# vgl-hub/kreeq

Hardware: AMD Instinct MI355X
Metric: distinct+total k-mers/sec at k=21 (count path) (higher is better)
Workload: dtype u64

## Files before the change

### include/kreeq_amd.h

```cpp
#ifndef KREEQ_AMD_H
#define KREEQ_AMD_H

#include <stdint.h>

#ifdef __cplusplus
extern "C" {
#endif

#define KQ_ABI_VERSION 4

typedef enum {
    KQ_OK = 0,
    KQ_ERR_INVALID = -1,
    KQ_ERR_NO_DEVICE = -2,
    KQ_ERR_HIP = -3,
    KQ_ERR_NOMEM = -4,
    KQ_ERR_TABLE_FULL = -5,
    KQ_ERR_CAPACITY = -6,
    KQ_ERR_MISMATCH = -7
} kq_status;

typedef struct kq_handle kq_handle;

typedef struct {
    uint64_t key;
    uint32_t fw[4], bw[4], cov;
    uint32_t hc;
} kq_entry;

typedef struct {
    uint32_t fw, bw, cov;
    uint8_t  isFw;
    uint8_t  pad[3];
} kq_dbgbase;

typedef struct {
    uint64_t total;
    uint64_t unique;
    uint64_t distinct;
    uint64_t missing;
    uint64_t edges;
} kq_stats;

typedef struct {
    uint64_t kmers_counted;
    uint64_t slots_used;
    uint64_t slots_total;
    uint64_t hc_used;
    uint64_t hc_total;
    uint64_t table_bytes;
    uint64_t table_passes;
} kq_info;


int  kq_create(kq_handle** out, int device, int k, int map_count, uint64_t capacity_hint);
void kq_destroy(kq_handle* h);
int  kq_clear(kq_handle* h);
int  kq_set_stream(kq_handle* h, void* hip_stream);
void* kq_get_stream(kq_handle* h);
enum { KQ_OPT_TRUST_CAPACITY = 1, KQ_OPT_COUNT_PATH = 2, KQ_OPT_SLICE_KMERS = 3, KQ_OPT_COUNT_MAP_RANGE = 4, KQ_OPT_PROFILE = 5,
       KQ_OPT_LOOKUP_PATH = 6, KQ_OPT_MERGE_PATH = 7, KQ_OPT_NARROW_MID = 8, KQ_OPT_PENDING_BYTES = 9, KQ_OPT_BUCKET_WINDOW = 10, KQ_OPT_OVERLAP = 11, KQ_OPT_COUNT_MAP_PASSES = 12, KQ_OPT_KERNEL_SET = 13, KQ_OPT_SHARD_WINDOW = 14, KQ_OPT_SUBGRAPH_BATCH = 15, KQ_OPT_VARIANT_BATCH = 16,
       KQ_OPT_TEST_FAIL_PLAN = 100  };
int  kq_set_option(kq_handle* h, int option, int64_t value);
int  kq_get_profile(kq_handle* h, char* buf, uint64_t cap);
int  kq_sync(kq_handle* h);
int  kq_flush(kq_handle* h);
int  kq_get_info(kq_handle* h, kq_info* out);
const char* kq_last_error(void);
int  kq_abi_version(void);
int  kq_device_available(void);
int  kq_device_memory(int device, uint64_t* free_bytes, uint64_t* total_bytes);


int  kq_count_batch(kq_handle* h, const char* bases, uint64_t len);
int  kq_count_batch_dev(kq_handle* h, const char* d_bases, uint64_t len);

void* kq_host_alloc(uint64_t bytes);
void  kq_host_free(void* p);
int  kq_count_batch_async(kq_handle* h, const char* bases, uint64_t len, uint64_t* ticket);
int  kq_host_wait(kq_handle* h, uint64_t ticket);

void kq_pack_bases(const char* bases, uint64_t len, uint32_t* codes, uint16_t* inv);
int  kq_count_packed_dev(kq_handle* h, const uint32_t* d_codes, const uint16_t* d_inv, uint64_t n_bases);
int  kq_count_packed_async(kq_handle* h, const uint32_t* codes, const uint16_t* inv, uint64_t n_bases, uint64_t* ticket);

int  kq_pack_bases_dev(kq_handle* h, const char* d_bases, uint64_t len, uint32_t* d_codes, uint16_t* d_inv);

enum { KQ_FASTX_FASTQ = 1, KQ_FASTX_FASTA = 2 };
int  kq_parse_fastx_dev(kq_handle* h, const char* d_text, uint64_t len, int format, char* d_bases, uint64_t cap, uint64_t* n_bases);
int  kq_count_fastx_dev(kq_handle* h, const char* d_text, uint64_t len, int format);
int  kq_count_fastx_async(kq_handle* h, const char* text, uint64_t len, int format, uint64_t* ticket);

typedef struct { uint64_t off; uint32_t size; uint32_t data_off; uint32_t data_len; uint32_t crc32; uint32_t isize; } kq_bgzf_block;
enum { KQ_BGZF_END = 1 };
int  kq_bgzf_scan(const void* data, uint64_t len, kq_bgzf_block* blocks, uint64_t cap, uint64_t* n_blocks, uint64_t* consumed);
int  kq_inflate_bgzf_dev(kq_handle* h, const void* d_comp, uint64_t comp_len, const kq_bgzf_block* blocks, uint64_t n_blocks,
                         char* d_text, uint64_t cap, uint64_t* n_text);
int  kq_count_bgzf_dev(kq_handle* h, const void* d_comp, uint64_t comp_len, const kq_bgzf_block* blocks, uint64_t n_blocks, int format, uint32_t flags);

enum { KQ_BGZF_EOF = 2 };
uint64_t kq_bgzf_bound(uint64_t n_text, uint32_t flags);
int  kq_deflate_bgzf_dev(kq_handle* h, const char* d_text, uint64_t n_text, void* d_out, uint64_t cap, uint64_t* n_out, uint32_t flags);
int  kq_deflate_bgzf(kq_handle* h, const char* text, uint64_t n_text, void* out, uint64_t cap, uint64_t* n_out, uint32_t flags);

int  kq_emit_records(kq_handle* h, const char* bases, uint64_t len,
                     uint64_t* keys, uint8_t* edges, uint64_t cap, uint64_t* n_out);
int  kq_emit_partitioned_dev(kq_handle* h, const char* d_bases, uint64_t len, int n_parts,
                             uint64_t* d_keys, uint8_t* d_edges, uint64_t cap,
                             uint64_t* part_counts);

int  kq_emit_packed_dev(kq_handle* h, const char* d_bases, uint64_t len, int n_parts,
                        uint64_t* d_recs, uint64_t cap, uint64_t* part_counts);
int  kq_insert_packed_dev(kq_handle* h, const uint64_t* d_recs, uint64_t n);

int  kq_emit_sharded_dev(kq_handle* h, const char* d_bases, uint64_t len, int n_parts, uint32_t* d_recs, uint8_t* d_aux, uint64_t cap,
                         uint64_t* d_bucket_counts, uint64_t* part_counts);
int  kq_insert_sharded_dev(kq_handle* h, const uint32_t* d_recs, const uint8_t* d_aux, uint64_t n, int n_peers, const uint64_t* d_bucket_counts);

int  kq_emit_sharded8_dev(kq_handle* h, const char* d_bases, uint64_t len, int n_parts, uint64_t* d_recs, uint64_t cap,
                          uint64_t* d_bucket_counts, uint64_t* part_counts);
int  kq_insert_sharded8_dev(kq_handle* h, const uint64_t* d_recs, uint64_t n, int n_peers, const uint64_t* d_bucket_counts);

int  kq_insert_records(kq_handle* h, const uint64_t* keys, const uint8_t* edges, uint64_t n);
int  kq_insert_records_dev(kq_handle* h, const uint64_t* d_keys, const uint8_t* d_edges, uint64_t n);


int  kq_summary(kq_handle* h, kq_stats* out);
int  kq_histogram(kq_handle* h, uint64_t* cov, uint64_t* cnt, uint64_t cap, uint64_t* n_out);


int  kq_lookup_sequence(kq_handle* h, const char* bases, uint64_t len, uint32_t cov_cutoff,
                        uint16_t map_lo, uint16_t map_hi, kq_dbgbase* per_base,
                        uint64_t counters[3]);
int  kq_lookup_sequence_dev(kq_handle* h, const char* d_bases, uint64_t len, uint32_t cov_cutoff,
                            uint16_t map_lo, uint16_t map_hi, kq_dbgbase* d_per_base,
                            uint64_t* d_counters);


enum { KQ_COPY_TO_DEVICE = 1, KQ_COPY_TO_HOST = 2 };
void* kq_dev_alloc(kq_handle* h, uint64_t bytes);
void  kq_dev_free(kq_handle* h, void* p);
int   kq_copy_async(kq_handle* h, void* dst, const void* src, uint64_t bytes, int kind);

int  kq_per_base_triples_dev(kq_handle* h, const kq_dbgbase* d_per_base, const uint64_t* seg_start, const uint64_t* seg_len,
                             uint64_t n_segs, uint32_t* d_triples);

int  kq_per_base_merge_dev(kq_handle* h, kq_dbgbase* d_per_base, const uint64_t* seg_start, const uint64_t* seg_len,
                           uint64_t n_segs, uint32_t* d_triples);

typedef struct { uint64_t first, n, abs_pos; uint32_t name_off, name_len, n_ctx, flags; } kq_table_seg;
enum { KQ_TABLE_SEG_HEADER = 1 };
enum { KQ_TABLE_KWIG = 1, KQ_TABLE_BED = 2, KQ_TABLE_CSV = 3 };
int  kq_format_table_dev(kq_handle* h, int format, const uint32_t* d_triples, uint64_t n_triples, const kq_table_seg* segs, uint64_t n_segs,
                         const char* names, uint64_t names_len, char* d_out, uint64_t cap, uint64_t* n_out);
int  kq_format_table(kq_handle* h, int format, const uint32_t* triples, uint64_t n_triples, const kq_table_seg* segs, uint64_t n_segs,
                     const char* names, uint64_t names_len, char* out, uint64_t cap, uint64_t* n_out);


int  kq_lookup_keys(kq_handle* h, const uint64_t* keys, uint64_t n, kq_entry* out);

int  kq_branch_scan(kq_handle* h, const char* bases, uint64_t len, uint32_t cov_cutoff, uint8_t* flags);

typedef struct { uint64_t pos, seg_start, seq_off; uint16_t seq_len, ref_len; uint8_t type, pad[3]; } kq_variant_path;
enum { KQ_VAR_SNV = 0, KQ_VAR_INS = 1, KQ_VAR_DEL = 2, KQ_VAR_COM = 3 };
int  kq_search_variants(kq_handle* h, const char* bases, uint64_t len, int depth, int max_span, uint32_t cov_cutoff,
                        kq_variant_path* paths, uint64_t path_cap, uint64_t* n_paths,
                        char* seq, uint64_t seq_cap, uint64_t* n_seq);


int  kq_merge(kq_handle* dst, kq_handle* src);

int  kq_import(kq_handle* h, const kq_entry* entries, uint64_t n);
int  kq_export(kq_handle* h, uint16_t map_lo, uint16_t map_hi, kq_entry* out, uint64_t cap,
               uint64_t* n_out);


int  kq_export_map_images(kq_handle* h, uint16_t map_lo, uint16_t map_hi, void* out, uint64_t cap, uint64_t* offsets,
                          kq_entry* hc_out, uint64_t hc_cap, uint64_t* n_hc);
int  kq_import_map_image(kq_handle* h, uint16_t map, const void* image, uint64_t n_bytes, uint64_t* n_entries,
                         uint64_t* n_tombstones);


enum { KQ_SUBGRAPH_NO_REFERENCE = 1 };
int  kq_subgraph_seed(kq_handle* db, kq_handle* sub, const char* bases, uint64_t len, uint32_t flags);
int  kq_subgraph_seed_dev(kq_handle* db, kq_handle* sub, const char* d_bases, uint64_t len, uint32_t flags);
int  kq_subgraph_expand(kq_handle* db, kq_handle* sub, int depth, uint64_t* n_added);
int  kq_subgraph_best_first(kq_handle* db, kq_handle* sub, int depth, uint32_t cov_cutoff, uint64_t* n_added);
int  kq_subgraph_trim(kq_handle* sub, uint32_t cov_cutoff);

typedef struct { uint64_t seq_off, head_key; uint32_t n_kmers, cov; uint8_t head_rc, pad[7]; } kq_gfa_segment;
typedef struct { uint32_t from, to, count; uint8_t from_rc, to_rc, pad[2]; } kq_gfa_edge;
typedef struct { uint64_t n_segments, n_seq, n_edges, n_dropped_edges, n_cycles; } kq_gfa_counts;
enum { KQ_GFA_NO_COLLAPSE = 1 };
int  kq_subgraph_gfa(kq_handle* sub, uint32_t flags, kq_gfa_segment* segs, uint64_t seg_cap, char* seq, uint64_t seq_cap,
                     kq_gfa_edge* edges, uint64_t edge_cap, kq_gfa_counts* counts);

#ifdef __cplusplus
}
#endif
#endif
```

### kreeq_amd/capi.py

```python
import ctypes as C
import os

import numpy as np

from . import build as _build

ENTRY_DTYPE = np.dtype([("key", "<u8"), ("fw", "<u4", 4), ("bw", "<u4", 4), ("cov", "<u4"), ("hc", "<u4")])
DBGBASE_DTYPE = np.dtype([("fw", "<u4"), ("bw", "<u4"), ("cov", "<u4"), ("isFw", "u1"), ("pad", "u1", 3)])
VARIANT_PATH_DTYPE = np.dtype([("pos", "<u8"), ("seg_start", "<u8"), ("seq_off", "<u8"), ("seq_len", "<u2"), ("ref_len", "<u2"), ("type", "u1"), ("pad", "u1", 3)])
VAR_SNV, VAR_INS, VAR_DEL, VAR_COM = 0, 1, 2, 3
ERR_CAPACITY = -6

SYMBOLS = ["kq_create", "kq_destroy", "kq_clear", "kq_set_option", "kq_get_profile", "kq_set_stream", "kq_get_stream", "kq_sync", "kq_flush", "kq_get_info", "kq_last_error",
           "kq_abi_version", "kq_device_available", "kq_device_memory", "kq_count_batch", "kq_count_batch_dev", "kq_host_alloc", "kq_host_free", "kq_count_batch_async", "kq_host_wait", "kq_pack_bases", "kq_count_packed_dev", "kq_count_packed_async",
           "kq_pack_bases_dev", "kq_parse_fastx_dev", "kq_count_fastx_dev", "kq_count_fastx_async", "kq_bgzf_scan", "kq_inflate_bgzf_dev", "kq_count_bgzf_dev", "kq_bgzf_bound", "kq_deflate_bgzf_dev", "kq_deflate_bgzf", "kq_emit_records",
           "kq_emit_partitioned_dev", "kq_emit_packed_dev", "kq_insert_packed_dev", "kq_emit_sharded_dev", "kq_insert_sharded_dev", "kq_emit_sharded8_dev", "kq_insert_sharded8_dev", "kq_insert_records", "kq_insert_records_dev", "kq_summary", "kq_histogram",
           "kq_lookup_sequence", "kq_lookup_sequence_dev", "kq_dev_alloc", "kq_dev_free", "kq_copy_async", "kq_per_base_triples_dev", "kq_per_base_merge_dev", "kq_format_table_dev", "kq_format_table", "kq_lookup_keys", "kq_branch_scan", "kq_search_variants", "kq_merge", "kq_import", "kq_export",
           "kq_export_map_images", "kq_import_map_image", "kq_subgraph_seed", "kq_subgraph_seed_dev", "kq_subgraph_expand", "kq_subgraph_best_first", "kq_subgraph_trim", "kq_subgraph_gfa"]

FASTX_FASTQ, FASTX_FASTA = 1, 2
BGZF_END = 1
BGZF_EOF = 2
BGZF_MEMBER_TEXT = 0xff00
BGZF_BLOCK_DTYPE = np.dtype([("off", "<u8"), ("size", "<u4"), ("data_off", "<u4"), ("data_len", "<u4"), ("crc32", "<u4"), ("isize", "<u4"), ("pad", "<u4")])
# ... 64 lines not shown
    L = C.CDLL(path)
    vp, u64, u32, u16, ci = C.c_void_p, C.c_uint64, C.c_uint32, C.c_uint16, C.c_int
    L.kq_create.argtypes = [C.POINTER(vp), ci, ci, ci, u64]
    L.kq_destroy.argtypes = [vp]
    L.kq_destroy.restype = None
    L.kq_clear.argtypes = [vp]
    L.kq_set_stream.argtypes = [vp, vp]
    L.kq_set_option.argtypes = [vp, ci, C.c_int64]
    L.kq_get_profile.argtypes = [vp, C.c_char_p, u64]
    L.kq_get_stream.argtypes = [vp]
    L.kq_get_stream.restype = vp
    L.kq_sync.argtypes = [vp]
    L.kq_flush.argtypes = [vp]
    L.kq_get_info.argtypes = [vp, C.POINTER(Info)]
    L.kq_last_error.restype = C.c_char_p
    L.kq_device_memory.argtypes = [ci, C.POINTER(u64), C.POINTER(u64)]
    L.kq_count_batch.argtypes = [vp, vp, u64]
    L.kq_count_batch_dev.argtypes = [vp, vp, u64]
    L.kq_host_alloc.argtypes = [u64]
    L.kq_host_alloc.restype = vp
    L.kq_host_free.argtypes = [vp]
    L.kq_host_free.restype = None
    L.kq_count_batch_async.argtypes = [vp, vp, u64, C.POINTER(u64)]
    L.kq_host_wait.argtypes = [vp, u64]
    L.kq_pack_bases.argtypes = [vp, u64, vp, vp]
    L.kq_pack_bases.restype = None
    L.kq_count_packed_dev.argtypes = [vp, vp, vp, u64]
    L.kq_count_packed_async.argtypes = [vp, vp, vp, u64, C.POINTER(u64)]
    L.kq_pack_bases_dev.argtypes = [vp, vp, u64, vp, vp]
    L.kq_parse_fastx_dev.argtypes = [vp, vp, u64, ci, vp, u64, C.POINTER(u64)]
    L.kq_count_fastx_dev.argtypes = [vp, vp, u64, ci]
    L.kq_count_fastx_async.argtypes = [vp, vp, u64, ci, C.POINTER(u64)]
    L.kq_bgzf_scan.argtypes = [vp, u64, vp, u64, C.POINTER(u64), C.POINTER(u64)]
    L.kq_inflate_bgzf_dev.argtypes = [vp, vp, u64, vp, u64, vp, u64, C.POINTER(u64)]
    L.kq_count_bgzf_dev.argtypes = [vp, vp, u64, vp, u64, ci, u32]
    L.kq_bgzf_bound.argtypes = [u64, u32]
    L.kq_bgzf_bound.restype = u64
    L.kq_deflate_bgzf_dev.argtypes = [vp, vp, u64, vp, u64, C.POINTER(u64), u32]
    L.kq_deflate_bgzf.argtypes = [vp, vp, u64, vp, u64, C.POINTER(u64), u32]
    L.kq_emit_records.argtypes = [vp, vp, u64, vp, vp, u64, C.POINTER(u64)]
    L.kq_emit_partitioned_dev.argtypes = [vp, vp, u64, ci, vp, vp, u64, vp]
    L.kq_emit_packed_dev.argtypes = [vp, vp, u64, ci, vp, u64, vp]
    L.kq_insert_packed_dev.argtypes = [vp, vp, u64]
    L.kq_emit_sharded_dev.argtypes = [vp, vp, u64, ci, vp, vp, u64, vp, vp]
    L.kq_insert_sharded_dev.argtypes = [vp, vp, vp, u64, ci, vp]
    L.kq_emit_sharded8_dev.argtypes = [vp, vp, u64, ci, vp, u64, vp, vp]
    L.kq_insert_sharded8_dev.argtypes = [vp, vp, u64, ci, vp]
    L.kq_insert_records.argtypes = [vp, vp, vp, u64]
    L.kq_insert_records_dev.argtypes = [vp, vp, vp, u64]
    L.kq_summary.argtypes = [vp, C.POINTER(Stats)]
    L.kq_histogram.argtypes = [vp, vp, vp, u64, C.POINTER(u64)]
    L.kq_lookup_sequence.argtypes = [vp, vp, u64, u32, u16, u16, vp, vp]
    L.kq_lookup_sequence_dev.argtypes = [vp, vp, u64, u32, u16, u16, vp, vp]
    L.kq_dev_alloc.argtypes = [vp, u64]
    L.kq_dev_alloc.restype = vp
    L.kq_dev_free.argtypes = [vp, vp]
    L.kq_dev_free.restype = None
    L.kq_copy_async.argtypes = [vp, vp, vp, u64, ci]
    L.kq_per_base_triples_dev.argtypes = [vp, vp, vp, vp, u64, vp]
    L.kq_per_base_merge_dev.argtypes = [vp, vp, vp, vp, u64, vp]
    L.kq_format_table_dev.argtypes = [vp, ci, vp, u64, vp, u64, vp, u64, vp, u64, C.POINTER(u64)]
    L.kq_format_table.argtypes = [vp, ci, vp, u64, vp, u64, vp, u64, vp, u64, C.POINTER(u64)]
    L.kq_lookup_keys.argtypes = [vp, vp, u64, vp]
    L.kq_branch_scan.argtypes = [vp, vp, u64, u32, vp]
    L.kq_search_variants.argtypes = [vp, vp, u64, ci, ci, u32, vp, u64, C.POINTER(u64), vp, u64, C.POINTER(u64)]
    L.kq_merge.argtypes = [vp, vp]
    L.kq_import.argtypes = [vp, vp, u64]
    L.kq_export.argtypes = [vp, u16, u16, vp, u64, C.POINTER(u64)]
    L.kq_export_map_images.argtypes = [vp, u16, u16, vp, u64, vp, vp, u64, C.POINTER(u64)]
    L.kq_import_map_image.argtypes = [vp, u16, vp, u64, C.POINTER(u64), C.POINTER(u64)]
    L.kq_subgraph_seed.argtypes = [vp, vp, vp, u64, u32]
    L.kq_subgraph_seed_dev.argtypes = [vp, vp, vp, u64, u32]
    L.kq_subgraph_expand.argtypes = [vp, vp, ci, C.POINTER(u64)]
    L.kq_subgraph_best_first.argtypes = [vp, vp, ci, u32, C.POINTER(u64)]
    L.kq_subgraph_trim.argtypes = [vp, u32]
    L.kq_subgraph_gfa.argtypes = [vp, u32, vp, u64, vp, u64, vp, u64, C.POINTER(GfaCounts)]
    _lib = L
    return L


def _check(rc):
    if rc != 0:
        raise KqError(rc, load().kq_last_error().decode(errors="replace"))


def _p(a):
    return a.ctypes.data_as(C.c_void_p) if a is not None else None


def pack_bases(bases: bytes):
    buf = np.frombuffer(bases, dtype=np.uint8)
    units = (len(buf) + 15) // 16
    codes, inv = np.zeros(max(units, 1), dtype=np.uint32), np.zeros(max(units, 1), dtype=np.uint16)
    load().kq_pack_bases(_p(buf) if len(buf) else None, len(buf), _p(codes), _p(inv))
    return codes[:units], inv[:units]


def bgzf_bound(n_text, flags=0):
    return int(load().kq_bgzf_bound(n_text, flags))


def bgzf_scan(data: bytes, cap=None):
    buf = np.frombuffer(data, dtype=np.uint8)
    n, used = C.c_uint64(0), C.c_uint64(0)
    L = load()
    room = len(buf) // 26 + 1 if cap is None else cap
    blocks = np.zeros(max(room, 1), dtype=BGZF_BLOCK_DTYPE)
    rc = L.kq_bgzf_scan(_p(buf) if len(buf) else None, len(buf), _p(blocks) if room else None, room, C.byref(n), C.byref(used))
    if rc != 0:
        e = KqError(rc, L.kq_last_error().decode(errors="replace"))
        e.n_blocks, e.consumed = n.value, used.value
        raise e
    return blocks[:n.value], used.value


def device_available():
    return bool(load().kq_device_available())


def device_memory(device=0):
    f, t = C.c_uint64(0), C.c_uint64(0)
    _check(load().kq_device_memory(device, C.byref(f), C.byref(t)))
    return f.value, t.value


class KreeqDB:

    def __init__(self, k=21, map_count=128, device=0, capacity_hint=0):
        self.k, self.map_count, self.device = k, map_count, device
        self._h = C.c_void_p()
        _check(load().kq_create(C.byref(self._h), device, k, map_count, capacity_hint))

    def close(self, _load=load):
        if getattr(self, "_h", None):
            _load().kq_destroy(self._h)
            self._h = None

    __del__ = close

    @property
    def handle(self):
        return self._h

    def set_stream(self, hip_stream_ptr):
        _check(load().kq_set_stream(self._h, C.c_void_p(hip_stream_ptr)))

    def sync(self):
        _check(load().kq_sync(self._h))

    def flush(self):
        _check(load().kq_flush(self._h))

    def set_option(self, option, value):
        opt = {"trust_capacity": 1, "count_path": 2, "slice_kmers": 3, "count_map_range": 4, "profile": 5, "lookup_path": 6, "merge_path": 7, "narrow_mid": 8, "pending_bytes": 9, "bucket_window": 10, "overlap": 11, "count_map_passes": 12, "kernel_set": 13, "shard_window": 14, "subgraph_batch": 15, "variant_batch": 16, "test_fail_plan": 100}[option]
        if option == "count_map_range":
            value = int(value[0]) | (int(value[1]) << 16)
        if option in ("count_path", "lookup_path", "merge_path"):
            value = {"auto": 0, "direct": 1, "partitioned": 2}[value]
        _check(load().kq_set_option(self._h, opt, int(value)))

    def clear(self):
        _check(load().kq_clear(self._h))

    def profile(self):
        buf = C.create_string_buffer(1024)
        _check(load().kq_get_profile(self._h, buf, 1024))
        return {k: float(v) for k, v in (kv.split("=") for kv in buf.value.decode().split(";") if kv)}

    def info(self):
        i = Info()
        _check(load().kq_get_info(self._h, C.byref(i)))
        return {f: getattr(i, f) for f, _ in Info._fields_}

    def count_batch(self, bases: bytes):
        buf = np.frombuffer(bases, dtype=np.uint8)
        _check(load().kq_count_batch(self._h, _p(buf), len(buf)))

    def count_batch_async(self, host_ptr, n):
        t = C.c_uint64(0)
        _check(load().kq_count_batch_async(self._h, C.c_void_p(host_ptr), n, C.byref(t)))
        return t.value

    def count_packed_dev(self, codes_ptr, inv_ptr, n_bases):
        _check(load().kq_count_packed_dev(self._h, C.c_void_p(codes_ptr), C.c_void_p(inv_ptr), n_bases))

    def count_packed_async(self, codes_ptr, inv_ptr, n_bases):
        t = C.c_uint64(0)
        _check(load().kq_count_packed_async(self._h, C.c_void_p(codes_ptr), C.c_void_p(inv_ptr), n_bases, C.byref(t)))
        return t.value

    def pack_bases_dev(self, bases_ptr, n, codes_ptr, inv_ptr):
        _check(load().kq_pack_bases_dev(self._h, C.c_void_p(bases_ptr), n, C.c_void_p(codes_ptr), C.c_void_p(inv_ptr)))

    def parse_fastx_dev(self, text_ptr, n, fmt, out_ptr, cap):
        nb = C.c_uint64(0)
        rc = load().kq_parse_fastx_dev(self._h, C.c_void_p(text_ptr), n, fmt, C.c_void_p(out_ptr) if out_ptr else None, cap, C.byref(nb))
        if rc != 0:
            e = KqError(rc, load().kq_last_error().decode(errors="replace"))
            e.needed = nb.value
            raise e
        return nb.value

    def count_fastx_dev(self, text_ptr, n, fmt):
        _check(load().kq_count_fastx_dev(self._h, C.c_void_p(text_ptr), n, fmt))

    def count_fastx_async(self, host_ptr, n, fmt):
        t = C.c_uint64(0)
        _check(load().kq_count_fastx_async(self._h, C.c_void_p(host_ptr), n, fmt, C.byref(t)))
        return t.value

    def inflate_bgzf_dev(self, comp_ptr, comp_len, blocks, out_ptr, cap):
        blocks = np.ascontiguousarray(blocks, dtype=BGZF_BLOCK_DTYPE)
        nt = C.c_uint64(0)
        rc = load().kq_inflate_bgzf_dev(self._h, C.c_void_p(comp_ptr), comp_len, _p(blocks) if len(blocks) else None, len(blocks),
                                        C.c_void_p(out_ptr) if out_ptr else None, cap, C.byref(nt))
        if rc != 0:
            e = KqError(rc, load().kq_last_error().decode(errors="replace"))
            e.needed = nt.value
            raise e
        return nt.value

    def deflate_bgzf_dev(self, text_ptr, n_text, out_ptr, cap, flags=0):
        no = C.c_uint64(0)
        rc = load().kq_deflate_bgzf_dev(self._h, C.c_void_p(text_ptr) if text_ptr else None, n_text, C.c_void_p(out_ptr) if out_ptr else None, cap, C.byref(no), flags)
        if rc != 0:
            e = KqError(rc, load().kq_last_error().decode(errors="replace"))
            e.needed = no.value
            raise e
        return no.value

    def deflate_bgzf(self, text: bytes, flags=0, cap=None):
        src = np.frombuffer(text, dtype=np.uint8)
        room = bgzf_bound(len(src), flags) if cap is None else cap
        out = np.empty(max(room, 1), dtype=np.uint8)
        no = C.c_uint64(0)
        rc = load().kq_deflate_bgzf(self._h, _p(src) if len(src) else None, len(src), _p(out) if room else None, room, C.byref(no), flags)
        if rc != 0:
            e = KqError(rc, load().kq_last_error().decode(errors="replace"))
            e.needed = no.value
            raise e
        return out[:no.value].tobytes()

    def count_bgzf_dev(self, comp_ptr, comp_len, blocks, fmt, flags=0):
        blocks = np.ascontiguousarray(blocks, dtype=BGZF_BLOCK_DTYPE)
        _check(load().kq_count_bgzf_dev(self._h, C.c_void_p(comp_ptr), comp_len, _p(blocks) if len(blocks) else None, len(blocks), fmt, flags))

    def host_wait(self, ticket):
        _check(load().kq_host_wait(self._h, ticket))

    def count_batch_dev(self, ptr, n):
        _check(load().kq_count_batch_dev(self._h, C.c_void_p(ptr), n))

    def emit_records(self, bases: bytes):
        buf = np.frombuffer(bases, dtype=np.uint8)
        n = C.c_uint64(0)
        _check(load().kq_emit_records(self._h, _p(buf), len(buf), None, None, 0, C.byref(n)))
        keys = np.empty(n.value, dtype=np.uint64)
        edges = np.empty(n.value, dtype=np.uint8)
        if n.value:
            _check(load().kq_emit_records(self._h, _p(buf), len(buf), _p(keys), _p(edges), n.value, C.byref(n)))
        return keys, edges

    def emit_partitioned_dev(self, bases_ptr, n, n_parts, keys_ptr, edges_ptr, cap):
        counts = np.zeros(n_parts, dtype=np.uint64)
        _check(load().kq_emit_partitioned_dev(self._h, C.c_void_p(bases_ptr), n, n_parts, C.c_void_p(keys_ptr), C.c_void_p(edges_ptr),
                                              cap, _p(counts)))
        return counts

    def emit_packed_dev(self, bases_ptr, n, n_parts, recs_ptr, cap):
        counts = np.zeros(n_parts, dtype=np.uint64)
        _check(load().kq_emit_packed_dev(self._h, C.c_void_p(bases_ptr), n, n_parts, C.c_void_p(recs_ptr), cap, _p(counts)))
        return counts

    def insert_packed_dev(self, recs_ptr, n):
        _check(load().kq_insert_packed_dev(self._h, C.c_void_p(recs_ptr), n))

    def emit_sharded_dev(self, bases_ptr, n, n_parts, recs_ptr, aux_ptr, cap, bucket_counts_ptr, sync=True):
        counts = np.zeros(n_parts, dtype=np.uint64) if sync else None
        _check(load().kq_emit_sharded_dev(self._h, C.c_void_p(bases_ptr), n, n_parts, C.c_void_p(recs_ptr), C.c_void_p(aux_ptr), cap,
                                          C.c_void_p(bucket_counts_ptr), _p(counts)))
        return counts

    def insert_sharded_dev(self, recs_ptr, aux_ptr, n, n_peers, bucket_counts_ptr):
        _check(load().kq_insert_sharded_dev(self._h, C.c_void_p(recs_ptr), C.c_void_p(aux_ptr), n, n_peers, C.c_void_p(bucket_counts_ptr)))

    def emit_sharded8_dev(self, bases_ptr, n, n_parts, recs_ptr, cap, bucket_counts_ptr, sync=True):
        counts = np.zeros(n_parts, dtype=np.uint64) if sync else None
        _check(load().kq_emit_sharded8_dev(self._h, C.c_void_p(bases_ptr), n, n_parts, C.c_void_p(recs_ptr), cap,
                                           C.c_void_p(bucket_counts_ptr), _p(counts)))
        return counts

    def insert_sharded8_dev(self, recs_ptr, n, n_peers, bucket_counts_ptr):
        _check(load().kq_insert_sharded8_dev(self._h, C.c_void_p(recs_ptr), n, n_peers, C.c_void_p(bucket_counts_ptr)))

    def insert_records(self, keys, edges):
        keys = np.ascontiguousarray(keys, dtype=np.uint64)
        edges = np.ascontiguousarray(edges, dtype=np.uint8)
        assert len(keys) == len(edges)
        _check(load().kq_insert_records(self._h, _p(keys), _p(edges), len(keys)))

    def insert_records_dev(self, keys_ptr, edges_ptr, n):
        _check(load().kq_insert_records_dev(self._h, C.c_void_p(keys_ptr), C.c_void_p(edges_ptr), n))

    def summary(self, with_hist=False):
        st = Stats()
        _check(load().kq_summary(self._h, C.byref(st)))
        d = {f: getattr(st, f) for f, _ in Stats._fields_}
# ... 165 lines not shown
```

### kreeq_amd/csrc/kq_formats.h

```cpp
#pragma once
#include <cstdint>
namespace kq {
#ifndef KQ_REGION_SHIFT
#define KQ_REGION_SHIFT 11
#endif
constexpr int REGION_SHIFT = KQ_REGION_SHIFT;
constexpr uint32_t REGION_SLOTS = 1u << REGION_SHIFT;
constexpr int HI_K = 29;
constexpr int TILE_STARTS = 4032;
constexpr uint64_t n_tiles_of(uint64_t lead, uint64_t len) { return (lead + len + TILE_STARTS - 1) / TILE_STARTS; }
struct EmitRange { uint64_t lo, hi; };

constexpr int NB_MAX = 2048;
constexpr int PART_MAX_K = 28;
constexpr int FMT_PACK8 = 0, FMT_WIDE = 1, FMT_NARROW = 2;
constexpr int FMT_PACK8_TO_NARROW = 3;
constexpr uint32_t NARROW_CBITS = 8, NARROW_MAX_K = 21;
constexpr int FMT_TOP8 = 4;
constexpr int FMT_TIGHT = 5;
constexpr int FMT_NARROW_TO_TIGHT = 6;

constexpr int MS_THREADS = 256;
constexpr int MS_ITEMS = 16;
constexpr int MS_TILE = MS_THREADS * MS_ITEMS;
constexpr int SEG_MAX = 65536;
constexpr uint32_t SUB_BITS_MAX = 8;
constexpr int AUX_IDX6 = 0, AUX_EDGE_BYTE = 1, AUX_TIGHT = 2;
constexpr uint64_t TIGHT_MIN_REGIONS = 1ull << 16;
constexpr int P1_F = 1;
constexpr uint32_t P2_UNIT = 4 * MS_TILE;
constexpr uint32_t SCAN_CHUNK = 16384;

struct PartCfg {
    uint64_t n_regions;
    uint32_t g_shift;
    uint32_t n_coarse;
    uint32_t mode;
    uint32_t map_count;
    uint32_t map_mask;
    uint32_t filt_lo, filt_hi;
    uint32_t raw_out;
    uint32_t narrow;
    uint32_t owner_sub;
    uint32_t sub_bits;
    uint32_t win_lo, win_hi;
    uint32_t n_rng;
};

constexpr int P3_MAX_SETS = 64;
struct P3Set { const uint64_t* recs; const uint8_t* aux; const unsigned long long* base; uint64_t n_max; };

struct LevelCfg {
    uint64_t n_regions;
    uint32_t n_seg, nb, seg_shift, out_shift;
    uint32_t in_raw;
    uint32_t k;
    uint32_t narrow;
    uint32_t top8;
    uint32_t nr_shift, nr_rps, nr_sub, nr_div, nr_inv;
    uint32_t nr_mid, nr_fshift, nr_fmask, nr_f24;
    uint32_t spb;
    uint32_t rep_shift;
    const uint32_t* rstart = nullptr;
};
}
```

### kreeq_amd/csrc/kq_kernels.h

```cpp
#pragma once

#include <hip/hip_runtime.h>

#include <type_traits>

#include "../../include/kreeq_amd.h"
#include "kq_device.h"
#include "kq_partition.h"

using namespace kq;


__global__ __launch_bounds__(TILE_THREADS) void k_count_direct(TableView t, const uint8_t* __restrict__ ab,
                                                                uint64_t lead, uint64_t len, int k, EmitRange er, PartCfg filt,
                                                                const uint16_t* __restrict__ pinv ) {
    uint32_t n_new = 0;
    uint64_t n_kmers = 0;
    scan_tiles(ab, lead, len, k, [&](uint64_t pos, uint64_t fw, uint64_t rv, uint32_t prev, uint32_t next) {
        if (pos < er.lo || pos >= er.hi) return;
        const bool is_fw = fw < rv;
        const uint64_t key = is_fw ? fw : rv;
        if (filt.filt_lo != 0 || filt.filt_hi != filt.map_count) {
            const uint32_t m = map_index(key, filt.map_count, filt.map_mask);
            if (m < filt.filt_lo || m >= filt.filt_hi) return;
// ... 360 lines not shown
        __syncthreads();
        const uint32_t total = __builtin_amdgcn_readfirstlane(s_loff[NB]);
        s_hist[ct] = 0;
        p1c_steps(total, (uint32_t)THREADS, [&](auto n_it) {
            constexpr int N = decltype(n_it)::value;
            uint64_t cv[N];
            uint32_t cg[N];
#pragma unroll
            for (int it = 0; it < N; ++it) cv[it] = s_buf[ct + it * THREADS];
#pragma unroll
            for (int it = 0; it < N; ++it) cg[it] = s_grel[ct + it * THREADS < total ? narrow_word_bin(cv[it]) : 0u] + (ct + it * THREADS);
            landed(nxt.x); landed(nxt.y); landed(nxt.z); landed(nxt.w);
#pragma unroll
            for (int it = 0; it < N; ++it) {
                if (ct + it * THREADS < total) { recs[cg[it]] = (uint32_t)cv[it]; recs_aux[cg[it]] = (uint8_t)(cv[it] >> 48); }
            }
        });
        landed(nxt.x); landed(nxt.y); landed(nxt.z); landed(nxt.w);
    }
}

__global__ __launch_bounds__(1024) void k_lv_units(const unsigned long long* __restrict__ seg_off, const unsigned long long* __restrict__ seg_hi, LevelCfg lv,
                                                   unsigned long long* __restrict__ unit_base) {
    __shared__ unsigned long long s_part[1024];
    const uint32_t tid = threadIdx.x, per = (lv.n_seg + 1023) / 1024;
    const uint32_t lo = min(tid * per, lv.n_seg), hi = min(lo + per, lv.n_seg);
    unsigned long long sum = 0;
    for (uint32_t b = lo; b < hi; ++b) sum += (seg_hi[b] - seg_off[b] + P2_UNIT - 1) / P2_UNIT;
    s_part[tid] = sum;
    __syncthreads();
    if (tid < 64) {
        unsigned long long loc[16], tot = 0;
#pragma unroll
        for (int j = 0; j < 16; ++j) { loc[j] = s_part[tid * 16 + j]; tot += loc[j]; }
        unsigned long long incl = tot;
#pragma unroll
        for (int o = 1; o < 64; o <<= 1) { unsigned long long nn = __shfl_up(incl, o, 64); if ((int)tid >= o) incl += nn; }
        unsigned long long run = incl - tot;
#pragma unroll
        for (int j = 0; j < 16; ++j) { s_part[tid * 16 + j] = run; run += loc[j]; }
        if (tid == 63) unit_base[lv.n_seg] = incl;
    }
    __syncthreads();
    unsigned long long run = s_part[tid];
    for (uint32_t b = lo; b < hi; ++b) { unit_base[b] = run; run += (seg_hi[b] - seg_off[b] + P2_UNIT - 1) / P2_UNIT; }
}
__device__ __forceinline__ uint32_t seg_of_unit(const unsigned long long* unit_base, uint32_t n_seg, uint64_t u) {
    uint32_t lo = 0, hi = n_seg;
    while (hi - lo > 1) { uint32_t mid = (lo + hi) >> 1; if (unit_base[mid] <= u) lo = mid; else hi = mid; }
    return lo;
}
template <int FMT>
__global__ __launch_bounds__(MS_THREADS) void k_lv_hist(const uint64_t* __restrict__ recs, const uint8_t* __restrict__ , LevelCfg lv,
                                                        const unsigned long long* __restrict__ seg_off, const unsigned long long* __restrict__ seg_hi,
                                                        const unsigned long long* __restrict__ unit_base, uint32_t* __restrict__ m2) {
    __shared__ uint32_t s_hist[NB_MAX];
    const uint64_t n_units = unit_base[lv.n_seg];
    for (uint64_t u = blockIdx.x; u < n_units; u += gridDim.x) {
        const uint32_t b_in = seg_of_unit(unit_base, lv.n_seg, u);
        const uint32_t b = lv.spb > 1 ? b_in / lv.spb : b_in;
        const uint64_t lo = seg_off[b_in] + (u - unit_base[b_in]) * P2_UNIT;
        const uint64_t hi = lo + P2_UNIT < seg_hi[b_in] ? lo + P2_UNIT : seg_hi[b_in];
        for (uint32_t i = threadIdx.x; i < lv.nb; i += MS_THREADS) s_hist[i] = 0;
        __syncthreads();
        const uint64_t last = hi - 1;
        if (FMT == FMT_NARROW) {
            const uint4* v4 = reinterpret_cast<const uint4*>(recs);
            const uint64_t q0 = lo >> 2, q1 = (hi + 3) >> 2;
            for (uint64_t qb = q0; qb < q1; qb += 4ull * MS_THREADS) {
                uint4 q[4];
#pragma unroll
                for (int j = 0; j < 4; ++j) q[j] = v4[min(qb + (uint64_t)j * MS_THREADS + threadIdx.x, q1 - 1)];
#pragma unroll
                for (int j = 0; j < 4; ++j) {
                    const uint64_t qi = qb + (uint64_t)j * MS_THREADS + threadIdx.x;
                    const uint32_t e[4] = {q[j].x, q[j].y, q[j].z, q[j].w};
#pragma unroll
                    for (int c = 0; c < 4; ++c) {
                        const uint64_t ri = 4 * qi + c;
                        if (qi < q1 && ri >= lo && ri < hi) atomicAdd(&s_hist[narrow_bin(lv, b, e[c])], 1u);
                    }
                }
            }
        } else
        for (uint64_t base = lo; base < hi; base += 8ull * MS_THREADS) {
            uint64_t r[8];
#pragma unroll
            for (int j = 0; j < 8; ++j) {
                const uint64_t i = min(base + (uint64_t)j * MS_THREADS + threadIdx.x, last);
                r[j] = FMT == FMT_NARROW ? (uint64_t)reinterpret_cast<const uint32_t*>(recs)[i] : recs[i];
            }
#pragma unroll
            for (int j = 0; j < 8; ++j)
                if (base + (uint64_t)j * MS_THREADS + threadIdx.x < hi) {
                    const uint32_t bin = FMT == FMT_NARROW ? narrow_bin(lv, b, (uint32_t)r[j])
                        : FMT == FMT_TOP8 ? narrow_bin(lv, b, (uint32_t)(r[j] >> 32))
                        : (FMT == FMT_PACK8 && lv.top8) ? (uint32_t)(rec_hash<false>(r[j]) >> (64 - NARROW_CBITS))
                        : level_bin(lv, b, hash_region(lv.in_raw ? table_hash(r[j], lv.k) : rec_hash<FMT == FMT_WIDE>(r[j]), lv.n_regions));
                    atomicAdd(&s_hist[bin], 1u);
                }
        }
        __syncthreads();
        for (uint32_t i = threadIdx.x; i < lv.nb; i += MS_THREADS) m2[u * lv.nb + i] = s_hist[i];
        __syncthreads();
    }
}
__global__ __launch_bounds__(256) void k_lv_offsets(uint32_t* __restrict__ m2, LevelCfg lv, const unsigned long long* __restrict__ unit_base,
                                                    unsigned long long* __restrict__ group_count) {
    const uint64_t r = ((uint64_t)blockIdx.x * blockDim.x + threadIdx.x) >> 6;
    const uint32_t lane = threadIdx.x & 63;
    const uint32_t n_lseg = lv.n_seg / lv.spb;
    if (r >= (uint64_t)n_lseg * lv.nb) return;
    const uint32_t b = (uint32_t)(r / lv.nb), bin = (uint32_t)(r % lv.nb);
    const uint64_t u0 = unit_base[b * lv.spb], u1 = unit_base[(b + 1) * lv.spb];
    unsigned long long run = 0;
    for (uint64_t base = u0; base < u1; base += 64) {
        const uint64_t u = base + lane;
        const uint32_t c = u < u1 ? m2[u * lv.nb + bin] : 0u;
        unsigned long long incl = c;
#pragma unroll
        for (int o = 1; o < 64; o <<= 1) { const unsigned long long n = __shfl_up(incl, o, 64); if ((int)lane >= o) incl += n; }
        if (u < u1) m2[u * lv.nb + bin] = (uint32_t)(run + incl - c);
        run += __shfl(incl, 63, 64);
    }
    if (lane == 0) group_count[r] = run;
}
__global__ __launch_bounds__(256) void k_lv_offsets_thread(uint32_t* __restrict__ m2, LevelCfg lv, const unsigned long long* __restrict__ unit_base,
                                                           unsigned long long* __restrict__ group_count) {
    const uint64_t r = (uint64_t)blockIdx.x * blockDim.x + threadIdx.x;
    const uint32_t n_lseg = lv.n_seg / lv.spb;
    if (r >= (uint64_t)n_lseg * lv.nb) return;
    const uint32_t b = (uint32_t)(r / lv.nb), bin = (uint32_t)(r % lv.nb);
    const uint64_t u0 = unit_base[b * lv.spb], u1 = unit_base[(b + 1) * lv.spb];
    unsigned long long run = 0;
    for (uint64_t u = u0; u < u1; ++u) {
        const uint32_t c = m2[u * lv.nb + bin];
        m2[u * lv.nb + bin] = (uint32_t)run;
        run += c;
    }
    group_count[r] = run;
}
#ifndef KQ_LV_THREADS
#define KQ_LV_THREADS 512
#define KQ_LV_ITEMS 8
#define KQ_LV_OCC 4
#endif
constexpr int LV_THREADS = KQ_LV_THREADS, LV_ITEMS = KQ_LV_ITEMS, LV_TILE = LV_THREADS * LV_ITEMS;
template <int FMT, int NBC>
__global__ __launch_bounds__(LV_THREADS, KQ_LV_OCC) void k_lv_scatter(const uint64_t* __restrict__ recs, const uint8_t* __restrict__ recs_aux, LevelCfg lv,
                                                           const unsigned long long* __restrict__ seg_off, const unsigned long long* __restrict__ seg_hi,
                                                           const unsigned long long* __restrict__ unit_base, const uint32_t* __restrict__ m2,
                                                           const unsigned long long* __restrict__ group_base, uint64_t* __restrict__ out,
                                                           uint8_t* __restrict__ out_aux) {
    constexpr bool WIDE = FMT == FMT_WIDE, TIGHT = FMT == FMT_NARROW_TO_TIGHT, NARROW = FMT == FMT_NARROW || TIGHT, CONVERT = FMT == FMT_PACK8_TO_NARROW,
                   TOP8 = FMT == FMT_TOP8, HAS_AUX = WIDE || NARROW;
    constexpr int MS_FMT = (CONVERT || TIGHT) ? FMT_NARROW : TOP8 ? FMT_PACK8 : FMT;
    const uint32_t* recs32 = reinterpret_cast<const uint32_t*>(recs);
    __shared__ MsShared<NBC, MS_FMT, LV_TILE> s;
    __shared__ uint32_t s_rst[TIGHT ? NBC : 1];
    const uint32_t nb = lv.nb;
    const uint64_t n_units = unit_base[lv.n_seg];
    for (uint64_t u = blockIdx.x; u < n_units; u += gridDim.x) {
        const uint32_t b_in = seg_of_unit(unit_base, lv.n_seg, u);
        const uint32_t b = lv.spb > 1 ? b_in / lv.spb : b_in;
        const uint64_t lo = seg_off[b_in] + (u - unit_base[b_in]) * P2_UNIT;
        const uint64_t hi = lo + P2_UNIT < seg_hi[b_in] ? lo + P2_UNIT : seg_hi[b_in];
        for (uint32_t i = threadIdx.x; i < nb; i += LV_THREADS)
            s.gbase[i] = (uint32_t)(group_base[(uint64_t)b * nb + i] + m2[u * nb + i]);
        if (TIGHT) {
            const uint32_t first = (b >> lv.nr_shift) * lv.nr_rps + (b & ((1u << lv.nr_shift) - 1u)) * lv.nr_sub;
            for (uint32_t i = threadIdx.x; i < nb; i += LV_THREADS) s_rst[i] = lv.rstart[first + i];
        }
        __syncthreads();
        uint64_t nxt[LV_ITEMS];
        uint32_t nxt_aux[LV_ITEMS];
        const uint64_t last = hi - 1;
#pragma unroll
        for (int j = 0; j < LV_ITEMS; ++j) {
            const uint64_t i = min(lo + (uint64_t)j * LV_THREADS + threadIdx.x, last);
            nxt[j] = NARROW ? (uint64_t)recs32[i] : recs[i];
            nxt_aux[j] = HAS_AUX ? recs_aux[i] : 0;
        }
#pragma unroll
        for (int j = 0; j < LV_ITEMS; ++j) { landed(nxt[j]); if (HAS_AUX) landed(nxt_aux[j]); }
        for (uint64_t pos = lo; pos < hi; pos += LV_TILE) {
            uint64_t rec[LV_ITEMS];
            uint32_t aux[LV_ITEMS], bin[LV_ITEMS];
#pragma unroll
            for (int j = 0; j < LV_ITEMS; ++j) {
                const uint64_t i = pos + (uint64_t)j * LV_THREADS + threadIdx.x;
                rec[j] = (WIDE && lv.in_raw) ? table_hash(nxt[j], lv.k) : nxt[j];
                aux[j] = nxt_aux[j];
                if (TIGHT) {
                    const uint32_t bn = i >= hi ? nb : narrow_bin(lv, b, (uint32_t)rec[j]);
                    rec[j] = narrow_word(tight_rec(b >> lv.nr_shift, (uint32_t)rec[j], aux[j], s_rst[bn < nb ? bn : 0u]), 0u, bn);
                }
                else if (NARROW) rec[j] = narrow_word((uint32_t)rec[j], aux[j], i >= hi ? nb : narrow_bin(lv, b, (uint32_t)rec[j]));
                else if (CONVERT) {
                    const uint64_t hh = rec_hash<false>(rec[j]);
                    rec[j] = narrow_word(narrow_main(hh), narrow_aux(hh, (uint32_t)(rec[j] >> REC_EDGE_SHIFT) & 63u), i >= hi ? nb : (uint32_t)(hh >> (64 - NARROW_CBITS)));
                }
                else if (TOP8) bin[j] = i >= hi ? nb : narrow_bin(lv, b, (uint32_t)(rec[j] >> 32));
                else bin[j] = i >= hi ? nb : level_bin(lv, b, hash_region(rec_hash<WIDE>(rec[j]), lv.n_regions));
            }
#pragma unroll
            for (int j = 0; j < LV_ITEMS; ++j) {
                const uint64_t i = min(pos + LV_TILE + (uint64_t)j * LV_THREADS + threadIdx.x, last);
                nxt[j] = NARROW ? (uint64_t)recs32[i] : recs[i];
                nxt_aux[j] = HAS_AUX ? recs_aux[i] : 0;
            }
            block_multisplit<MS_FMT, LV_THREADS, LV_ITEMS>(s, rec, aux, bin, nb, out, out_aux, [&] {
#pragma unroll
                for (int j = 0; j < LV_ITEMS; ++j) { landed(nxt[j]); if (HAS_AUX) landed(nxt_aux[j]); }
            }, NBC <= 512 ? lv.rep_shift : 0u);
        }
    }
}
#ifndef KQ_LVS_OCC
#define KQ_LVS_OCC 4
#define KQ_LVS_OCC_TIGHT 4
#endif
template <bool TIGHT>
__global__ __launch_bounds__(LV_THREADS, TIGHT ? KQ_LVS_OCC_TIGHT : KQ_LVS_OCC) void k_lv_scatter_s(const uint32_t* __restrict__ recs32, const uint8_t* __restrict__ recs_aux, LevelCfg lv,
                                                           const unsigned long long* __restrict__ seg_off, const unsigned long long* __restrict__ seg_hi,
                                                           const unsigned long long* __restrict__ unit_base, const uint32_t* __restrict__ m2,
                                                           const unsigned long long* __restrict__ group_base, uint32_t* __restrict__ out,
                                                           uint8_t* __restrict__ out_aux) {
    constexpr int NC = 512;
    static_assert(LV_THREADS == NC && LV_ITEMS == 8, "one counter per thread");
    __shared__ uint64_t s_buf[LV_TILE];
    __shared__ uint32_t s_hist[2][NC], s_loff[NC + 1], s_grel[NC], s_wave[LV_THREADS / 64];
    __shared__ uint32_t s_rst[TIGHT ? NC : 1];
    const int tid = threadIdx.x;
    const uint32_t nb = lv.nb, rs = lv.rep_shift, n_ctr = (nb + 1) << rs;
    const uint32_t sub = (uint32_t)tid & ((1u << rs) - 1u), my_bin = (uint32_t)tid >> rs;
    const bool own_bin = sub == 0 && my_bin < nb;
    const uint64_t n_units = unit_base[lv.n_seg];
    for (uint64_t u = blockIdx.x; u < n_units; u += gridDim.x) {
        const uint32_t b_in = seg_of_unit(unit_base, lv.n_seg, u);
        const uint32_t b = lv.spb > 1 ? b_in / lv.spb : b_in;
        const uint64_t lo = seg_off[b_in] + (u - unit_base[b_in]) * P2_UNIT;
        const uint64_t hi = lo + P2_UNIT < seg_hi[b_in] ? lo + P2_UNIT : seg_hi[b_in];
        uint32_t gabs = own_bin ? (uint32_t)(group_base[(uint64_t)b * nb + my_bin] + m2[u * nb + my_bin]) : 0u;
        if (TIGHT) {
            const uint32_t first = (b >> lv.nr_shift) * lv.nr_rps + (b & ((1u << lv.nr_shift) - 1u)) * lv.nr_sub;
            if ((uint32_t)tid < nb) s_rst[tid] = lv.rstart[first + tid];
        }
        s_hist[0][tid] = 0;
        __syncthreads();
        uint32_t nxt[LV_ITEMS], nxt_aux[LV_ITEMS];
        const uint64_t last = hi - 1;
#pragma unroll
        for (int j = 0; j < LV_ITEMS; ++j) {
            const uint64_t i = min(lo + (uint64_t)j * LV_THREADS + tid, last);
            nxt[j] = recs32[i];
            nxt_aux[j] = recs_aux[i];
        }
#pragma unroll
        for (int j = 0; j < LV_ITEMS; ++j) { landed(nxt[j]); landed(nxt_aux[j]); }
        uint32_t par = 0;
        for (uint64_t pos = lo; pos < hi; pos += LV_TILE, par ^= 1u) {
            uint32_t* hist = s_hist[par];
            uint64_t w[LV_ITEMS];
#pragma unroll
            for (int j = 0; j < LV_ITEMS; ++j) {
                const uint64_t i = pos + (uint64_t)j * LV_THREADS + tid;
                const uint32_t bn = i >= hi ? nb : narrow_bin(lv, b, nxt[j]);
                w[j] = TIGHT ? narrow_word(tight_rec(b >> lv.nr_shift, nxt[j], nxt_aux[j], s_rst[bn < nb ? bn : 0u]), 0u, bn) : narrow_word(nxt[j], nxt_aux[j], bn);
                if (bn != nb) atomicAdd(&hist[(bn << rs) | sub], 1u);
            }
#pragma unroll
            for (int j = 0; j < LV_ITEMS; ++j) {
                const uint64_t i = min(pos + LV_TILE + (uint64_t)j * LV_THREADS + tid, last);
                nxt[j] = recs32[i];
                nxt_aux[j] = recs_aux[i];
            }
            __syncthreads();
            const uint32_t cnt = (uint32_t)tid < n_ctr ? hist[tid] : 0u;
            uint32_t incl = cnt;
#pragma unroll
            for (int o = 1; o < 64; o <<= 1) { const uint32_t n = __shfl_up(incl, o, 64); if ((tid & 63) >= o) incl += n; }
            if ((tid & 63) == 63) s_wave[tid >> 6] = incl;
            s_hist[par ^ 1u][tid] = 0;
            __syncthreads();
            uint32_t excl = incl - cnt;
            for (int v = 0; v < (tid >> 6); ++v) excl += s_wave[v];
            s_loff[tid] = excl;
            hist[tid] = excl;
            if (own_bin) s_grel[my_bin] = gabs - excl;
            __syncthreads();
            if (own_bin) gabs += s_loff[(my_bin + 1) << rs] - excl;
#pragma unroll
            for (int j = 0; j < LV_ITEMS; ++j) {
                const uint32_t bn = narrow_word_bin(w[j]);
                if (bn != nb) s_buf[atomicAdd(&hist[(bn << rs) | sub], 1u)] = w[j];
            }
            __syncthreads();
            const uint32_t total = s_loff[nb << rs];
            uint64_t cv[LV_ITEMS];
            uint32_t cg[LV_ITEMS];
#pragma unroll
            for (int it = 0; it < LV_ITEMS; ++it) cv[it] = s_buf[tid + it * LV_THREADS];
#pragma unroll
            for (int it = 0; it < LV_ITEMS; ++it) cg[it] = s_grel[(uint32_t)(tid + it * LV_THREADS) < total ? narrow_word_bin(cv[it]) : 0u] + (tid + it * LV_THREADS);
#pragma unroll
            for (int j = 0; j < LV_ITEMS; ++j) { landed(nxt[j]); landed(nxt_aux[j]); }
#pragma unroll
            for (int it = 0; it < LV_ITEMS; ++it) {
                if ((uint32_t)(tid + it * LV_THREADS) < total) {
                    out[cg[it]] = (uint32_t)cv[it];
                    if (!TIGHT) out_aux[cg[it]] = (uint8_t)(cv[it] >> 48);
                }
            }
        }
    }
}
#ifndef KQ_LVG_BACK
#define KQ_LVG_BACK 0
#endif
__global__ __launch_bounds__(LV_THREADS, KQ_LVS_OCC_TIGHT) void k_lv_segment_s(const uint32_t* __restrict__ recs32, const uint8_t* __restrict__ recs_aux, LevelCfg lv,
                                                           const unsigned long long* __restrict__ seg_off, unsigned long long* __restrict__ gb,
                                                           uint32_t* __restrict__ out) {
    constexpr int NC = 512;
    constexpr bool BACK = KQ_LVG_BACK != 0;
    static_assert(LV_THREADS == NC && LV_ITEMS == 8, "one counter per thread");
    __shared__ uint64_t s_buf[LV_TILE];
    __shared__ uint32_t s_hist[2][NC], s_loff[NC + 1], s_grel[NC], s_wave[LV_THREADS / 64], s_rst[NC];
    const int tid = threadIdx.x;
    const uint32_t nb = lv.nb, rs = lv.rep_shift, n_ctr = (nb + 1) << rs;
    const uint32_t sub = (uint32_t)tid & ((1u << rs) - 1u), my_bin = (uint32_t)tid >> rs;
    const bool own_bin = sub == 0 && my_bin < nb;
    const uint32_t b = blockIdx.x;
    const uint64_t lo = seg_off[b], hi = seg_off[b + 1];
    {
        const uint32_t first = (b >> lv.nr_shift) * lv.nr_rps + (b & ((1u << lv.nr_shift) - 1u)) * lv.nr_sub;
        if ((uint32_t)tid < nb) s_rst[tid] = lv.rstart[first + tid];
    }
    s_hist[0][tid] = 0;
    s_hist[1][tid] = 0;
    __syncthreads();
    {
        const uint4* v4 = reinterpret_cast<const uint4*>(recs32);
        const uint64_t q0 = lo >> 2, q1 = hi > lo ? (hi + 3) >> 2 : q0;
        for (uint64_t qb = q0; qb < q1; qb += 4ull * LV_THREADS) {
            uint4 q[4];
#pragma unroll
            for (int j = 0; j < 4; ++j) q[j] = v4[min(qb + (uint64_t)j * LV_THREADS + tid, q1 - 1)];
#pragma unroll
            for (int j = 0; j < 4; ++j) {
                const uint64_t qi = qb + (uint64_t)j * LV_THREADS + tid;
                const uint32_t e[4] = {q[j].x, q[j].y, q[j].z, q[j].w};
#pragma unroll
                for (int c = 0; c < 4; ++c) {
                    const uint64_t ri = 4 * qi + c;
                    if (qi < q1 && ri >= lo && ri < hi) atomicAdd(&s_hist[1][(narrow_bin(lv, b, e[c]) << rs) | sub], 1u);
                }
            }
        }
    }
    __syncthreads();
    uint32_t gabs = 0;
    {
        uint32_t cnt = 0;
        if (own_bin) for (uint32_t r = 0; r < (1u << rs); ++r) cnt += s_hist[1][(uint32_t)tid + r];
        uint32_t incl = cnt;
#pragma unroll
        for (int o = 1; o < 64; o <<= 1) { const uint32_t n = __shfl_up(incl, o, 64); if ((tid & 63) >= o) incl += n; }
        if ((tid & 63) == 63) s_wave[tid >> 6] = incl;
        __syncthreads();
        uint32_t excl = incl - cnt;
        for (int v = 0; v < (tid >> 6); ++v) excl += s_wave[v];
        if (own_bin) {
            gabs = (uint32_t)lo + excl;
            gb[(uint64_t)b * nb + my_bin] = lo + excl;
        }
        if (b + 1 == lv.n_seg && tid == 0) gb[(uint64_t)lv.n_seg * nb] = hi;
    }
    if (hi == lo) return;
    uint32_t nxt[LV_ITEMS], nxt_aux[LV_ITEMS];
    const uint64_t last = hi - 1, n_rounds = (hi - lo + LV_TILE - 1) / LV_TILE;
    uint64_t pos = BACK ? lo + (n_rounds - 1) * LV_TILE : lo;
#pragma unroll
    for (int j = 0; j < LV_ITEMS; ++j) {
        const uint64_t i = min(pos + (uint64_t)j * LV_THREADS + tid, last);
        nxt[j] = recs32[i];
        nxt_aux[j] = recs_aux[i];
    }
#pragma unroll
    for (int j = 0; j < LV_ITEMS; ++j) { landed(nxt[j]); landed(nxt_aux[j]); }
    uint32_t par = 0;
    for (uint64_t r = 0; r < n_rounds; ++r, par ^= 1u) {
        uint32_t* hist = s_hist[par];
        uint64_t w[LV_ITEMS];
#pragma unroll
        for (int j = 0; j < LV_ITEMS; ++j) {
            const uint64_t i = pos + (uint64_t)j * LV_THREADS + tid;
            const uint32_t bn = i >= hi ? nb : narrow_bin(lv, b, nxt[j]);
            w[j] = narrow_word(tight_rec(b >> lv.nr_shift, nxt[j], nxt_aux[j], s_rst[bn < nb ? bn : 0u]), 0u, bn);
            if (bn != nb) atomicAdd(&hist[(bn << rs) | sub], 1u);
        }
        pos = BACK ? (r + 1 < n_rounds ? pos - LV_TILE : pos) : pos + LV_TILE;
#pragma unroll
        for (int j = 0; j < LV_ITEMS; ++j) {
            const uint64_t i = min(pos + (uint64_t)j * LV_THREADS + tid, last);
            nxt[j] = recs32[i];
            nxt_aux[j] = recs_aux[i];
        }
        __syncthreads();
        const uint32_t cnt = (uint32_t)tid < n_ctr ? hist[tid] : 0u;
        uint32_t incl = cnt;
#pragma unroll
        for (int o = 1; o < 64; o <<= 1) { const uint32_t n = __shfl_up(incl, o, 64); if ((tid & 63) >= o) incl += n; }
        if ((tid & 63) == 63) s_wave[tid >> 6] = incl;
        s_hist[par ^ 1u][tid] = 0;
        __syncthreads();
        uint32_t excl = incl - cnt;
        for (int v = 0; v < (tid >> 6); ++v) excl += s_wave[v];
        s_loff[tid] = excl;
        hist[tid] = excl;
        if (own_bin) s_grel[my_bin] = gabs - excl;
        __syncthreads();
        if (own_bin) gabs += s_loff[(my_bin + 1) << rs] - excl;
#pragma unroll
        for (int j = 0; j < LV_ITEMS; ++j) {
            const uint32_t bn = narrow_word_bin(w[j]);
            if (bn != nb) s_buf[atomicAdd(&hist[(bn << rs) | sub], 1u)] = w[j];
        }
        __syncthreads();
        const uint32_t total = s_loff[nb << rs];
        uint64_t cv[LV_ITEMS];
        uint32_t cg[LV_ITEMS];
#pragma unroll
        for (int it = 0; it < LV_ITEMS; ++it) cv[it] = s_buf[tid + it * LV_THREADS];
#pragma unroll
        for (int it = 0; it < LV_ITEMS; ++it) cg[it] = s_grel[(uint32_t)(tid + it * LV_THREADS) < total ? narrow_word_bin(cv[it]) : 0u] + (tid + it * LV_THREADS);
#pragma unroll
        for (int j = 0; j < LV_ITEMS; ++j) { landed(nxt[j]); landed(nxt_aux[j]); }
#pragma unroll
        for (int it = 0; it < LV_ITEMS; ++it)
            if ((uint32_t)(tid + it * LV_THREADS) < total) out[cg[it]] = (uint32_t)cv[it];
    }
}
__global__ void k_set2(unsigned long long* p, unsigned long long a, unsigned long long b) { p[0] = a; p[1] = b; }

__global__ __launch_bounds__(1024) void k_scan_sums(const unsigned long long* __restrict__ a, uint64_t n, unsigned long long* __restrict__ sums) {
    const uint64_t lo = (uint64_t)blockIdx.x * SCAN_CHUNK, hi = lo + SCAN_CHUNK < n ? lo + SCAN_CHUNK : n;
    unsigned long long v = 0;
    for (uint64_t i = lo + threadIdx.x; i < hi; i += 1024) v += a[i];
    uint64_t t = block_sum(v);
    if (threadIdx.x == 0) sums[blockIdx.x] = t;
}
__global__ __launch_bounds__(1024) void k_scan_apply(unsigned long long* __restrict__ a, uint64_t n, const unsigned long long* __restrict__ sums) {
    __shared__ unsigned long long s_part[1024];
    const uint64_t lo = (uint64_t)blockIdx.x * SCAN_CHUNK + (uint64_t)threadIdx.x * (SCAN_CHUNK / 1024);
    unsigned long long v[SCAN_CHUNK / 1024], sum = 0;
#pragma unroll
    for (uint32_t j = 0; j < SCAN_CHUNK / 1024; ++j) { v[j] = lo + j < n ? a[lo + j] : 0; sum += v[j]; }
    s_part[threadIdx.x] = sum;
    __syncthreads();
    if (threadIdx.x < 64) {
        unsigned long long loc[16], tot = 0;
#pragma unroll
        for (int j = 0; j < 16; ++j) { loc[j] = s_part[threadIdx.x * 16 + j]; tot += loc[j]; }
        unsigned long long incl = tot;
#pragma unroll
        for (int o = 1; o < 64; o <<= 1) { unsigned long long nn = __shfl_up(incl, o, 64); if ((int)threadIdx.x >= o) incl += nn; }
        unsigned long long run = incl - tot;
#pragma unroll
        for (int j = 0; j < 16; ++j) { s_part[threadIdx.x * 16 + j] = run; run += loc[j]; }
    }
    __syncthreads();
    unsigned long long run = sums[blockIdx.x] + s_part[threadIdx.x];
#pragma unroll
    for (uint32_t j = 0; j < SCAN_CHUNK / 1024; ++j) { if (lo + j < n) a[lo + j] = run; run += v[j]; }
}


template <class T> __device__ __forceinline__ T ld_global(const T* p) { return *(const __attribute__((address_space(1))) T*)p; }

template <uint32_t GRP, class LO = uint64_t>
struct SetTickets {
    LO lo; uint32_t cnt, first, n_grp;
    __device__ __forceinline__ void build(const P3Set* __restrict__ sets, uint32_t n_sets, uint64_t r, uint32_t lane) {
        lo = 0; cnt = 0;
        if (lane < n_sets) { const unsigned long long* b = ld_global(&sets[lane].base); lo = (LO)ld_global(b + r); cnt = (uint32_t)(ld_global(b + r + 1) - lo); }
        scan(lane);
    }
    __device__ __forceinline__ void build(const uint32_t* __restrict__ roff, uint32_t pitch, uint64_t r, uint32_t lane) {
        lo = 0; cnt = 0;
        if (lane < pitch) { const uint32_t* p = roff + r * pitch + lane; const uint32_t a = ld_global(p), b = ld_global(p + pitch); lo = a; cnt = b - a; }
        scan(lane);
    }
    __device__ __forceinline__ void scan(uint32_t lane) {
        const uint32_t mine = (cnt + GRP - 1) / GRP;
        uint32_t incl = mine;
#pragma unroll
        for (int o = 1; o < P3_MAX_SETS; o <<= 1) { const uint32_t v = __shfl_up(incl, o, 64); if ((int)lane >= o) incl += v; }
        first = incl - mine;
        n_grp = __builtin_amdgcn_readlane(incl, 63);
    }
    __device__ __forceinline__ void locate(uint32_t g, uint32_t& q, uint32_t& off, uint32_t& q_cnt, uint64_t& q_lo) const {
        const uint64_t nonempty = __ballot(cnt != 0);
        const uint64_t m = __ballot(cnt != 0 && first <= g);
        q = (g < n_grp && m) ? 63u - (uint32_t)__clzll((unsigned long long)m) : (uint32_t)__ffsll((unsigned long long)nonempty) - 1u;
        const uint32_t f = __builtin_amdgcn_readlane(first, q);
        q_cnt = __builtin_amdgcn_readlane(cnt, q);
        if constexpr (sizeof(LO) == 8) q_lo = ((uint64_t)__builtin_amdgcn_readlane((uint32_t)((uint64_t)lo >> 32), q) << 32) | __builtin_amdgcn_readlane((uint32_t)lo, q);
        else q_lo = __builtin_amdgcn_readlane((uint32_t)lo, q);
        off = (g < n_grp ? g - f : 0u) * GRP;
    }
};

template <int THREADS, bool HOT, class TK>
__device__ __forceinline__ bool region_gate_built(const TK& tk, const TableView& t, uint64_t r,
                                                  int table_is_empty, unsigned long long* __restrict__ hot_list ) {
    const int tid = threadIdx.x;
    uint64_t n_recs = tk.cnt;
#pragma unroll
    for (int o = 32; o > 0; o >>= 1) n_recs += __shfl_xor(n_recs, o, 64);
    if (n_recs == 0) {
        if (!HOT && table_is_empty == 2) {
            ulonglong2* g2 = reinterpret_cast<ulonglong2*>(t.slots + (r << REGION_SHIFT));
            for (int i = tid; i < (int)REGION_SLOTS; i += THREADS) g2[i] = make_ulonglong2(0ull, 0ull);
        }
        return false;
    }
    if (!HOT && n_recs > 32ull * REGION_SLOTS) {
        if (tid == 0) hot_list[1 + atomicAdd(&hot_list[0], 1ull)] = r;
        return false;
    }
    return true;
}
template <int THREADS, bool HOT, uint32_t GRP>
__device__ __forceinline__ bool region_gate(SetTickets<GRP>& tk, const TableView& t, const P3Set* __restrict__ sets, uint32_t n_sets, uint64_t r,
                                            int table_is_empty, unsigned long long* __restrict__ hot_list) {
    tk.build(sets, n_sets, r, threadIdx.x & 63u);
    return region_gate_built<THREADS, HOT>(tk, t, r, table_is_empty, hot_list);
}
constexpr int HC_LDS = 64;
__device__ __forceinline__ void hc_lds_reset(uint64_t (&hckey)[HC_LDS], uint32_t (&hccnt)[HC_LDS][8]) {
    const int tid = threadIdx.x;
    if (tid < HC_LDS) {
        hckey[tid] = EMPTY_KEY;
#pragma unroll
        for (int e = 0; e < 8; ++e) hccnt[tid][e] = 0;
    }
}
__device__ __forceinline__ void hc_lds_add(const TableView& t, uint64_t (&hckey)[HC_LDS], uint32_t (&hccnt)[HC_LDS][8], uint64_t h, const uint32_t (&e)[8]) {
    const uint64_t key = key_of_hash(h, t.k);
    int hslot = -1;
    uint32_t hp = (uint32_t)(h >> 40) & (HC_LDS - 1);
    for (int probe = 0; probe < HC_LDS; ++probe, hp = (hp + 1) & (HC_LDS - 1)) {
        uint64_t cur = __hip_atomic_load(&hckey[hp], __ATOMIC_RELAXED, __HIP_MEMORY_SCOPE_WORKGROUP);
        if (cur == EMPTY_KEY) cur = atomicCAS((unsigned long long*)&hckey[hp], (unsigned long long)EMPTY_KEY, (unsigned long long)key);
        if (cur == EMPTY_KEY || cur == key) { hslot = (int)hp; break; }
    }
    if (hslot >= 0) {
#pragma unroll
        for (int w = 0; w < 8; ++w) if (e[w]) atomicAdd(&hccnt[hslot][w], e[w]);
    } else {
        hc_add(t, h, 0, 0, e);
    }
}
__device__ __forceinline__ void hc_lds_flush(const TableView& t, uint64_t (&hckey)[HC_LDS], uint32_t (&hccnt)[HC_LDS][8]) {
    const int tid = threadIdx.x;
    if (tid < HC_LDS && hckey[tid] != EMPTY_KEY) {
        HcSlot* hs = hc_upsert(t, hckey[tid]);
        if (!hs) atomicOr(&t.st->err_hc_full, 1u);
        else {
#pragma unroll
            for (int e = 0; e < 8; ++e) if (hccnt[tid][e]) atomicAdd((unsigned long long*)&hs->cnt[e], (unsigned long long)hccnt[tid][e]);
        }
    }
}
template <class C>
__device__ __forceinline__ void region_totals_wave(uint32_t n_new, uint32_t n_ok, C& s_new, C& s_kmers) {
#pragma unroll
    for (int o = 32; o > 0; o >>= 1) { n_new += __shfl_down(n_new, o, 64); n_ok += __shfl_down(n_ok, o, 64); }
    if ((threadIdx.x & 63) == 0) { if (n_new) atomicAdd(&s_new, (C)n_new); if (n_ok) atomicAdd(&s_kmers, (C)n_ok); }
}
template <class C>
__device__ __forceinline__ void region_totals_store(const TableView& t, const C& s_new, const C& s_kmers) {
    if (threadIdx.x == 0) {
        if (s_new) atomicAdd(&t.st->slots_used, (unsigned long long)s_new);
        if (s_kmers) atomicAdd(&t.st->kmers_added, (unsigned long long)s_kmers);
    }
}

constexpr uint32_t TOT_LINES = 4096;
template <class C>
// ... 920 lines not shown
```

### kreeq_amd/csrc/kq_partition.h

```cpp
#pragma once
#include "kq_device.h"
#include "kq_formats.h"

namespace kq {

constexpr int REC_EDGE_SHIFT = 56;

__device__ __forceinline__ uint32_t level_bin(const LevelCfg& lv, uint32_t b, uint64_t region) {
    return (uint32_t)(region >> lv.out_shift) - (lv.seg_shift >= 32 ? 0u : (b << (lv.seg_shift - lv.out_shift)));
}

__device__ __forceinline__ uint32_t edge_idx6(bool is_fw, uint32_t prev, uint32_t next) {
    uint32_t f, b;
    if (is_fw) { f = next < 4 ? next : 7u; b = prev < 4 ? prev : 7u; }
    else       { f = prev < 4 ? 3u - prev : 7u; b = next < 4 ? 3u - next : 7u; }
    return f | (b << 3);
}
__device__ __forceinline__ uint32_t edge_idx6_any(bool is_fw, uint32_t prev, uint32_t next) {
    const uint32_t f = is_fw ? next : prev, b = is_fw ? prev : next, m = is_fw ? 0u : 0x1Bu;
    return (f | (b << 3)) ^ m;
}
__device__ __forceinline__ uint64_t rec_pack(uint64_t key, bool is_fw, uint32_t prev, uint32_t next) {
    return key | ((uint64_t)edge_idx6(is_fw, prev, next) << REC_EDGE_SHIFT);
}
__device__ __forceinline__ uint64_t idx6_to_pack(uint32_t v) {
    const uint32_t f = v & 7u, b = (v >> 3) & 7u;
    return (f < 4 ? 1ull << (8 * f) : 0ull) | (b < 4 ? 1ull << (8 * (4 + b)) : 0ull);
}
__device__ __forceinline__ uint32_t idx6_to_edge_byte(uint32_t v) {
    const uint32_t f = v & 7u, b = (v >> 3) & 7u;
    return (f < 4 ? 1u << (7 - f) : 0u) | (b < 4 ? 1u << (7 - (4 + b)) : 0u);
}
__device__ __forceinline__ uint64_t rec_key(uint64_t rec) { return rec & ((1ull << REC_EDGE_SHIFT) - 1); }
__device__ __forceinline__ uint64_t rec_edge_pack(uint64_t rec) {
    const uint32_t f = (uint32_t)(rec >> REC_EDGE_SHIFT) & 7u, b = (uint32_t)(rec >> (REC_EDGE_SHIFT + 3)) & 7u;
    return (f < 4 ? 1ull << (8 * f) : 0ull) | (b < 4 ? 1ull << (8 * (4 + b)) : 0ull);
}
template <bool WIDE>
__device__ __forceinline__ uint64_t rec_hash(uint64_t rec) { return WIDE ? rec : rec << 8; }
__device__ __forceinline__ uint64_t rec_pack_hash(uint64_t h, bool is_fw, uint32_t prev, uint32_t next) {
    return (h >> 8) | ((uint64_t)edge_idx6(is_fw, prev, next) << REC_EDGE_SHIFT);
}

__device__ __forceinline__ uint32_t tight_rec(uint32_t bucket, uint32_t main32, uint32_t aux, uint32_t rstart_r) {
    const uint32_t d = ((bucket << (32 - NARROW_CBITS)) | (main32 >> NARROW_CBITS)) - rstart_r;
    return (d << 16) | ((main32 & 0xFFu) << 8) | ((aux & 3u) << 6) | (aux >> 2);
}
__device__ __forceinline__ uint64_t tight_hash(uint32_t t, uint32_t rstart_r) { return ((uint64_t)((t >> 16) + rstart_r) << 32) | ((uint64_t)((t >> 6) & 1023u) << 22); }
__device__ __forceinline__ uint64_t top8_rec(uint64_t h, uint32_t idx6) { return ((h << NARROW_CBITS) & ~63ull) | idx6; }
__device__ __forceinline__ uint64_t top8_hash(uint32_t bucket, uint64_t rec) { return ((uint64_t)bucket << (64 - NARROW_CBITS)) | ((rec & ~63ull) >> NARROW_CBITS); }
__device__ __forceinline__ uint32_t narrow_main(uint64_t h) { return (uint32_t)(h >> (32 - NARROW_CBITS)); }
__device__ __forceinline__ uint32_t narrow_aux(uint64_t h, uint32_t idx6) { return ((uint32_t)(h >> (30 - NARROW_CBITS)) & 3u) | (idx6 << 2); }
__device__ __forceinline__ uint64_t narrow_hash(uint32_t bucket, uint32_t main32, uint32_t aux) {
    return ((uint64_t)bucket << (64 - NARROW_CBITS)) | ((uint64_t)main32 << (32 - NARROW_CBITS)) | ((uint64_t)(aux & 3u) << (30 - NARROW_CBITS));
}
__device__ __forceinline__ uint64_t narrow_word(uint32_t main32, uint32_t aux, uint32_t bin) { return (uint64_t)main32 | ((uint64_t)(bin | (aux << 16)) << 32); }
__device__ __forceinline__ uint32_t narrow_word_bin(uint64_t w) { return (uint32_t)(w >> 32) & 0xFFFFu; }
__device__ __forceinline__ uint32_t narrow_region(uint32_t bucket, uint32_t main32, uint64_t n_regions) {
    return __umulhi((bucket << (32 - NARROW_CBITS)) | (main32 >> NARROW_CBITS), (uint32_t)n_regions);
}
__device__ __forceinline__ uint32_t narrow_bin(const LevelCfg& lv, uint32_t , uint32_t main32) {
    const uint32_t f = main32 >> NARROW_CBITS;
    if (lv.nr_mid) return f >> lv.nr_fshift;
    const uint32_t fs = f & lv.nr_fmask;
    return lv.nr_f24 ? umul24u(fs, lv.nr_sub) >> lv.nr_fshift : (uint32_t)(((uint64_t)fs * lv.nr_sub) >> lv.nr_fshift);
}

template <int NBC, int FMT, int TILE = MS_TILE>
struct MsShared {
    static constexpr int tile = TILE;
    uint64_t stage[TILE];
    uint16_t sbin[FMT != FMT_NARROW ? TILE : 4];
    uint8_t  saux[FMT == FMT_WIDE ? TILE : 8];
    uint32_t hist[NBC];
    uint32_t loff[NBC];
    uint32_t gbase[NBC];
    uint32_t wave_sum[16];
};

template <int THREADS, class S>
__device__ __forceinline__ void ms_scan(S& s, uint32_t nb) {
    constexpr int NBC = (int)(sizeof(s.hist) / sizeof(uint32_t));
    constexpr int MS_BINS_PER_THREAD = (NBC + THREADS - 1) / THREADS;
    const int tid = threadIdx.x;
    uint32_t v[MS_BINS_PER_THREAD], sum = 0;
#pragma unroll
    for (int j = 0; j < MS_BINS_PER_THREAD; ++j) { uint32_t b = MS_BINS_PER_THREAD * tid + j; v[j] = (b < nb) ? s.hist[b] : 0; sum += v[j]; }
    uint32_t incl = sum;
#pragma unroll
    for (int o = 1; o < 64; o <<= 1) { uint32_t n = __shfl_up(incl, o, 64); if ((tid & 63) >= o) incl += n; }
    if ((tid & 63) == 63) s.wave_sum[tid >> 6] = incl;
    __syncthreads();
    uint32_t base = 0;
    for (int w = 0; w < (tid >> 6); ++w) base += s.wave_sum[w];
    uint32_t run = base + incl - sum;
#pragma unroll
    for (int j = 0; j < MS_BINS_PER_THREAD; ++j) { uint32_t b = MS_BINS_PER_THREAD * tid + j; if (b < nb) s.loff[b] = run; run += v[j]; }
    __syncthreads();
}

__device__ __forceinline__ void landed(uint32_t& v) { asm volatile("" : "+v"(v)); }
__device__ __forceinline__ void landed(uint64_t& v) { asm volatile("" : "+v"(v)); }
struct NoHook { __device__ __forceinline__ void operator()() const {} };
template <int FMT, int THREADS = MS_THREADS, int ITEMS = MS_ITEMS, class S, class F = NoHook>
__device__ __forceinline__ void block_multisplit(S& s, const uint64_t (&rec)[ITEMS], const uint32_t (&aux)[ITEMS],
                                                 const uint32_t (&bin)[ITEMS], uint32_t nb,
                                                 uint64_t* __restrict__ out, uint8_t* __restrict__ out_aux, F pre_store = F(), uint32_t rs = 0) {
    const int tid = threadIdx.x;
    const uint32_t sub = (uint32_t)tid & ((1u << rs) - 1u), n_ctr = (nb + 1) << rs;
    for (uint32_t b = tid; b < n_ctr; b += THREADS) s.hist[b] = 0;
    __syncthreads();
    static_assert(THREADS * ITEMS <= S::tile, "round size");
    uint32_t rank[ITEMS];
#pragma unroll
    for (int i = 0; i < ITEMS; ++i) {
        const uint32_t b = FMT == FMT_NARROW ? narrow_word_bin(rec[i]) : bin[i];
        rank[i] = 0;
        if (b != nb) rank[i] = atomicAdd(&s.hist[(b << rs) | sub], 1u);
    }
    __syncthreads();
    ms_scan<THREADS>(s, n_ctr);
    for (uint32_t b = tid; b < nb; b += THREADS) s.gbase[b] -= s.loff[b << rs];
#pragma unroll
    for (int i = 0; i < ITEMS; ++i) {
        const uint32_t b = FMT == FMT_NARROW ? narrow_word_bin(rec[i]) : bin[i];
        if (b == nb) continue;
        const uint32_t p = s.loff[(b << rs) | sub] + rank[i];
        if (FMT == FMT_NARROW) {
            s.stage[p] = rec[i];
        } else {
            s.stage[p] = rec[i];
            s.sbin[p] = (uint16_t)bin[i];
            if (FMT == FMT_WIDE) s.saux[p] = (uint8_t)aux[i];
        }
    }
    __syncthreads();
    const uint32_t total = s.loff[nb << rs];
    uint32_t cb[ITEMS];
    uint32_t cg[ITEMS];
    uint64_t cv[ITEMS];
    if (FMT == FMT_NARROW) {
#pragma unroll
        for (int it = 0; it < ITEMS; ++it) { cv[it] = s.stage[tid + it * THREADS]; cb[it] = (uint32_t)(tid + it * THREADS) < total ? narrow_word_bin(cv[it]) : 0u; }
    } else {
#pragma unroll
        for (int it = 0; it < ITEMS; ++it) { const uint32_t j = tid + it * THREADS; cb[it] = j < total ? s.sbin[j] : 0u; cv[it] = s.stage[j]; }
    }
#pragma unroll
    for (int it = 0; it < ITEMS; ++it) cg[it] = s.gbase[cb[it]] + (tid + it * THREADS);
    pre_store();
#pragma unroll
    for (int it = 0; it < ITEMS; ++it) {
        const uint32_t j = tid + it * THREADS;
        if (j < total) {
            if (FMT == FMT_NARROW) {
                reinterpret_cast<uint32_t*>(out)[cg[it]] = (uint32_t)cv[it];
                if (out_aux) out_aux[cg[it]] = (uint8_t)(cv[it] >> 48);
            } else {
                out[cg[it]] = cv[it];
                if (FMT == FMT_WIDE) out_aux[cg[it]] = s.saux[j];
            }
        }
    }
    __syncthreads();
    for (uint32_t b = tid; b < nb; b += THREADS) s.gbase[b] += s.loff[(b + 1) << rs];
}

__device__ __forceinline__ uint32_t owner_part_of(uint64_t key, uint32_t map_count, uint32_t map_mask, uint32_t n_parts) {
    const uint32_t m = map_mask ? (uint32_t)key & map_mask : (uint32_t)(key % map_count);
    return (uint32_t)(((uint64_t)m * n_parts) / map_count);
}
__device__ __forceinline__ uint32_t map_index(uint64_t key, uint32_t map_count, uint32_t map_mask) {
    return map_mask ? (uint32_t)key & map_mask : (uint32_t)(key % map_count);
}
__device__ __forceinline__ uint32_t p1_bin(const PartCfg& cfg, uint64_t key, uint64_t h) {
    if (cfg.filt_lo != 0 || cfg.filt_hi != cfg.map_count) {
        const uint32_t m = map_index(key, cfg.map_count, cfg.map_mask);
        if (m < cfg.filt_lo || m >= cfg.filt_hi) return cfg.n_coarse;
    }
    return cfg.mode == 0 ? (cfg.narrow ? (uint32_t)(h >> (64 - NARROW_CBITS)) : (uint32_t)(hash_region(h, cfg.n_regions) >> cfg.g_shift))
                         : (owner_part_of(key, cfg.map_count, cfg.map_mask, cfg.n_coarse >> cfg.owner_sub) << cfg.owner_sub) |
                           (threadIdx.x & ((1u << cfg.owner_sub) - 1u));
}

}
```

### kreeq_amd/csrc/kq_plan_host.h

```cpp
#pragma once
#include <algorithm>
#include <cstddef>
#include <cstdint>

#include "kq_formats.h"

namespace kq {

inline uint64_t round_regions(uint64_t regions, int k) {
    if (regions < 16) regions = 16;
    if (regions >= (uint64_t)NB_MAX || k >= HI_K) regions = (regions + 255) / 256 * 256;
    if (regions >= (1ull << 19)) {
        uint32_t sbits = 3;
        while (sbits < SUB_BITS_MAX && (((regions + 255) / 256) >> sbits) > 256) ++sbits;
        const uint64_t unit = 256ull << sbits;
        regions = (regions + unit - 1) / unit * unit;
    }
    return regions;
}
inline uint64_t initial_regions(uint64_t capacity_hint, int k) {
    const uint64_t slots = (uint64_t)((double)(capacity_hint ? capacity_hint : (1u << 20)) / 0.7);
    return round_regions((slots + REGION_SLOTS - 1) >> REGION_SHIFT, k);
}
struct GrowTarget { uint64_t slots, regions; bool ok; };
inline GrowTarget grow_target(uint64_t n_slots, uint64_t n_regions, uint64_t need_slots) {
    GrowTarget g{n_slots, n_regions, true};
    while (g.slots < need_slots) { g.slots *= 2; g.regions *= 2; }
    g.ok = g.regions < (1ull << 32);
    return g;
}
struct WindowGeom { uint64_t virt, alloc_new; bool ok; };
inline WindowGeom window_geometry(uint64_t alloc_now, uint32_t lo, uint32_t hi, int k) {
    const uint64_t nb = hi - lo;
    WindowGeom g;
    g.virt = round_regions(std::max<uint64_t>((alloc_now + nb - 1) / nb * 256, (uint64_t)NB_MAX), k);
    g.ok = g.virt < (1ull << 32);
    g.alloc_new = lo == 0 && hi == 256 ? g.virt : nb * (g.virt >> 8);
    return g;
}
inline uint64_t main_need(uint64_t used, uint64_t extra) { return (uint64_t)((double)(used + extra) / 0.85) + REGION_SLOTS; }
constexpr uint64_t HC_CAP_BIG = 1ull << 25;
constexpr uint64_t HC_UNOBSERVED = ~0ull;
inline bool hc_follows_fill(uint64_t kmers_bound) { return kmers_bound / 255 + 1 > (1ull << 23); }
inline uint64_t hc_need(uint64_t kmers_bound, uint64_t hc_used = HC_UNOBSERVED) {
    const uint64_t bound = kmers_bound / 255 + 1;
    uint64_t need = hc_follows_fill(kmers_bound) ? HC_CAP_BIG : 2 * bound;
    if (hc_used != HC_UNOBSERVED) need = std::max<uint64_t>(need, 8 * hc_used);
    return need;
}

struct TableShape { int k; uint64_t n_regions; int map_count; uint32_t mid_rps; };

inline PartCfg plan_cfg(const TableShape& t, bool allow_narrow = false) {
    PartCfg cfg;
    cfg.n_regions = t.n_regions;
    uint32_t g = 1;
    while (((cfg.n_regions + (1ull << g) - 1) >> g) > 512 && g < 10) ++g;
    while (((cfg.n_regions + (1ull << g) - 1) >> g) >= (uint64_t)NB_MAX) ++g;
    cfg.g_shift = cfg.n_regions < (uint64_t)NB_MAX ? 0 : g;
    cfg.n_coarse = (uint32_t)((cfg.n_regions + (1ull << cfg.g_shift) - 1) >> cfg.g_shift);
    cfg.mode = 0; cfg.map_count = (uint32_t)t.map_count;
    cfg.map_mask = (t.map_count & (t.map_count - 1)) == 0 ? (uint32_t)t.map_count - 1 : 0;
    cfg.filt_lo = 0; cfg.filt_hi = (uint32_t)t.map_count;
    cfg.raw_out = 0;
    cfg.narrow = 0; cfg.sub_bits = 0; cfg.owner_sub = 0; cfg.n_rng = 0; cfg.win_lo = 0; cfg.win_hi = 1u << NARROW_CBITS;
    if (allow_narrow && (t.k <= (int)NARROW_MAX_K || t.k > PART_MAX_K) && cfg.n_regions >= (uint64_t)NB_MAX && cfg.n_regions % (1u << NARROW_CBITS) == 0) {
        const uint64_t rps = cfg.n_regions >> NARROW_CBITS;
        uint32_t sb = 0;
        if (rps >= t.mid_rps) {
            const uint64_t target_nb = std::max<uint64_t>(1, std::min<uint64_t>(256, t.mid_rps / 8));
            while ((rps >> sb) > target_nb && sb < SUB_BITS_MAX && rps % (2ull << sb) == 0) ++sb;
        }
        if ((rps >> sb) < (uint64_t)NB_MAX && (sb > 0 || rps < (uint64_t)NB_MAX)) { cfg.narrow = 1; cfg.sub_bits = sb; }
    }
    if (cfg.narrow) { cfg.n_coarse = 1u << NARROW_CBITS; if (cfg.g_shift == 0) cfg.g_shift = 1; }
    return cfg;
}
inline bool part_table_ok(const TableShape& t, bool narrow_possible) {
    if (t.n_regions <= (1ull << 20)) return true;
    if (!narrow_possible) return false;
    return plan_cfg(t, true).narrow != 0;
}
inline int plan_fmt(const PartCfg& cfg, int k) { return !cfg.narrow ? FMT_PACK8 : k > PART_MAX_K ? FMT_TOP8 : FMT_NARROW; }
inline int sequence_fmt(int fmt, int k) { return k > PART_MAX_K && fmt != FMT_TOP8 ? FMT_WIDE : fmt; }
inline bool tight_ok(int fmt, uint64_t n_regions, bool has_region_starts) { return fmt == FMT_NARROW && n_regions >= TIGHT_MIN_REGIONS && has_region_starts; }

struct PlanSizes {
    PartCfg cfg;
    bool two_level;
    int fmt;
    uint64_t n_max, R;
    uint32_t g1;
    uint64_t m1_n, m2_n, sums_n, groups_n;
    uint64_t seg_max;
    uint64_t rec_words, aux_words;
    bool split2;
};
inline PlanSizes plan_sizes(const TableShape& t, int n_cu, uint64_t n_max, uint64_t n_tiles, uint32_t p1_bins, bool allow_narrow, uint64_t min_segs) {
    PlanSizes p;
    p.cfg = plan_cfg(t, allow_narrow);
    n_max = (n_max + 7) & ~7ull;
    p.two_level = p.cfg.g_shift != 0;
    p.fmt = plan_fmt(p.cfg, t.k);
    p.n_max = n_max; p.R = p.cfg.n_regions;
    p.g1 = (uint32_t)std::max<uint64_t>(1, std::min<uint64_t>(n_tiles, (uint64_t)n_cu * (p1_bins < 512 ? 18 : 12)));
    p.m1_n = (uint64_t)p1_bins * p.g1 * P1_F;
    const uint64_t nb_max = std::max<uint64_t>(std::max<uint64_t>(1ull << p.cfg.g_shift, p.cfg.n_coarse), p.cfg.narrow ? (p.cfg.n_regions >> NARROW_CBITS) >> p.cfg.sub_bits : 0);
    p.seg_max = std::max<uint64_t>(min_segs, p.cfg.narrow ? ((uint64_t)1 << NARROW_CBITS) << p.cfg.sub_bits : (uint64_t)NB_MAX);
    p.m2_n = (n_max / P2_UNIT + p.seg_max + 2) * nb_max;
    p.groups_n = std::max<uint64_t>(std::max<uint64_t>(p.R, (uint64_t)p.cfg.n_coarse << p.cfg.g_shift), min_segs) + 2;
    p.sums_n = std::max(p.m1_n, p.groups_n) / SCAN_CHUNK + 2;
    p.aux_words = (n_max + 7) / 8 + 1;
    p.rec_words = p.fmt == FMT_NARROW ? n_max / 2 + 2 : n_max;
    p.split2 = (p.rec_words + p.aux_words) * 8 >= ((size_t)512 << 20);
    return p;
}
struct PlanLayout { uint64_t recs1, aux1, recs2, aux2, m1, seg_off, unit_base, group_base, sums, total, hot, m2, words; size_t part2_bytes; };
inline PlanLayout plan_layout(const PlanSizes& p) {
    uint64_t here = 0, there = 0;
    auto take = [](uint64_t& cursor, uint64_t n_words) { const uint64_t at = cursor; cursor += n_words; return at; };
    PlanLayout l;
    l.recs1 = take(here, p.rec_words);
    l.aux1 = take(here, p.aux_words);
    uint64_t& second = p.split2 ? there : here;
    l.recs2 = take(second, p.rec_words);
    l.aux2 = take(second, p.aux_words);
    l.m1 = take(here, p.m1_n);
    l.seg_off = take(here, p.seg_max + 2);
    l.unit_base = take(here, p.seg_max + 2);
    l.group_base = take(here, p.groups_n);
    l.sums = take(here, p.sums_n);
    l.total = take(here, 4);
    l.hot = take(here, p.R + 2);
    l.m2 = take(here, (p.m2_n + 1) / 2);
    l.words = here;
    l.part2_bytes = (size_t)there * 8;
    return l;
}

inline LevelCfg with_rep_shift(const LevelCfg& lv) {
    LevelCfg lvr = lv;
    lvr.rep_shift = 0;
    while (lvr.rep_shift < 6 && (((uint64_t)lv.nb + 1) << (lvr.rep_shift + 1)) <= 512) ++lvr.rep_shift;
    return lvr;
}
inline LevelCfg level_coarse_to_regions(const PartCfg& cfg) {
    LevelCfg lv; lv.n_regions = cfg.n_regions; lv.n_seg = cfg.n_coarse; lv.nb = 1u << cfg.g_shift; lv.seg_shift = cfg.g_shift; lv.out_shift = 0; lv.in_raw = 0; lv.k = 0; lv.narrow = 0; lv.top8 = 0;
    lv.nr_shift = lv.nr_rps = lv.nr_sub = lv.nr_inv = 0; lv.nr_div = 1;
    lv.nr_mid = 0; lv.nr_fshift = 24; lv.nr_fmask = 0xFFFFFFu; lv.nr_f24 = 0;
    lv.spb = 1;
    return lv;
}
inline LevelCfg level_narrow(const PartCfg& cfg, uint32_t sub_bits = 0, bool middle = false, bool top8_records = false) {
    LevelCfg lv; lv.n_regions = cfg.n_regions;
    const uint32_t rps = (uint32_t)(cfg.n_regions >> NARROW_CBITS), subsz = rps >> sub_bits;
    lv.seg_shift = 0; lv.out_shift = 0; lv.in_raw = 0; lv.k = 0; lv.narrow = top8_records ? 2 : 1; lv.top8 = 0;
    lv.nr_rps = rps; lv.nr_sub = subsz;
    if (middle) { lv.n_seg = 1u << NARROW_CBITS; lv.nb = 1u << sub_bits; lv.nr_shift = 0; lv.nr_div = subsz; }
    else        { lv.n_seg = (1u << NARROW_CBITS) << sub_bits; lv.nb = subsz; lv.nr_shift = sub_bits; lv.nr_div = 1; }
    lv.nr_inv = lv.nr_div > 1 ? (uint32_t)(((1ull << 32) + lv.nr_div - 1) / lv.nr_div) : 0;
    lv.nr_mid = middle ? 1u : 0u; lv.nr_fshift = 24 - sub_bits; lv.nr_fmask = (1u << (24 - sub_bits)) - 1u;
    lv.nr_f24 = ((uint64_t)subsz << (24 - sub_bits)) <= (1ull << 32) && subsz < (1u << 24) ? 1u : 0u;
    lv.spb = 1;
    return lv;
}
inline LevelCfg level_flat_to_coarse(const PartCfg& cfg) {
    LevelCfg lv; lv.n_regions = cfg.n_regions; lv.n_seg = 1; lv.nb = cfg.n_coarse; lv.seg_shift = 32; lv.out_shift = cfg.g_shift; lv.in_raw = 0; lv.k = 0; lv.narrow = 0; lv.top8 = 0;
    lv.nr_shift = lv.nr_rps = lv.nr_sub = lv.nr_inv = 0; lv.nr_div = 1;
    lv.nr_mid = 0; lv.nr_fshift = 24; lv.nr_fmask = 0xFFFFFFu; lv.nr_f24 = 0;
    lv.spb = 1;
    return lv;
}

struct SetLayout { bool has_aux; size_t aux_off , base_off, total; };
inline SetLayout set_bytes(uint64_t n_max, int fmt, uint64_t R) {
    const size_t rec = (fmt == FMT_NARROW || fmt == FMT_TIGHT) ? 4 : 8;
    SetLayout l;
    l.has_aux = fmt == FMT_NARROW || fmt == FMT_WIDE;
    l.aux_off = ((size_t)n_max * rec + 63) & ~(size_t)63;
    l.base_off = l.aux_off + (l.has_aux ? ((size_t)n_max + 63) & ~(size_t)63 : 0);
    l.total = (l.base_off + (size_t)(R + 2) * 8 + 255) & ~(size_t)255;
    return l;
}
inline size_t arena_want(size_t need, size_t arena_bytes, bool was_full, int64_t pend_budget) {
    if (need > arena_bytes) return pend_budget > 0 ? (size_t)pend_budget : std::max<size_t>(4 * need, (size_t)64 << 20);
    return was_full && pend_budget < 0 ? 2 * arena_bytes : arena_bytes;
}
constexpr size_t ARENA_STAY = ~(size_t)0;
inline size_t arena_budget(size_t want, size_t need, size_t arena_bytes, int64_t pend_budget, size_t free_b, size_t total_b, size_t table_bytes) {
    size_t budget = want;
    const size_t avail = free_b + arena_bytes, reserve = std::max<size_t>(total_b / 8, (size_t)8 << 30);
    const size_t ceiling = avail > 2 * reserve ? avail - reserve : avail / 2;
    if (pend_budget < 0) budget = std::min<size_t>(want, std::min<size_t>(ceiling, std::max<size_t>(4 * need, 4 * table_bytes)));
    if (budget <= arena_bytes && need <= arena_bytes) return 0;
    return budget < need ? ARENA_STAY : budget;
}

inline void aligned_view(const char* d, const uint8_t** ab, uint64_t* lead) {
    uintptr_t p = (uintptr_t)d;
    *lead = p & 15;
    *ab = (const uint8_t*)(p - *lead);
}
struct SliceView { const uint8_t* ab; const uint16_t* pinv; uint64_t lead, len; EmitRange er; };
inline SliceView slice_view(const char* d_bases, const uint16_t* d_inv, uint64_t len, int k, uint64_t a, uint64_t b) {
    const uint64_t sub_off = a ? a - 1 : 0;
    SliceView v;
    v.len = std::min(len, b + k) - sub_off;
    v.er = EmitRange{a - sub_off, b - sub_off};
    v.pinv = nullptr;
    if (d_inv) { v.ab = (const uint8_t*)(reinterpret_cast<const uint32_t*>(d_bases) + sub_off / 16); v.pinv = d_inv + sub_off / 16; v.lead = sub_off % 16; }
    else aligned_view(d_bases + sub_off, &v.ab, &v.lead);
    return v;
}
inline uint64_t slice_at_cap(uint64_t kmers, uint64_t slice_kmers, uint64_t n_slots, uint64_t cap) {
    const uint64_t slice = std::min<uint64_t>(cap, std::max<uint64_t>(slice_kmers, n_slots / 4));
    const uint64_t n_slices = (kmers + slice - 1) / slice;
    return (kmers + n_slices - 1) / n_slices;
}
inline bool slice_reads_free(uint64_t kmers, uint64_t slice_kmers, bool slice_user, int64_t pend_budget, uint64_t n_slots) {
    if (slice_user || kmers <= slice_kmers) return false;
    return pend_budget != 0 ? slice_at_cap(kmers, slice_kmers, n_slots, 1ull << 31) > (1ull << 30) : 2 * n_slots > slice_kmers;
}
inline uint64_t choose_slice(uint64_t kmers, uint64_t slice_kmers, bool slice_user, int64_t pend_budget, uint64_t n_slots, size_t free_b, size_t work_bytes, bool have_mem_info) {
    if (slice_user || kmers <= slice_kmers) return slice_kmers;
    if (pend_budget != 0) {
        const uint64_t large = slice_at_cap(kmers, slice_kmers, n_slots, 1ull << 31);
        if (large <= (1ull << 30) || (have_mem_info && free_b + work_bytes >= (size_t)11 * large + ((size_t)2 << 30))) return large;
        return slice_at_cap(kmers, slice_kmers, n_slots, 1ull << 30);
    }
    if (2 * n_slots <= slice_kmers || !have_mem_info) return slice_kmers;
    const uint64_t by_mem = (uint64_t)((free_b + work_bytes) / 24);
    return std::max(slice_kmers, std::min<uint64_t>(std::min<uint64_t>(2 * n_slots, 1ull << 31), by_mem));
}
inline bool slices_fork(int overlap, bool profile, int count_path, uint64_t kmers, uint64_t slice, bool whole_table) {
    return overlap && !profile && count_path != 1 && (kmers + slice - 1) / slice >= 2 && slice >= (1u << 20) && (overlap == 2 || whole_table);
}
inline bool slice_partitions(uint64_t n, bool table_ok, uint64_t table_bytes, uint64_t n_regions, int64_t pend_budget, uint64_t pend_records, bool have_arena, size_t arena_bytes) {
    double pass_records = (double)n;
    if (pend_budget != 0) {
        const double per_set = (double)set_bytes(n, FMT_PACK8, n_regions).total;
        const double room = have_arena ? (double)arena_bytes : 4.0 * (double)table_bytes;
        pass_records = (double)pend_records + (double)n * std::max(1.0, std::min(8.0, room / per_set));
    }
    return n >= (1u << 20) && table_ok && (double)table_bytes <= 200.0 * pass_records;
}
inline bool lookup_partitions(bool per_base, int lookup_path, bool table_ok, uint64_t kmers, uint64_t slice_kmers, uint64_t table_bytes) {
    return !per_base && lookup_path != 1 && table_ok &&
           (lookup_path == 2 || (kmers >= (1u << 20) && (double)table_bytes <= 64.0 * (double)std::min<uint64_t>(kmers, slice_kmers)));
}

inline uint32_t part_first_bucket(int p, int n_parts) { return (uint32_t)(((uint64_t)p * 256 + n_parts - 1) / n_parts); }
inline uint32_t owner_sub_bits(int n_parts) {
    uint32_t sb = 0;
    while (((uint32_t)n_parts << (sb + 1)) <= 256u && sb < 5) ++sb;
    return sb;
}

}
```

### kreeq_amd/csrc/kq_select_host.h

```cpp
#pragma once
#include "kq_formats.h"

namespace kq {

constexpr int KS_P1_ROUND2 = 1,
              KS_LV_NARROW_S = 2,
              KS_LV_TIGHT_UNITS = 4,
              KS_P3_SET_OFFSETS = 16,
              KS_SEG_NEVER = 32,
              KS_SEG_ALWAYS = 64,
              KS_P1_NO_COMPACT = 128,
              KS_ALL = KS_P1_ROUND2 | KS_LV_NARROW_S | KS_LV_TIGHT_UNITS | KS_P3_SET_OFFSETS | KS_SEG_NEVER | KS_SEG_ALWAYS | KS_P1_NO_COMPACT;

enum Kernel { K_P1_HIST, K_P1_SCATTER, K_P1_SCATTER_S, K_P1_SCATTER_C, K_LV_HIST, K_LV_SCATTER, K_LV_SCATTER_S, K_LV_SEGMENT_S, K_LV_UNITS ,
              K_COUNT_REGIONS, K_COUNT_REGIONS_Q4, K_COUNT_REGIONS_Q4R, K_LOOKUP_REGIONS };
struct KernelSel {
    Kernel fam; int fmt = 0, nbc = 0, bin = 0, kc = 0, tpr = 0; bool flag = false;
    bool operator==(const KernelSel& o) const { return fam == o.fam && fmt == o.fmt && nbc == o.nbc && bin == o.bin && kc == o.kc && tpr == o.tpr && flag == o.flag; }
};
inline KernelSel sel_of(Kernel fam, int fmt, int nbc, int bin, int kc, int tpr = 0, bool flag = false) { KernelSel s{fam}; s.fmt = fmt; s.nbc = nbc; s.bin = bin; s.kc = kc; s.tpr = tpr; s.flag = flag; return s; }

struct P1Case { bool plain, owner_plain, narrow_filt, narrow_win; };
inline P1Case p1_case(int k, uint32_t mode, uint32_t narrow, uint32_t map_mask, bool full_range, bool windowed) {
    const bool plain = mode == 0 && full_range;
    return P1Case{plain, mode == 1 && map_mask != 0 && full_range, mode == 0 && narrow && !plain && map_mask != 0 && k <= (int)NARROW_MAX_K,
                  plain && narrow && (k <= (int)NARROW_MAX_K || k > PART_MAX_K) && windowed};
}
inline KernelSel select_p1_hist(int k, uint32_t mode, uint32_t narrow, uint32_t map_mask, bool full_range, bool windowed) {
    const P1Case c = p1_case(k, mode, narrow, map_mask, full_range, windowed);
    const int bin = c.owner_plain ? 3 : c.narrow_filt ? 4 : c.narrow_win ? 6 : !c.plain ? 0 : narrow ? 2 : 1;
    return sel_of(K_P1_HIST, 0, 0, bin, bin == 0 ? 0 : bin == 1 ? (k == 31 ? 31 : 0) : bin == 6 && k == 31 ? 31 : k == 21 ? 21 : 0);
}
inline KernelSel select_p1_hist_cached(int k, int pass_bin) { return sel_of(K_P1_HIST, 0, 0, pass_bin == 4 ? 5 : 2, k == 21 ? 21 : 0); }
inline KernelSel select_p1_scatter(int k, uint32_t mode, uint32_t narrow, uint32_t map_mask, bool full_range, bool windowed, bool lockstep,
                                   uint32_t n_coarse, int tpr, int kernel_set) {
    const P1Case c = p1_case(k, mode, narrow, map_mask, full_range, windowed);
    const bool small = n_coarse < 512;
    const int nbc = small ? 512 : NB_MAX, kc21 = k == 21 ? 21 : 0, kc31 = k == 31 ? 31 : 0;
    if (narrow) {
        const bool top8 = k > PART_MAX_K;
        int bin, kc, t = 1;
        if (top8) { bin = c.narrow_win ? 6 : c.plain ? 2 : 0; kc = bin ? kc31 : 0; }
        else if (c.narrow_filt) { bin = 4; kc = kc21; }
        else if (c.narrow_win) { bin = 6; kc = kc21; }
        else if (c.plain) { bin = 2; kc = kc21; t = tpr; }
        else { bin = 0; kc = 0; }
        if (kernel_set & KS_P1_ROUND2) return sel_of(K_P1_SCATTER, top8 ? FMT_TOP8 : FMT_NARROW, 512, bin, kc);
        if (bin == 4 && !(kernel_set & KS_P1_NO_COMPACT)) return sel_of(K_P1_SCATTER_C, 0, 0, 0, kc);
        return sel_of(K_P1_SCATTER_S, 0, 0, bin, kc, t, top8);
    }
    if (lockstep) return c.plain && k == 31 ? sel_of(K_P1_SCATTER, FMT_WIDE, nbc, 1, 31)  : sel_of(K_P1_SCATTER, FMT_WIDE, nbc, 0, 0);
    if (c.owner_plain && small) return sel_of(K_P1_SCATTER, FMT_PACK8, 512, 3, kc21);
    return sel_of(K_P1_SCATTER, FMT_PACK8, nbc, c.plain ? 1 : 0, 0);
}

inline int level_format(uint32_t lv_narrow, bool lockstep) { return lv_narrow == 2 ? FMT_TOP8 : lv_narrow ? FMT_NARROW : lockstep ? FMT_WIDE : FMT_PACK8; }
inline KernelSel select_level_hist(uint32_t lv_narrow, bool lockstep) { return sel_of(K_LV_HIST, level_format(lv_narrow, lockstep), 0, 0, 0); }
inline KernelSel select_level_scatter(uint32_t lv_narrow, bool lockstep, bool lv_top8, uint32_t nb, bool rstart, int kernel_set) {
    const int fmt = level_format(lv_narrow, lockstep), nbc = nb < 512 ? 512 : NB_MAX;
    if (lv_top8) return sel_of(K_LV_SCATTER, FMT_PACK8_TO_NARROW, 512, 0, 0);
    if (fmt == FMT_NARROW && nb < 512 && (rstart ? !(kernel_set & KS_LV_TIGHT_UNITS) : (kernel_set & KS_LV_NARROW_S) != 0)) return sel_of(K_LV_SCATTER_S, 0, 0, 0, 0, 0, rstart);
    return sel_of(K_LV_SCATTER, fmt == FMT_NARROW && rstart ? FMT_NARROW_TO_TIGHT : fmt, nbc, 0, 0);
}
inline KernelSel select_last_level(int plan_fmt, uint32_t lv_narrow, bool rstart, uint32_t nr_shift, uint32_t nb, uint32_t spb, bool even_buckets, int kernel_set) {
    const bool ok = plan_fmt == FMT_NARROW && lv_narrow == 1 && rstart && nr_shift != 0 && nb < 512 && spb == 1;
    return sel_of(ok && ((kernel_set & KS_SEG_ALWAYS) || (even_buckets && !(kernel_set & KS_SEG_NEVER))) ? K_LV_SEGMENT_S : K_LV_UNITS, 0, 0, 0, 0);
}

inline bool table_pass_wants_matrix(int fmt, int kernel_set) { return (fmt == FMT_TIGHT || fmt == FMT_NARROW) && !(kernel_set & KS_P3_SET_OFFSETS); }
inline KernelSel select_table_pass(int fmt, int k, bool matrix) {
    if (fmt == FMT_TIGHT || fmt == FMT_NARROW) return sel_of(matrix ? K_COUNT_REGIONS_Q4R : K_COUNT_REGIONS_Q4, 0, 0, 0, k == 21 ? 21 : 0, 0, fmt == FMT_TIGHT);
    return sel_of(K_COUNT_REGIONS, fmt, 0, 0, 0);
}
inline KernelSel select_hot_pass(int fmt) { return sel_of(K_COUNT_REGIONS, fmt == FMT_TIGHT ? FMT_NARROW : fmt, 0, 0, 0, 0, true); }
inline KernelSel select_lookup(int fmt) { return sel_of(K_LOOKUP_REGIONS, fmt, 0, 0, 0); }

}
```

### kreeq_amd/csrc/kreeq_amd.hip

```cpp
#include <hip/hip_runtime.h>
#include <hipcub/hipcub.hpp>

#include <algorithm>
#include <cstdarg>
#include <cstdio>
#include <cstdlib>
#include <cstring>
#include <mutex>
#include <new>
#include <numeric>
#include <string>
#include <thread>
#include <type_traits>
#include <vector>

#include "../../include/kreeq_amd.h"
#include "kq_device.h"
#include "kq_partition.h"
#include "kq_mem_host.h"
#include "kq_plan_host.h"
#include "kq_roff_host.h"
#include "kq_seg_gate_host.h"
#include "kq_select_host.h"
#include "kq_bgzf_host.h"

using namespace kq;

#include "kq_kernels.h"
#include "kq_fastx.h"
#include "kq_bgzf.h"
#include "kq_deflate.h"
#include "kq_dbimage.h"
#include "kq_subgraph.h"
#include "kq_gfa.h"
#include "kq_variants.h"
#include "kq_table.h"


static thread_local std::string g_err;
static int fail(int code, const char* fmt, ...) {
    char buf[512];
    va_list ap; va_start(ap, fmt); vsnprintf(buf, sizeof buf, fmt, ap); va_end(ap);
    g_err = buf;
    return code;
}
#define HIPC(expr)                                                                                   \
    do {                                                                                             \
        hipError_t e_ = (expr);                                                                      \
        if (e_ != hipSuccess)                                                                        \
            return fail(e_ == hipErrorOutOfMemory ? KQ_ERR_NOMEM : KQ_ERR_HIP, "%s: %s (%s:%d)", #expr, \
                        hipGetErrorString(e_), __FILE__, __LINE__);                                  \
    } while (0)

struct Scrambled {
    void* p = nullptr; size_t bytes = 0, chunk = 0;
    std::vector<hipMemGenericAllocationHandle_t> hs;
    bool vmm = false;

    Scrambled() = default;
    Scrambled(const Scrambled&) = delete;
    Scrambled& operator=(const Scrambled&) = delete;
    Scrambled(Scrambled&& o) noexcept { swap(o); }
    Scrambled& operator=(Scrambled&& o) noexcept { if (this != &o) { reset(); swap(o); } return *this; }
    ~Scrambled() { reset(); }
    void swap(Scrambled& o) noexcept { std::swap(p, o.p); std::swap(bytes, o.bytes); std::swap(chunk, o.chunk); hs.swap(o.hs); std::swap(vmm, o.vmm); }
    friend void swap(Scrambled& a, Scrambled& b) noexcept { a.swap(b); }

    void reset() {
        if (!p) return;
        (void)hipDeviceSynchronize();
        if (vmm) {
            (void)hipMemUnmap(p, hs.size() * chunk);
            for (auto& hnd : hs) (void)hipMemRelease(hnd);
            (void)hipMemAddressFree(p, hs.size() * chunk);
        } else (void)hipFree(p);
        p = nullptr; bytes = chunk = 0; hs.clear(); vmm = false;
    }
    bool alloc(size_t n, int device, bool try_vmm) {
        reset();
        if (try_vmm && map_chunks(n, device)) return true;
        if (hipMalloc(&p, n) != hipSuccess) { (void)hipGetLastError(); p = nullptr; return false; }
        bytes = n; vmm = false;
        return true;
    }
private:
    bool map_chunks(size_t n_bytes, int device) {
        static const size_t chunk_mb = getenv("KQ_SCRAMBLE_MB") ? (size_t)atoi(getenv("KQ_SCRAMBLE_MB")) : 2;
        if (!chunk_mb) return false;
        hipMemAllocationProp prop = {};
        prop.type = hipMemAllocationTypePinned; prop.location.type = hipMemLocationTypeDevice; prop.location.id = device;
        size_t gran = 0;
        if (hipMemGetAllocationGranularity(&gran, &prop, hipMemAllocationGranularityMinimum) != hipSuccess || !gran) { (void)hipGetLastError(); return false; }
        const size_t ck = ((chunk_mb << 20) + gran - 1) / gran * gran, n = (n_bytes + ck - 1) / ck;
        void* base = nullptr;
        if (hipMemAddressReserve(&base, n * ck, 0, nullptr, 0) != hipSuccess) { (void)hipGetLastError(); return false; }
        std::vector<hipMemGenericAllocationHandle_t> fresh;
        fresh.reserve(n);
        bool ok = true;
        for (size_t i = 0; i < n && ok; ++i) { hipMemGenericAllocationHandle_t hnd; ok = hipMemCreate(&hnd, ck, &prop, 0) == hipSuccess; if (ok) fresh.push_back(hnd); }
        size_t mapped = 0;
        if (ok) {
            size_t mul = 7919;
            while (std::gcd(mul, n) != 1) ++mul;
            for (; mapped < n && ok; ++mapped) ok = hipMemMap((char*)base + mapped * ck, ck, 0, fresh[(mapped * mul + 13) % n], 0) == hipSuccess;
            if (!ok) --mapped;
        }
        if (ok) {
            hipMemAccessDesc acc = {};
            acc.location = prop.location; acc.flags = hipMemAccessFlagsProtReadWrite;
            ok = hipMemSetAccess(base, n * ck, &acc, 1) == hipSuccess;
        }
        if (!ok) {
            (void)hipGetLastError();
            if (mapped) (void)hipMemUnmap(base, mapped * ck);
            for (auto& hnd : fresh) (void)hipMemRelease(hnd);
            (void)hipMemAddressFree(base, n * ck);
            return false;
        }
        p = base; bytes = n * ck; chunk = ck; hs.swap(fresh); vmm = true;
        return true;
    }
};
static int scr_ensure(Scrambled& b, size_t need, int device) {
    if (b.bytes >= need) return KQ_OK;
    b.reset();
    const size_t sz = need + std::min<size_t>(need / 4, (size_t)256 << 20) + 4096;
    if (!b.alloc(sz, device, true)) return fail(KQ_ERR_NOMEM, "partition scratch allocation failed");
    return KQ_OK;
}

struct ScratchSet { DevMem part; Scrambled part2; };

struct kq_handle {
    int device = 0, k = 0, map_count = 0;
    Stream own_stream;
    hipStream_t stream = nullptr;
    int n_cu = 256;
    DevMem slots;
    uint64_t n_regions = 0;
    uint32_t win_lo = 0, win_hi = 256;
    bool windowed = false;
    DevMem hc;
    uint64_t hc_cap = 0;
    DevMem rstart;
    DevMem st;
    PinnedMem st_host;
    DevMem scratch;
    DevMem stage;
    uint64_t kmers_bound = 0;
    uint64_t used_bound = 0;
    uint64_t hc_check_at = 0;
    bool table_empty = true;
    uint32_t mid_rps = 2048;
    int merge_path = 0;
    int lookup_path = 0;
    bool slots_dirty = false;
    bool trust_capacity = false;
    int count_path = 0;
    uint64_t slice_kmers = 1ull << 28;
    bool slice_user = false;
    uint32_t filt_lo = 0, filt_hi = 0;
    bool profile = false;
    std::vector<std::pair<const char*, Event>> marks;
    ScratchSet work, fork_work;
    hipStream_t base = nullptr;
    Stream fork_stream[2];
    bool fork_busy[2] = {false, false};
    static constexpr int EV_RING = 64;
    Event ev_ring[EV_RING];
    uint64_t ev_next = 0;
    int overlap = 1;
    int kernel_set = 0;
    struct HistKey { const void* ab; const void* pinv; uint64_t lead, len, er_lo, er_hi; uint32_t g1, n_rng; int k;
                     bool operator==(const HistKey& o) const { return ab == o.ab && pinv == o.pinv && lead == o.lead && len == o.len && er_lo == o.er_lo && er_hi == o.er_hi && g1 == o.g1 && n_rng == o.n_rng && k == o.k; } };
    struct HistEntry { HistKey key; DevMem m1_all; };
    std::vector<HistEntry> hist_cache;
    size_t hist_cache_bytes = 0;
    int map_passes = 1;
    Scrambled arena;
    size_t arena_bytes = 0, arena_used = 0;
    DevMem d_sets;
    P3Set pend_sets[P3_MAX_SETS] = {};
    DevMem tot;
    DevMem roff;
    int n_pend = 0, pend_fmt = -1, pend_aux_fmt = 0;
    uint64_t pend_records = 0;
    int64_t pend_budget = -1;
    uint64_t table_passes = 0;
    static constexpr int IN_SLOTS = 3, IN_TICKETS = 512;
    Stream copy_stream;
    DevMem in_buf[IN_SLOTS];
    Event in_consumed[IN_SLOTS];
    std::vector<Event> in_copied;
    uint64_t in_next = 0;
    std::mutex in_m;
    uint8_t in_bad[IN_TICKETS] = {};
    DevMem fx_units, fx_out, in_cmp[IN_SLOTS];
    DevMem fx_res;
    PinnedMem fx_res_host;
    int fx_bad = 0;
    DevMem bz_desc, bz_stat, bz_text, bz_carry;
    PinnedMem bz_desc_host, bz_stat_host;
    DevMem df_slots, df_sizes, df_offs, df_stat, df_in, df_out;
    PinnedMem df_stat_host;
    uint64_t bz_carry_len = 0;
    bool bz_bad = false;
    std::string bz_err;
    bool hist_cache_off = false;
    bool test_fail_plan = false;
    DevMem hot;
    uint64_t var_batch = 0;
    uint64_t sg_batch = 0;
    std::vector<DevMem> user_mem;
    DevMem tab_segs;

    TableView view() const {
        TableView v; v.slots = slots.as<Slot>() - (reg_lo() << REGION_SHIFT); v.n_regions = n_regions; v.hc = hc.as<HcSlot>(); v.hc_mask = hc_cap - 1; v.st = d_state(); v.k = (uint32_t)k;
        v.reg_lo = reg_lo(); v.reg_hi = reg_hi();
        v.rps = k >= HI_K ? (uint32_t)(n_regions >> 8) : 0u;
        v.rstart = rstart.as<uint32_t>();
        return v;
    }
    DevState* d_state() const { return st.as<DevState>(); }
    DevState* host_state() const { return st_host.as<DevState>(); }
    FxResult* fx_host() const { return fx_res_host.as<FxResult>(); }
    uint64_t reg_lo() const { return windowed ? (uint64_t)win_lo * (n_regions >> 8) : 0; }
    uint64_t reg_hi() const { return windowed ? (uint64_t)win_hi * (n_regions >> 8) : n_regions; }
    uint64_t n_alloc_regions() const { return reg_hi() - reg_lo(); }
    uint64_t n_slots() const { return n_alloc_regions() << REGION_SHIFT; }
    uint64_t table_bytes() const { return n_slots() * sizeof(Slot); }
    TableShape shape() const { return TableShape{k, n_regions, map_count, mid_rps}; }
};

static void marks_reset(kq_handle* h);
static int flush_pending(kq_handle* h);

static int ev_get(kq_handle* h, hipEvent_t* out) {
    Event& e = h->ev_ring[h->ev_next++ % kq_handle::EV_RING];
    if (!e) HIPC(e.create(hipEventDisableTiming));
    else HIPC(hipEventSynchronize(e.get()));
    *out = e.get();
    return KQ_OK;
}
static int join_forks(kq_handle* h) {
    for (int w = 0; w < 2; ++w) {
        if (!h->fork_busy[w]) continue;
        hipEvent_t e; int rc = ev_get(h, &e); if (rc) return rc;
        HIPC(hipEventRecord(e, h->fork_stream[w].get()));
        HIPC(hipStreamWaitEvent(h->base, e, 0));
        h->fork_busy[w] = false;
    }
    return KQ_OK;
}

static int grid_for(const kq_handle* h, uint64_t work_items, int per_block, int per_cu = 8) {
    uint64_t blocks = (work_items + per_block - 1) / per_block;
    uint64_t cap = (uint64_t)h->n_cu * per_cu;
    if (blocks > cap) blocks = cap;
    if (blocks < 1) blocks = 1;
    return (int)blocks;
}

static void clear_words(kq_handle* h, void* p, uint32_t words_per_slot, uint64_t n_slots) {
    const uint64_t n_pairs = n_slots * words_per_slot / 2;
    hipLaunchKernelGGL(k_clear_slots, dim3(grid_for(h, n_pairs, 256)), dim3(256), 0, h->stream, (ulonglong2*)p, words_per_slot, n_pairs);
}
static void clear_main(kq_handle* h, Slot* p, uint64_t n_slots) { (void)hipMemsetAsync(p, 0, (size_t)n_slots * sizeof(Slot), h->stream); }
static void materialize(kq_handle* h) {
    if (!h->slots_dirty) return;
    clear_main(h, h->slots.as<Slot>(), h->n_slots());
    h->slots_dirty = false;
}
static int alloc_main(kq_handle* h, uint64_t n_regions, uint64_t alloc_regions, DevMem& slots, DevMem& rstart) {
    HIPC(slots.alloc((size_t)(alloc_regions << REGION_SHIFT) * sizeof(Slot)));
    if (rstart.alloc((size_t)(n_regions + 1) * sizeof(uint32_t)) != hipSuccess) { slots.reset(); return fail(KQ_ERR_NOMEM, "region index allocation failed"); }
    clear_main(h, slots.as<Slot>(), alloc_regions << REGION_SHIFT);
    hipLaunchKernelGGL(k_region_starts, dim3(grid_for(h, n_regions + 1, 256)), dim3(256), 0, h->stream, rstart.as<uint32_t>(), n_regions);
    return KQ_OK;
}
static int alloc_hc(kq_handle* h, uint64_t cap, DevMem& hc) {
    HIPC(hc.alloc((size_t)cap * sizeof(HcSlot)));
    clear_words(h, hc.get(), sizeof(HcSlot) / 8, cap);
    return KQ_OK;
}

static int read_state_raw(kq_handle* h) {
    HIPC(hipMemcpyAsync(h->host_state(), h->d_state(), sizeof(DevState), hipMemcpyDeviceToHost, h->stream));
    HIPC(hipStreamSynchronize(h->stream));
    return KQ_OK;
}
static int read_state(kq_handle* h) {
    int frc = flush_pending(h);
    if (frc) return frc;
    return read_state_raw(h);
}
static int check_errors(kq_handle* h) {
    int rc = read_state(h);
    if (rc) return rc;
    if (h->host_state()->err_table_full) return fail(KQ_ERR_TABLE_FULL, "k-mer table region overflow (slots %llu / %llu)",
                                                 (unsigned long long)h->host_state()->slots_used, (unsigned long long)h->n_slots());
    if (h->host_state()->err_hc_full) return fail(KQ_ERR_TABLE_FULL, "high-copy side table overflow (%llu / %llu)",
                                              (unsigned long long)h->host_state()->hc_used, (unsigned long long)h->hc_cap);
    return KQ_OK;
}

static int grow_main(kq_handle* h, uint64_t need_slots) {
    int frc = flush_pending(h);
    if (frc) return frc;
    const GrowTarget grown = grow_target(h->n_slots(), h->n_regions, need_slots);
    const uint64_t want = grown.slots, new_regions = grown.regions;
    if (!grown.ok) return fail(KQ_ERR_TABLE_FULL, "cannot grow k-mer table to %llu slots: region index overflow", (unsigned long long)want);
    DevMem slots, rstart;
    int rc = alloc_main(h, new_regions, want >> REGION_SHIFT, slots, rstart);
    if (rc) return rc == KQ_ERR_NOMEM ? fail(KQ_ERR_TABLE_FULL, "cannot grow k-mer table to %llu slots: out of device memory",
                                             (unsigned long long)want) : rc;
    const uint64_t n_old = h->n_slots();
    const TableView old_view = h->view();
    slots.swap(h->slots); rstart.swap(h->rstart);
    h->n_regions = new_regions;
    if (h->slots_dirty) h->slots_dirty = false;
    else hipLaunchKernelGGL(k_rehash, dim3(grid_for(h, n_old, 256)), dim3(256), 0, h->stream, h->view(), old_view);
    HIPC(hipStreamSynchronize(h->stream));
    return KQ_OK;
}
static int grow_hc(kq_handle* h, uint64_t need) {
    uint64_t want = h->hc_cap;
    while (want < need) want *= 2;
    DevMem hc;
    int rc = alloc_hc(h, want, hc);
    if (rc) return rc;
    const uint64_t n_old = h->hc_cap;
    hc.swap(h->hc); h->hc_cap = want;
    HIPC(hipMemsetAsync(&h->d_state()->hc_used, 0, sizeof(unsigned long long), h->stream));
    hipLaunchKernelGGL(k_rehash_hc, dim3(grid_for(h, n_old, 256)), dim3(256), 0, h->stream, h->view(), hc.as<HcSlot>(), n_old);
    HIPC(hipStreamSynchronize(h->stream));
    return KQ_OK;
}

static int reserve(kq_handle* h, uint64_t extra, uint64_t extra_instances) {
    int rc;
    bool state_read = false;
    if (!h->trust_capacity) {
        uint64_t need = main_need(h->used_bound, extra);
        if (need > h->n_slots()) {
            rc = read_state(h); if (rc) return rc;
            state_read = true;
            h->used_bound = h->host_state()->slots_used;
            need = main_need(h->used_bound, extra);
            if (need > h->n_slots()) { rc = grow_main(h, need); if (rc) return rc; }
        }
    }
    h->used_bound += extra;
    h->kmers_bound += extra_instances;
    uint64_t need_hc = hc_need(h->kmers_bound);
    if (hc_follows_fill(h->kmers_bound) && h->kmers_bound >= h->hc_check_at && h->n_pend == 0) {
        if (!state_read) { rc = read_state_raw(h); if (rc) return rc; }
        need_hc = hc_need(h->kmers_bound, h->host_state()->hc_used);
        h->hc_check_at = 2 * h->kmers_bound;
    }
    if (need_hc > h->hc_cap) { rc = grow_hc(h, need_hc); if (rc) return rc; }
    return KQ_OK;
}

static int stage_in(kq_handle* h, const void* host, size_t bytes, void** dev) {
    HIPC(h->stage.ensure(bytes + 64));
    if (bytes) HIPC(hipMemcpyAsync(h->stage.get(), host, bytes, hipMemcpyHostToDevice, h->stream));
    *dev = h->stage.get();
    return KQ_OK;
}

static void parallel_sort_entries(kq_entry* a, uint64_t n) {
    auto less = [](const kq_entry& x, const kq_entry& y) { return x.key < y.key; };
    unsigned hw = std::thread::hardware_concurrency();
    unsigned t = std::max(1u, std::min(16u, hw ? hw : 1u));
    while (t > 1 && n / t < (1u << 16)) t /= 2;
    if (t <= 1) { std::sort(a, a + n, less); return; }
    std::vector<uint64_t> cut(t + 1);
    for (unsigned i = 0; i <= t; ++i) cut[i] = n * i / t;
    {
        std::vector<std::thread> th;
        for (unsigned i = 0; i < t; ++i) th.emplace_back([&, i] { std::sort(a + cut[i], a + cut[i + 1], less); });
        for (auto& x : th) x.join();
    }
    for (unsigned width = 1; width < t; width *= 2) {
        std::vector<std::thread> th;
        for (unsigned i = 0; i + width < t; i += 2 * width) {
            const uint64_t lo = cut[i], mid = cut[i + width], hi = cut[std::min(i + 2 * width, t)];
            th.emplace_back([=] { std::inplace_merge(a + lo, a + mid, a + hi, less); });
        }
        for (auto& x : th) x.join();
    }
}

template <class Fn> struct KernelRow { KernelSel sel; Fn fn; };
template <class Fn, size_t N, class... A>
static int launch_row(const KernelRow<Fn> (&rows)[N], const char* family, const KernelSel& s, kq_handle* h, dim3 grid, dim3 block, A... args) {
    for (const KernelRow<Fn>& r : rows) if (r.sel == s) { hipLaunchKernelGGL(r.fn, grid, block, 0, h->stream, args...); return KQ_OK; }
    return fail(KQ_ERR_INVALID, "%s has no instantiation <fmt %d, nbc %d, bin %d, kc %d, tpr %d, flag %d> (selector family %d)", family, s.fmt, s.nbc, s.bin, s.kc, s.tpr, (int)s.flag, (int)s.fam);
}
template <int B, int K> static KernelRow<decltype(&k_p1_hist<0, 0>)> p1h() { return {sel_of(K_P1_HIST, 0, 0, B, K), k_p1_hist<B, K>}; }
template <int W, int N, int B, int K> static KernelRow<decltype(&k_p1_scatter<0, 512, 0, 0>)> p1w() { return {sel_of(K_P1_SCATTER, W, N, B, K), k_p1_scatter<W, N, B, K>}; }
template <int B, int K, int T, bool TOP8 = false> static KernelRow<decltype(&k_p1_scatter_s<0, 0, 1>)> p1s() { return {sel_of(K_P1_SCATTER_S, 0, 0, B, K, T, TOP8), k_p1_scatter_s<B, K, T, TOP8>}; }
template <int K> static KernelRow<decltype(&k_p1_scatter_c<0>)> p1c() { return {sel_of(K_P1_SCATTER_C, 0, 0, 0, K), k_p1_scatter_c<K>}; }
template <int W> static KernelRow<decltype(&k_lv_hist<0>)> lvh() { return {sel_of(K_LV_HIST, W, 0, 0, 0), k_lv_hist<W>}; }
template <int W, int N> static KernelRow<decltype(&k_lv_scatter<0, 512>)> lvw() { return {sel_of(K_LV_SCATTER, W, N, 0, 0), k_lv_scatter<W, N>}; }
template <bool T> static KernelRow<decltype(&k_lv_scatter_s<false>)> lvs() { return {sel_of(K_LV_SCATTER_S, 0, 0, 0, 0, 0, T), k_lv_scatter_s<T>}; }
template <int W, bool HOT> static KernelRow<decltype(&k_count_regions<0, false>)> p3g() { return {sel_of(K_COUNT_REGIONS, W, 0, 0, 0, 0, HOT), k_count_regions<W, HOT>}; }
template <int K, bool T> static KernelRow<decltype(&k_count_regions_q4<0, false>)> p3q() { return {sel_of(K_COUNT_REGIONS_Q4, 0, 0, 0, K, 0, T), k_count_regions_q4<K, T>}; }
template <int K, bool T> static KernelRow<decltype(&k_count_regions_q4r<0, false>)> p3r() { return {sel_of(K_COUNT_REGIONS_Q4R, 0, 0, 0, K, 0, T), k_count_regions_q4r<K, T>}; }
template <int W> static KernelRow<decltype(&k_lookup_regions<0>)> lkr() { return {sel_of(K_LOOKUP_REGIONS, W, 0, 0, 0), k_lookup_regions<W>}; }

extern "C" {

const char* kq_last_error(void) { return g_err.c_str(); }
int kq_abi_version(void) { return KQ_ABI_VERSION; }

int kq_device_available(void) {
    int n = 0;
    if (hipGetDeviceCount(&n) != hipSuccess || n <= 0) return 0;
    hipDeviceProp_t p;
    if (hipGetDeviceProperties(&p, 0) != hipSuccess) return 0;
    return strncmp(p.gcnArchName, "gfx950", 6) == 0 ? 1 : 0;
}

int kq_device_memory(int device, uint64_t* free_bytes, uint64_t* total_bytes) {
    if (!free_bytes || !total_bytes) return fail(KQ_ERR_INVALID, "null argument");
    int n = 0;
    if (hipGetDeviceCount(&n) != hipSuccess || n <= 0) return fail(KQ_ERR_NO_DEVICE, "no HIP device visible (this library has no CPU path)");
    if (device < 0 || device >= n) return fail(KQ_ERR_NO_DEVICE, "device %d out of range (%d visible)", device, n);
    HIPC(hipSetDevice(device));
    size_t f = 0, t = 0;
    HIPC(hipMemGetInfo(&f, &t));
    *free_bytes = f; *total_bytes = t;
    return KQ_OK;
}

static int set_window(kq_handle* h, uint32_t lo, uint32_t hi, bool shard = false) {
    if (lo >= hi || hi > 256) return fail(KQ_ERR_INVALID, "bucket window [%u, %u) is not a range of the 256 hash-prefix buckets", lo, hi);
    if (shard && h->k > (int)NARROW_MAX_K && h->k < HI_K)
        return fail(KQ_ERR_INVALID, "shard windows need k <= %u (5-byte records) or k >= %d (8-byte hash-remainder records); k = %u..%d shards own map ranges", NARROW_MAX_K, HI_K, NARROW_MAX_K + 1, HI_K - 1);
    if (!shard && h->k > (int)NARROW_MAX_K) return fail(KQ_ERR_INVALID, "bucket windows need k <= %u (5-byte records)", NARROW_MAX_K);
    if (!h->table_empty || h->n_pend || h->kmers_bound) return fail(KQ_ERR_INVALID, "the bucket window is chosen before anything is counted");
    if (h->windowed && hi - lo == h->win_hi - h->win_lo && !(lo == 0 && hi == 256)) {
        HIPC(hipStreamSynchronize(h->stream));
        h->win_lo = lo; h->win_hi = hi;
        return KQ_OK;
    }
    const WindowGeom g = window_geometry(h->n_alloc_regions(), lo, hi, h->k);
    if (!g.ok) return fail(KQ_ERR_INVALID, "bucket window too narrow for a table of %llu regions", (unsigned long long)h->n_alloc_regions());
    HIPC(hipStreamSynchronize(h->stream));
    DevMem slots, rstart;
    int rc = alloc_main(h, g.virt, g.alloc_new, slots, rstart);
    if (rc) return rc;
    HIPC(hipStreamSynchronize(h->stream));
    slots.swap(h->slots); rstart.swap(h->rstart);
    h->n_regions = g.virt; h->win_lo = lo; h->win_hi = hi; h->windowed = !(lo == 0 && hi == 256);
    h->slots_dirty = false;
    return KQ_OK;
}

int kq_create(kq_handle** out, int device, int k, int map_count, uint64_t capacity_hint) {
    if (!out) return fail(KQ_ERR_INVALID, "out is null");
    *out = nullptr;
    if (k < 2 || k > 32) return fail(KQ_ERR_INVALID, "k must be in 2..32 (got %d)", k);
    if (map_count < 1 || map_count > 65535) return fail(KQ_ERR_INVALID, "map_count must be in 1..65535 (got %d)", map_count);
    int n = 0;
    if (hipGetDeviceCount(&n) != hipSuccess || n <= 0) return fail(KQ_ERR_NO_DEVICE, "no HIP device visible (this library has no CPU path)");
    if (device < 0 || device >= n) return fail(KQ_ERR_NO_DEVICE, "device %d out of range (%d visible)", device, n);
    HIPC(hipSetDevice(device));
    hipDeviceProp_t prop;
    HIPC(hipGetDeviceProperties(&prop, device));
    if (strncmp(prop.gcnArchName, "gfx950", 6) != 0)
        return fail(KQ_ERR_NO_DEVICE, "device %d is %s; this library carries gfx950 code only", device, prop.gcnArchName);
    kq_handle* h = new (std::nothrow) kq_handle();
    if (!h) return fail(KQ_ERR_NOMEM, "host allocation failed");
    h->device = device; h->k = k; h->map_count = map_count; h->n_cu = prop.multiProcessorCount;
    h->filt_hi = (uint32_t)map_count;
    hipError_t e = h->own_stream.create(hipStreamNonBlocking);
    if (e != hipSuccess) { delete h; return fail(KQ_ERR_HIP, "hipStreamCreate: %s", hipGetErrorString(e)); }
    h->stream = h->base = h->own_stream.get();
    int rc = KQ_OK;
    do {
        if (h->st.alloc(sizeof(DevState)) != hipSuccess || h->st_host.alloc(sizeof(DevState)) != hipSuccess) {
            rc = fail(KQ_ERR_NOMEM, "state allocation failed"); break;
        }
        (void)hipMemsetAsync(h->d_state(), 0, sizeof(DevState), h->stream);
        const uint64_t regions = initial_regions(capacity_hint, k);
        rc = alloc_main(h, regions, regions, h->slots, h->rstart); if (rc) break;
        h->n_regions = regions;
        uint64_t hc = 1u << 16;
        rc = alloc_hc(h, hc, h->hc); if (rc) break;
        h->hc_cap = hc;
        if (hipStreamSynchronize(h->stream) != hipSuccess) { rc = fail(KQ_ERR_HIP, "table initialisation failed"); break; }
    } while (0);
    if (rc) { kq_destroy(h); return rc; }
    *out = h;
    return KQ_OK;
}

void kq_destroy(kq_handle* h) {
    if (!h) return;
    (void)hipSetDevice(h->device);
    if (h->stream) (void)hipStreamSynchronize(h->stream);
    for (auto& s : h->fork_stream) if (s) (void)hipStreamSynchronize(s.get());
    if (h->copy_stream) (void)hipStreamSynchronize(h->copy_stream.get());
    delete h;
}

int kq_clear(kq_handle* h) {
    if (!h) return fail(KQ_ERR_INVALID, "null handle");
    HIPC(hipSetDevice(h->device));
    h->slots_dirty = true;
    clear_words(h, h->hc.get(), sizeof(HcSlot) / 8, h->hc_cap);
    HIPC(hipMemsetAsync(h->d_state(), 0, sizeof(DevState), h->stream));
    h->kmers_bound = 0;
    h->used_bound = 0;
    h->hc_check_at = 0;
    h->table_empty = true;
    h->n_pend = 0; h->arena_used = 0; h->pend_records = 0;
    h->fx_bad = 0;
    h->bz_bad = false; h->bz_carry_len = 0;
    return KQ_OK;
}

int kq_set_stream(kq_handle* h, void* s) {
    if (!h) return fail(KQ_ERR_INVALID, "null handle");
    HIPC(hipStreamSynchronize(h->stream));
    h->stream = h->base = s ? (hipStream_t)s : h->own_stream.get();
    return KQ_OK;
}
int kq_set_option(kq_handle* h, int option, int64_t value) {
    if (!h) return fail(KQ_ERR_INVALID, "null handle");
    switch (option) {
        case KQ_OPT_TRUST_CAPACITY: h->trust_capacity = value != 0; return KQ_OK;
        case KQ_OPT_COUNT_PATH:
            if (value < 0 || value > 2) return fail(KQ_ERR_INVALID, "KQ_OPT_COUNT_PATH must be 0, 1 or 2");
            h->count_path = (int)value; return KQ_OK;
        case KQ_OPT_COUNT_MAP_RANGE: {
            const int64_t lo = value & 0xFFFF, hi = (value >> 16) & 0xFFFF;
            if (lo >= hi || hi > h->map_count) return fail(KQ_ERR_INVALID, "map range [%lld,%lld) outside [0,%d]", (long long)lo, (long long)hi, h->map_count);
            h->filt_lo = (uint32_t)lo; h->filt_hi = (uint32_t)hi; return KQ_OK;
        }
        case KQ_OPT_NARROW_MID:
            if (value < 2 || value > (1 << 14)) return fail(KQ_ERR_INVALID, "KQ_OPT_NARROW_MID must be in [2, 16384]");
            h->mid_rps = (uint32_t)value; return KQ_OK;
        case KQ_OPT_MERGE_PATH:
            if (value < 0 || value > 2) return fail(KQ_ERR_INVALID, "KQ_OPT_MERGE_PATH must be 0, 1 or 2");
            h->merge_path = (int)value; return KQ_OK;
        case KQ_OPT_LOOKUP_PATH:
            if (value < 0 || value > 2) return fail(KQ_ERR_INVALID, "KQ_OPT_LOOKUP_PATH must be 0, 1 or 2");
            h->lookup_path = (int)value; return KQ_OK;
        case KQ_OPT_PROFILE: h->profile = value != 0; if (!h->profile) marks_reset(h); return KQ_OK;
        case KQ_OPT_TEST_FAIL_PLAN: h->test_fail_plan = value != 0; return KQ_OK;
        case KQ_OPT_COUNT_MAP_PASSES: {
            if (value != 1 && value != 2 && value != 4 && value != 8) return fail(KQ_ERR_INVALID, "KQ_OPT_COUNT_MAP_PASSES must be 1, 2, 4 or 8");
            if ((h->map_count & (h->map_count - 1)) != 0 || value > h->map_count) return fail(KQ_ERR_INVALID, "KQ_OPT_COUNT_MAP_PASSES needs a power-of-two map count");
            HIPC(hipStreamSynchronize(h->stream));
            h->hist_cache.clear(); h->hist_cache_bytes = 0;
            h->map_passes = (int)value; return KQ_OK;
        }
        case KQ_OPT_KERNEL_SET:
            if (value < 0 || (value & ~(int64_t)KS_ALL)) return fail(KQ_ERR_INVALID, "KQ_OPT_KERNEL_SET is a mask of bits 1, 2, 4, 16, 32, 64, 128");
            h->kernel_set = (int)value; return KQ_OK;
        case KQ_OPT_OVERLAP:
            if (value < 0 || value > 2) return fail(KQ_ERR_INVALID, "KQ_OPT_OVERLAP must be 0, 1 or 2");
            h->overlap = (int)value; return KQ_OK;
        case KQ_OPT_PENDING_BYTES: {
            if (value < -1) return fail(KQ_ERR_INVALID, "KQ_OPT_PENDING_BYTES must be -1 (auto), 0 (off) or a byte count");
            int rc = flush_pending(h);
            if (rc) return rc;
            if (h->arena.p && value != h->pend_budget) { HIPC(hipStreamSynchronize(h->stream)); h->arena.reset(); h->arena_bytes = 0; }
            h->pend_budget = value; return KQ_OK;
        }
        case KQ_OPT_BUCKET_WINDOW:
            HIPC(hipSetDevice(h->device));
            return set_window(h, (uint32_t)(value & 0xFFFF), (uint32_t)((value >> 16) & 0xFFFF));
        case KQ_OPT_SHARD_WINDOW:
            HIPC(hipSetDevice(h->device));
            return set_window(h, (uint32_t)(value & 0xFFFF), (uint32_t)((value >> 16) & 0xFFFF), true);
        case KQ_OPT_SLICE_KMERS:
            if (value < 1) return fail(KQ_ERR_INVALID, "KQ_OPT_SLICE_KMERS must be positive");
            h->slice_kmers = (uint64_t)value; h->slice_user = true; return KQ_OK;
        case KQ_OPT_SUBGRAPH_BATCH:
            if (value < 0) return fail(KQ_ERR_INVALID, "KQ_OPT_SUBGRAPH_BATCH must be 0 (automatic) or a number of searches");
            h->sg_batch = (uint64_t)value; return KQ_OK;
        case KQ_OPT_VARIANT_BATCH:
            if (value < 0) return fail(KQ_ERR_INVALID, "KQ_OPT_VARIANT_BATCH must be 0 (automatic) or a number of searches");
            h->var_batch = (uint64_t)value; return KQ_OK;
        default: return fail(KQ_ERR_INVALID, "unknown option %d", option);
    }
}
int kq_get_profile(kq_handle* h, char* buf, uint64_t cap) {
    if (!h || !buf || !cap) return fail(KQ_ERR_INVALID, "null argument");
    HIPC(hipSetDevice(h->device));
    HIPC(hipStreamSynchronize(h->stream));
    std::string out;
    for (size_t i = 1; i < h->marks.size(); ++i) {
        float ms = 0;
        HIPC(hipEventElapsedTime(&ms, h->marks[i - 1].second.get(), h->marks[i].second.get()));
        char tmp[96];
        snprintf(tmp, sizeof tmp, "%s%s=%.4f", out.empty() ? "" : ";", h->marks[i].first, ms);
        out += tmp;
    }
    if (out.size() + 1 > cap) return fail(KQ_ERR_CAPACITY, "profile buffer too small: need %zu", out.size() + 1);
    memcpy(buf, out.c_str(), out.size() + 1);
    return KQ_OK;
}
void* kq_get_stream(kq_handle* h) { return h ? (void*)h->stream : nullptr; }
int kq_sync(kq_handle* h) {
    if (!h) return fail(KQ_ERR_INVALID, "null handle");
    HIPC(hipSetDevice(h->device));
    HIPC(hipStreamSynchronize(h->stream));
    const int rc = check_errors(h);
    if (h->bz_bad) return fail(KQ_ERR_INVALID, "%s: submitted for counting and skipped (kq_clear resets this)", h->bz_err.c_str());
    if (h->fx_bad) return fail(KQ_ERR_INVALID, "malformed %s text was submitted for counting and skipped (kq_clear resets this)", h->fx_bad == KQ_FASTX_FASTQ ? "FASTQ" : "FASTA");
    return rc;
}
int kq_flush(kq_handle* h) {
    if (!h) return fail(KQ_ERR_INVALID, "null handle");
    HIPC(hipSetDevice(h->device));
    return flush_pending(h);
}
int kq_get_info(kq_handle* h, kq_info* out) {
    if (!h || !out) return fail(KQ_ERR_INVALID, "null argument");
    HIPC(hipSetDevice(h->device));
    int rc = read_state(h);
    if (rc) return rc;
    out->kmers_counted = h->host_state()->kmers_added;
    out->slots_used = h->host_state()->slots_used;
    out->slots_total = h->n_slots();
    out->hc_used = h->host_state()->hc_used;
    out->hc_total = h->hc_cap;
    out->table_bytes = h->n_slots() * sizeof(Slot) + h->hc_cap * sizeof(HcSlot);
    out->table_passes = h->table_passes;
    return KQ_OK;
}

struct PartPlan : PlanSizes {
    bool even_buckets = false;
    uint64_t *recs1, *recs2;
    uint8_t *aux1, *aux2;
    unsigned long long *m1, *seg_off, *unit_base, *group_base, *sums, *total, *hot;
    uint32_t* m2;
    uint8_t* a1() const { return fmt == FMT_WIDE || fmt == FMT_NARROW ? aux1 : nullptr; }
    uint8_t* a2() const { return fmt == FMT_WIDE || fmt == FMT_NARROW ? aux2 : nullptr; }
};
static int plan_alloc(kq_handle* h, PartPlan* p, uint64_t n_max, uint64_t n_tiles, uint32_t p1_bins, bool allow_narrow = false,
                      uint64_t min_segs = 0 ) {
    if (h->test_fail_plan) { h->test_fail_plan = false; return fail(KQ_ERR_NOMEM, "partition scratch allocation failed (injected by KQ_OPT_TEST_FAIL_PLAN)"); }
    if (n_max >= (1ull << 32) - 16) return fail(KQ_ERR_INVALID, "a partition pass handles fewer than 2^32 records (got %llu): slice the input", (unsigned long long)n_max);
    static_cast<PlanSizes&>(*p) = plan_sizes(h->shape(), h->n_cu, n_max, n_tiles, p1_bins, allow_narrow, min_segs);
    const PlanLayout at = plan_layout(*p);
    if (p->split2) { int rc2 = scr_ensure(h->work.part2, at.part2_bytes, h->device); if (rc2) return rc2; }
    HIPC(h->work.part.ensure((size_t)at.words * 8));
    uint64_t* const base = h->work.part.as<uint64_t>();
    uint64_t* const base2 = p->split2 ? (uint64_t*)h->work.part2.p : base;
    p->recs1 = base + at.recs1; p->aux1 = (uint8_t*)(base + at.aux1);
    p->recs2 = base2 + at.recs2; p->aux2 = (uint8_t*)(base2 + at.aux2);
    p->m1 = (unsigned long long*)(base + at.m1);
    p->seg_off = (unsigned long long*)(base + at.seg_off);
    p->unit_base = (unsigned long long*)(base + at.unit_base);
    p->group_base = (unsigned long long*)(base + at.group_base);
    p->sums = (unsigned long long*)(base + at.sums);
    p->total = (unsigned long long*)(base + at.total);
    p->hot = (unsigned long long*)(base + at.hot);
    p->m2 = (uint32_t*)(base + at.m2);
    return KQ_OK;
}
static void scan_u64(kq_handle* h, unsigned long long* a, uint64_t n, unsigned long long* sums_scratch, unsigned long long* total) {
    if (n <= 2 * SCAN_CHUNK) {
        hipLaunchKernelGGL(k_exclusive_scan, dim3(1), dim3(1024), 0, h->stream, a, n, total);
        return;
    }
    const uint64_t chunks = (n + SCAN_CHUNK - 1) / SCAN_CHUNK;
    hipLaunchKernelGGL(k_scan_sums, dim3((unsigned)chunks), dim3(1024), 0, h->stream, a, n, sums_scratch);
    hipLaunchKernelGGL(k_exclusive_scan, dim3(1), dim3(1024), 0, h->stream, sums_scratch, chunks, total);
    hipLaunchKernelGGL(k_scan_apply, dim3((unsigned)chunks), dim3(1024), 0, h->stream, a, n, sums_scratch);
}
static void mark(kq_handle* h, const char* name) {
    if (!h->profile) return;
    Event e;
    if (e.create(hipEventDefault) != hipSuccess) return;
    (void)hipEventRecord(e.get(), h->stream);
    h->marks.emplace_back(name, std::move(e));
}
static void marks_reset(kq_handle* h) { h->marks.clear(); }

struct P1Scan { const uint8_t* ab; uint64_t lead, len; EmitRange er; const uint16_t* pinv; };
static int launch_p1_hist(kq_handle* h, const KernelSel& s, uint32_t grid, const P1Scan& in, const PartCfg& cfg, uint32_t g1, unsigned long long* m1) {
    static const KernelRow<decltype(&k_p1_hist<0, 0>)> rows[] = {p1h<6, 21>(), p1h<6, 31>(), p1h<6, 0>(), p1h<2, 21>(), p1h<2, 0>(), p1h<1, 31>(), p1h<1, 0>(),
                                                                  p1h<3, 21>(), p1h<3, 0>(), p1h<4, 21>(), p1h<4, 0>(), p1h<0, 0>(), p1h<5, 21>(), p1h<5, 0>()};
    return launch_row(rows, "k_p1_hist", s, h, dim3(grid), dim3(TILE_THREADS), in.ab, in.lead, in.len, h->k, cfg, in.er, g1, m1, in.pinv);
}
static int launch_p1_scatter(kq_handle* h, const KernelSel& s, uint32_t grid, const P1Scan& in, const PartCfg& cfg, const unsigned long long* m1, uint64_t* out, uint8_t* out_aux, int aux_fmt) {
    static const KernelRow<decltype(&k_p1_scatter<0, 512, 0, 0>)> wide[] = {
        p1w<FMT_TOP8, 512, 6, 31>(), p1w<FMT_TOP8, 512, 6, 0>(), p1w<FMT_TOP8, 512, 2, 31>(), p1w<FMT_TOP8, 512, 2, 0>(), p1w<FMT_TOP8, 512, 0, 0>(),
        p1w<FMT_NARROW, 512, 4, 21>(), p1w<FMT_NARROW, 512, 4, 0>(), p1w<FMT_NARROW, 512, 6, 21>(), p1w<FMT_NARROW, 512, 6, 0>(), p1w<FMT_NARROW, 512, 2, 21>(), p1w<FMT_NARROW, 512, 2, 0>(), p1w<FMT_NARROW, 512, 0, 0>(),
        p1w<FMT_WIDE, 512, 1, 31>(), p1w<FMT_WIDE, NB_MAX, 1, 31>(), p1w<FMT_WIDE, 512, 0, 0>(), p1w<FMT_WIDE, NB_MAX, 0, 0>(),
        p1w<FMT_PACK8, 512, 3, 21>(), p1w<FMT_PACK8, 512, 3, 0>(), p1w<FMT_PACK8, 512, 1, 0>(), p1w<FMT_PACK8, NB_MAX, 1, 0>(), p1w<FMT_PACK8, 512, 0, 0>(), p1w<FMT_PACK8, NB_MAX, 0, 0>()};
    static const KernelRow<decltype(&k_p1_scatter_s<0, 0, 1>)> streamed[] = {
        p1s<4, 21, 1>(), p1s<4, 0, 1>(), p1s<6, 21, 1>(), p1s<6, 0, 1>(), p1s<2, 21, KQ_P1S_TPR>(), p1s<2, 0, KQ_P1S_TPR>(), p1s<0, 0, 1>(),
        p1s<6, 31, 1, true>(), p1s<6, 0, 1, true>(), p1s<2, 31, 1, true>(), p1s<2, 0, 1, true>(), p1s<0, 0, 1, true>()};
    static const KernelRow<decltype(&k_p1_scatter_c<0>)> compact[] = {p1c<21>(), p1c<0>()};
    if (s.fam == K_P1_SCATTER_S) return launch_row(streamed, "k_p1_scatter_s", s, h, dim3(grid), dim3(TILE_THREADS * s.tpr), in.ab, in.lead, in.len, h->k, cfg, in.er, m1, (uint32_t*)out, out_aux, in.pinv);
    if (s.fam == K_P1_SCATTER_C) return launch_row(compact, "k_p1_scatter_c", s, h, dim3(grid), dim3(TILE_THREADS), in.ab, in.lead, in.len, h->k, cfg, in.er, m1, (uint32_t*)out, out_aux, in.pinv);
    return launch_row(wide, "k_p1_scatter", s, h, dim3(grid), dim3(TILE_THREADS), in.ab, in.lead, in.len, h->k, cfg, in.er, m1, out, out_aux, aux_fmt, in.pinv);
}

static int run_p1(kq_handle* h, PartPlan* p, const PartCfg& cfg, const uint8_t* ab, uint64_t lead, uint64_t len, EmitRange er, uint64_t* out,
                  uint8_t* out_aux, int aux_fmt, const uint16_t* pinv = nullptr ) {
    const P1Scan in{ab, lead, len, er, pinv};
    const bool full_range = cfg.filt_lo == 0 && cfg.filt_hi == cfg.map_count, windowed = cfg.win_lo != 0 || cfg.win_hi != (1u << NARROW_CBITS);
    const KernelSel hist = select_p1_hist(h->k, cfg.mode, cfg.narrow, cfg.map_mask, full_range, windowed);
    const bool narrow_filt = hist.bin == 4, narrow_win = hist.bin == 6;
    int rc = KQ_OK;
    auto cached_hist = [&](const kq_handle::HistKey& key, size_t bytes, const PartCfg& all) -> kq_handle::HistEntry* {
        for (auto& e : h->hist_cache) if (e.key == key) return &e;
        if (h->hist_cache_bytes + bytes > ((size_t)4 << 30)) return nullptr;
        DevMem buf;
        if (buf.alloc(bytes) != hipSuccess) { (void)hipGetLastError(); return nullptr; }
        rc = launch_p1_hist(h, select_p1_hist_cached(h->k, hist.bin), p->g1, in, all, p->g1, buf.as<unsigned long long>());
        if (rc) return nullptr;
        h->hist_cache.push_back(kq_handle::HistEntry{key, std::move(buf)});
        h->hist_cache_bytes += bytes;
        return &h->hist_cache.back();
    };
    bool have_hist = false;
    const size_t row = (size_t)p->g1 * sizeof(unsigned long long), block = row << NARROW_CBITS;
    if (narrow_filt && h->map_passes > 1 && P1_F == 1 && !h->hist_cache_off) {
        const uint32_t n = (uint32_t)h->map_passes, per = cfg.map_count / n, rr = cfg.filt_lo / per;
        if (cfg.filt_lo == rr * per && cfg.filt_hi == (rr + 1) * per) {
            PartCfg all = cfg;
            all.n_rng = n; all.n_coarse = n << NARROW_CBITS;
            if (const auto* ent = cached_hist({ab, pinv, lead, len, er.lo, er.hi, p->g1, n, h->k}, n * block, all)) {
                (void)hipMemcpyAsync(p->m1, ent->m1_all.as<char>() + rr * block, block, hipMemcpyDeviceToDevice, h->stream);
                have_hist = true;
            }
        }
    }
    if (narrow_win && h->map_passes > 1 && P1_F == 1 && !h->hist_cache_off) {
        PartCfg all = cfg;
        all.win_lo = 0; all.win_hi = 1u << NARROW_CBITS;
        if (const auto* ent = cached_hist({ab, pinv, lead, len, er.lo, er.hi, p->g1, 0xB0C4E7u, h->k}, block, all)) {
            (void)hipMemcpyAsync(p->m1, ent->m1_all.get(), block, hipMemcpyDeviceToDevice, h->stream);
            if (cfg.win_lo) (void)hipMemsetAsync(p->m1, 0, (size_t)cfg.win_lo * row, h->stream);
            if (cfg.win_hi < (1u << NARROW_CBITS)) (void)hipMemsetAsync((char*)p->m1 + (size_t)cfg.win_hi * row, 0, (size_t)((1u << NARROW_CBITS) - cfg.win_hi) * row, h->stream);
            have_hist = true;
        }
    }
    if (!rc && !have_hist) rc = launch_p1_hist(h, hist, p->g1 * P1_F, in, cfg, p->g1, p->m1);
    if (rc) return rc;
    scan_u64(h, p->m1, (uint64_t)cfg.n_coarse * p->g1 * P1_F, p->sums, p->total);
    hipLaunchKernelGGL(k_p1_offsets, dim3((cfg.n_coarse + 256) / 256), dim3(256), 0, h->stream, p->m1, p->total, cfg, p->g1, p->seg_off);
    mark(h, "k_p1_hist+scan");
    rc = launch_p1_scatter(h, select_p1_scatter(h->k, cfg.mode, cfg.narrow, cfg.map_mask, full_range, windowed, out_aux != nullptr, cfg.n_coarse, KQ_P1S_TPR, h->kernel_set), p->g1, in, cfg, p->m1, out, out_aux, aux_fmt);
    mark(h, "k_p1_scatter");
    return rc;
}
struct LevelIn { const uint64_t* recs; const uint8_t* aux; const unsigned long long *seg_lo, *seg_hi; uint32_t n_seg, spb; };
static LevelIn own_segments(const PartPlan& p, const uint64_t* recs, const uint8_t* aux, uint32_t n_seg) { return LevelIn{recs, aux, p.seg_off, p.seg_off + 1, n_seg, 1}; }
struct LevelUnits { const uint64_t* in; const uint8_t* in_aux; LevelCfg lv; const unsigned long long *seg_lo, *seg_hi, *unit_base; uint32_t* m2; unsigned grid; };
static int launch_level_hist(kq_handle* h, const KernelSel& s, const LevelUnits& u) {
    static const KernelRow<decltype(&k_lv_hist<0>)> rows[] = {lvh<FMT_TOP8>(), lvh<FMT_NARROW>(), lvh<FMT_WIDE>(), lvh<FMT_PACK8>()};
    return launch_row(rows, "k_lv_hist", s, h, dim3(u.grid), dim3(MS_THREADS), u.in, u.in_aux, u.lv, u.seg_lo, u.seg_hi, u.unit_base, u.m2);
}
static int launch_level_scatter(kq_handle* h, const KernelSel& s, const LevelUnits& u, const unsigned long long* gb, uint64_t* out, uint8_t* out_aux) {
    static const KernelRow<decltype(&k_lv_scatter<0, 512>)> rows[] = {
        lvw<FMT_PACK8_TO_NARROW, 512>(), lvw<FMT_TOP8, 512>(), lvw<FMT_TOP8, NB_MAX>(), lvw<FMT_NARROW_TO_TIGHT, 512>(), lvw<FMT_NARROW_TO_TIGHT, NB_MAX>(),
        lvw<FMT_NARROW, 512>(), lvw<FMT_NARROW, NB_MAX>(), lvw<FMT_WIDE, 512>(), lvw<FMT_WIDE, NB_MAX>(), lvw<FMT_PACK8, 512>(), lvw<FMT_PACK8, NB_MAX>()};
    static const KernelRow<decltype(&k_lv_scatter_s<false>)> streamed[] = {lvs<true>(), lvs<false>()};
    if (s.fam == K_LV_SCATTER_S) return launch_row(streamed, "k_lv_scatter_s", s, h, dim3(u.grid), dim3(LV_THREADS), (const uint32_t*)u.in, u.in_aux, u.lv, u.seg_lo, u.seg_hi, u.unit_base, u.m2, gb, (uint32_t*)out, out_aux);
    return launch_row(rows, "k_lv_scatter", s, h, dim3(u.grid), dim3(LV_THREADS), u.in, u.in_aux, u.lv, u.seg_lo, u.seg_hi, u.unit_base, u.m2, gb, out, out_aux);
}
static int run_level(kq_handle* h, PartPlan* p, const LevelCfg& lv, const LevelIn& src, uint64_t* out, uint8_t* out_aux,
                     unsigned long long* gb = nullptr ) {
    if (!gb) gb = p->group_base;
    const LevelCfg lv_ = with_rep_shift(lv);
    const uint64_t groups = (uint64_t)(lv.n_seg / lv.spb) * lv.nb;
    hipLaunchKernelGGL(k_lv_units, dim3(1), dim3(1024), 0, h->stream, src.seg_lo, src.seg_hi, lv_, p->unit_base);
    const LevelUnits u{src.recs, src.aux, lv_, src.seg_lo, src.seg_hi, p->unit_base, p->m2, (unsigned)std::min<uint64_t>(p->n_max / P2_UNIT + lv.n_seg + 1, 1u << 30)};
    int rc = launch_level_hist(h, select_level_hist(lv.narrow, src.aux != nullptr), u);
    if (rc) return rc;
    if (p->n_max / P2_UNIT + 1 <= 8 * (uint64_t)(lv.n_seg / lv.spb))
        hipLaunchKernelGGL(k_lv_offsets_thread, dim3((unsigned)((groups + 255) / 256)), dim3(256), 0, h->stream, p->m2, lv_, p->unit_base, gb);
    else
        hipLaunchKernelGGL(k_lv_offsets, dim3((unsigned)((groups * 64 + 255) / 256)), dim3(256), 0, h->stream, p->m2, lv_, p->unit_base, gb);
    (void)hipMemsetAsync(gb + groups, 0, 8, h->stream);
    scan_u64(h, gb, groups + 1, p->sums, p->total + 1);
    mark(h, "k_lv_hist+offsets+scan");
    rc = launch_level_scatter(h, select_level_scatter(lv.narrow, src.aux != nullptr, lv.top8 != 0, lv.nb, lv.rstart != nullptr, h->kernel_set), u, gb, out, out_aux);
    mark(h, "k_lv_scatter");
    return rc;
}
static void run_segment_level(kq_handle* h, PartPlan* p, const LevelCfg& lv, const uint64_t* in, const uint8_t* in_aux, uint64_t* out, unsigned long long* gb) {
    mark(h, "segment_level");
    mark(h, "k_lv_hist+offsets+scan");
    hipLaunchKernelGGL(k_lv_segment_s, dim3(lv.n_seg), dim3(LV_THREADS), 0, h->stream, (const uint32_t*)in, in_aux, with_rep_shift(lv), p->seg_off, gb, (uint32_t*)out);
    mark(h, "k_lv_scatter");
}
__global__ void k_p3set(P3Set* sets, int i, P3Set v) { sets[i] = v; }

struct Dest {
    int fmt, aux_fmt;
    bool tight = false;
    uint64_t* recs = nullptr; uint8_t* aux = nullptr; unsigned long long* base = nullptr; uint64_t n_max = 0;
    bool in_arena() const { return recs != nullptr; }
};
static int arena_take(kq_handle* h, uint64_t n_max, uint64_t R, Dest* d) {
    if (h->pend_budget == 0) return KQ_OK;
    const int fmt = d->fmt;
    const SetLayout lay = set_bytes(n_max, fmt, R);
    const size_t need = lay.total;
    bool was_full = false;
    if (h->n_pend && (h->n_pend >= P3_MAX_SETS || h->pend_fmt != fmt || h->arena_used + need > h->arena_bytes)) {
        was_full = h->pend_fmt == fmt && h->n_pend < P3_MAX_SETS;
        int rc = flush_pending(h);
        if (rc) return rc;
    }
    const size_t want = arena_want(need, h->arena_bytes, was_full, h->pend_budget);
    if (want > h->arena_bytes) {
        size_t free_b = 0, total_b = 0;
        if (hipMemGetInfo(&free_b, &total_b) != hipSuccess) return KQ_OK;
        const size_t budget = arena_budget(want, need, h->arena_bytes, h->pend_budget, free_b, total_b, (size_t)h->table_bytes());
        if (budget == ARENA_STAY) return KQ_OK;
        if (budget) {
            if (h->arena.p) { HIPC(hipStreamSynchronize(h->stream)); HIPC(hipStreamSynchronize(h->base)); h->arena.reset(); h->arena_bytes = 0; }
            static const bool scramble_arena = !getenv("KQ_SCRAMBLE_ARENA") || atoi(getenv("KQ_SCRAMBLE_ARENA")) != 0;
            if (!h->arena.alloc(budget, h->device, scramble_arena && budget >= ((size_t)1 << 30))) return KQ_OK;
            h->arena_bytes = budget; h->arena_used = 0;
        }
    }
    uint8_t* set = (uint8_t*)h->arena.p + h->arena_used;
    d->recs = (uint64_t*)set;
    d->aux = lay.has_aux ? set + lay.aux_off : nullptr;
    d->base = (unsigned long long*)(set + lay.base_off);
    d->n_max = n_max;
    h->arena_used += need;
    return KQ_OK;
}
static int pend_add(kq_handle* h, const P3Set& set, int fmt, int aux_fmt) {
    if (h->n_pend && (h->n_pend >= P3_MAX_SETS || h->pend_fmt != fmt || h->pend_aux_fmt != aux_fmt)) {
        int rc = flush_pending(h);
        if (rc) return rc;
    }
    if (!h->d_sets) HIPC(h->d_sets.alloc(sizeof(P3Set) * P3_MAX_SETS));
    hipLaunchKernelGGL(k_p3set, dim3(1), dim3(1), 0, h->stream, h->d_sets.as<P3Set>(), h->n_pend, set);
    h->pend_sets[h->n_pend] = set;
    h->pend_fmt = fmt; h->pend_aux_fmt = aux_fmt;
    ++h->n_pend;
    h->pend_records += set.n_max;
    return KQ_OK;
}
static int flush_pending_base(kq_handle* h);
static int flush_pending(kq_handle* h) {
    if (!h->n_pend) return KQ_OK;
    hipStream_t work = h->stream;
    h->stream = h->base;
    int rc = join_forks(h);
    if (!rc) rc = flush_pending_base(h);
    if (!rc && h->fork_stream[0]) {
        hipEvent_t e; rc = ev_get(h, &e);
        if (!rc && hipEventRecord(e, h->base) != hipSuccess) rc = fail(KQ_ERR_HIP, "hipEventRecord failed");
        for (int w = 0; w < 2 && !rc; ++w) if (hipStreamWaitEvent(h->fork_stream[w].get(), e, 0) != hipSuccess) rc = fail(KQ_ERR_HIP, "hipStreamWaitEvent failed");
    }
    h->stream = work;
    return rc;
}
static_assert(ROFF_MAX_SETS == (uint32_t)P3_MAX_SETS, "the offset matrix has a column for every set of a pass");
static uint32_t* roff_take(kq_handle* h) {
    for (int i = 0; i < h->n_pend; ++i) if (h->pend_sets[i].n_max >> 32) return nullptr;
    const size_t need = roff_bytes(h->n_alloc_regions());
    if (!need || !roff_pitch((uint32_t)h->n_pend)) return nullptr;
    if (h->roff.bytes() < need && h->roff.alloc(need) != hipSuccess) { (void)hipGetLastError(); return nullptr; }
    return h->roff.as<uint32_t>();
}
static int launch_table_pass(kq_handle* h, const KernelSel& s, dim3 grid, const Q4SetsRow& rows, int empty, unsigned long long* hot, uint32_t rps) {
    static const KernelRow<decltype(&k_count_regions<0, false>)> generic[] = {p3g<FMT_TOP8, false>(), p3g<FMT_WIDE, false>(), p3g<FMT_PACK8, false>(), p3g<FMT_NARROW, true>(), p3g<FMT_TOP8, true>(), p3g<FMT_WIDE, true>(), p3g<FMT_PACK8, true>()};
    static const KernelRow<decltype(&k_count_regions_q4<0, false>)> compact[] = {p3q<21, true>(), p3q<0, true>(), p3q<21, false>(), p3q<0, false>()};
    static const KernelRow<decltype(&k_count_regions_q4r<0, false>)> matrix[] = {p3r<21, true>(), p3r<0, true>(), p3r<21, false>(), p3r<0, false>()};
    const P3Set* sets = h->d_sets.as<P3Set>();
    if (s.fam == K_COUNT_REGIONS_Q4R) return launch_row(matrix, "k_count_regions_q4r", s, h, grid, dim3(Q4_THREADS), h->view(), rows, empty, hot, rps);
    if (s.fam == K_COUNT_REGIONS_Q4) return launch_row(compact, "k_count_regions_q4", s, h, grid, dim3(Q4_THREADS), h->view(), sets, (uint32_t)h->n_pend, empty, hot, rps);
    return launch_row(generic, "k_count_regions", s, h, grid, dim3(P3_THREADS), h->view(), sets, (uint32_t)h->n_pend, h->pend_aux_fmt, empty, hot, rps);
}
static int flush_pending_base(kq_handle* h) {
    const uint64_t R = h->n_regions;
    HIPC(h->hot.ensure((size_t)(R + 2) * 8));
    int rc;
    if (hc_follows_fill(h->kmers_bound)) {
        rc = read_state_raw(h); if (rc) return rc;
        const uint64_t need_hc = hc_need(h->kmers_bound, h->host_state()->hc_used);
        if (need_hc > h->hc_cap) { rc = grow_hc(h, need_hc); if (rc) return rc; }
    }
    unsigned long long* hot = h->hot.as<unsigned long long>();
    HIPC(hipMemsetAsync(hot, 0, 8, h->stream));
    const dim3 grid((unsigned)std::min<uint64_t>(h->n_alloc_regions(), 1u << 30)), grid_hot(h->n_cu);
    const int empty = h->slots_dirty ? 2 : h->table_empty ? 1 : 0;
    const int fmt = h->pend_fmt;
    const uint32_t rps = (fmt == FMT_NARROW || fmt == FMT_TIGHT || fmt == FMT_TOP8) ? (uint32_t)(R >> NARROW_CBITS) : 1u;
    Q4SetsRow rows = {};
    if (table_pass_wants_matrix(fmt, h->kernel_set)) {
        if (uint32_t* roff = roff_take(h)) {
            rows.pitch = roff_pitch((uint32_t)h->n_pend);
            if (!h->tot) {
                const size_t tb = (size_t)TOT_LINES * 64;
                if (h->tot.alloc(tb) != hipSuccess) (void)hipGetLastError();
                else HIPC(hipMemsetAsync(h->tot.get(), 0, tb, h->stream));
            }
            rows.tot = h->tot.as<unsigned long long>();
            rows.roff = roff - h->reg_lo() * rows.pitch;
            for (int i = 0; i < h->n_pend; ++i) { rows.d[i].recs = (const uint32_t*)h->pend_sets[i].recs; rows.d[i].aux = h->pend_sets[i].aux; }
            const uint64_t n_rows = roff_rows(h->n_alloc_regions());
            hipLaunchKernelGGL(k_p3_region_offsets, dim3(grid_for(h, n_rows, ROFF_ROWS, 32)), dim3(ROFF_THREADS), 0, h->stream,
                               roff, h->d_sets.as<P3Set>(), (uint32_t)h->n_pend, rows.pitch, h->reg_lo(), n_rows);
        }
    }
    rc = launch_table_pass(h, select_table_pass(fmt, h->k, rows.roff != nullptr), grid, rows, empty, hot, rps);
    if (!rc) rc = launch_table_pass(h, select_hot_pass(fmt), grid_hot, rows, empty, hot, rps);
    if (rc) return rc;
    if (rows.roff && rows.tot) hipLaunchKernelGGL(k_fold_totals, dim3(1), dim3(256), 0, h->stream, rows.tot, h->d_state());
    h->n_pend = 0; h->arena_used = 0; h->pend_records = 0;
    ++h->table_passes;
    h->slots_dirty = false;
    h->table_empty = false;
    mark(h, "k_count_regions");
    HIPC(hipGetLastError());
    return KQ_OK;
}

static int dest_take(kq_handle* h, const PartPlan& p, uint64_t n_max, Dest* d) {
    d->tight = tight_ok(p.fmt, p.R, (bool)h->rstart);
    if (d->tight) { d->fmt = FMT_TIGHT; d->aux_fmt = AUX_TIGHT; }
    return arena_take(h, n_max, p.R, d);
}
static int sort_to_regions(kq_handle* h, PartPlan* p, const LevelIn& in, const Dest& d, P3Set* set) {
    const bool arena = d.in_arena();
    int rc = KQ_OK;
    uint64_t* fin = arena ? d.recs : p->recs2;
    uint8_t* fin_aux = arena ? d.aux : p->a2();
    unsigned long long* fin_base = arena ? d.base : p->group_base;
    if (p->fmt == FMT_NARROW || p->fmt == FMT_TOP8) {
        const uint32_t sb = p->cfg.sub_bits;
        const bool t8 = p->fmt == FMT_TOP8;
        const bool mid_to_2 = sb != 0 && in.recs == p->recs1;
        if (!arena && mid_to_2) { fin = p->recs1; fin_aux = p->a1(); }
        if (d.tight) fin_aux = nullptr;
        LevelCfg last = level_narrow(p->cfg, sb, false, t8);
        if (d.tight) last.rstart = h->rstart.as<uint32_t>();
        if (sb == 0) {
            last.n_seg = in.n_seg; last.spb = in.spb;
            rc = run_level(h, p, last, in, fin, fin_aux, fin_base);
        } else {
            LevelCfg mid = level_narrow(p->cfg, sb, true, t8);
            mid.n_seg = in.n_seg; mid.spb = in.spb;
            uint64_t* m = mid_to_2 ? p->recs2 : p->recs1;
            uint8_t* m_aux = mid_to_2 ? p->a2() : p->a1();
            rc = run_level(h, p, mid, in, m, m_aux);
            if (rc) return rc;
            (void)hipMemcpyAsync(p->seg_off, p->group_base, (size_t)(((1u << NARROW_CBITS) << sb) + 1) * 8, hipMemcpyDeviceToDevice, h->stream);
            if (select_last_level(p->fmt, last.narrow, last.rstart != nullptr, last.nr_shift, last.nb, last.spb, p->even_buckets, h->kernel_set).fam == K_LV_SEGMENT_S)
                run_segment_level(h, p, last, m, m_aux, fin, fin_base);
            else
                rc = run_level(h, p, last, own_segments(*p, m, m_aux, last.n_seg), fin, fin_aux, fin_base);
        }
    } else if (p->two_level) {
        rc = run_level(h, p, level_coarse_to_regions(p->cfg), in, fin, fin_aux, fin_base);
    } else {
        *set = P3Set{in.recs, in.aux, in.seg_lo, p->n_max};
        return KQ_OK;
    }
    *set = P3Set{fin, fin_aux, fin_base, arena ? d.n_max : p->n_max};
    return rc;
}

static int submit(kq_handle* h, const P3Set& set, const Dest& d) {
    HIPC(hipGetLastError());
    int rc = pend_add(h, set, d.fmt, d.aux_fmt);
    if (rc) return rc;
    return d.in_arena() ? KQ_OK : flush_pending(h);
}
static int sort_and_submit(kq_handle* h, PartPlan* p, const LevelIn& in, const Dest& d) {
    P3Set set; int rc = sort_to_regions(h, p, in, d, &set);
    return rc ? rc : submit(h, set, d);
}

static int plan_sequence(kq_handle* h, PartPlan* p, uint64_t lead, uint64_t len) {
    int rc = plan_alloc(h, p, len, n_tiles_of(lead, len), plan_cfg(h->shape(), true).n_coarse, true);
    if (rc) return rc;
    p->fmt = sequence_fmt(p->fmt, h->k);
    return KQ_OK;
}

static int count_partitioned(kq_handle* h, const uint8_t* ab, uint64_t lead, uint64_t len, EmitRange er, const uint16_t* pinv = nullptr) {
    PartPlan p;
    int rc = plan_sequence(h, &p, lead, len);
    if (rc) return rc;
    p.cfg.filt_lo = h->filt_lo; p.cfg.filt_hi = h->filt_hi;
    if (h->windowed) { p.cfg.win_lo = h->win_lo; p.cfg.win_hi = h->win_hi; }
    const bool leveled = p.fmt == FMT_NARROW || p.fmt == FMT_TOP8 || p.two_level;
    Dest dst{p.fmt, AUX_IDX6};
    const bool filtered = p.cfg.filt_lo != 0 || p.cfg.filt_hi != p.cfg.map_count || h->windowed;
    if (leveled && !filtered) { rc = dest_take(h, p, p.n_max, &dst); if (rc) return rc; }
    marks_reset(h);
    mark(h, "start");
    rc = run_p1(h, &p, p.cfg, ab, lead, len, er, p.recs1, p.a1(), AUX_IDX6, pinv);
    if (rc) return rc;
    if (leveled && filtered) {
        constexpr uint32_t NBK = 1u << NARROW_CBITS;
        const bool with_offsets = p.fmt == FMT_NARROW && p.cfg.sub_bits != 0 && p.cfg.n_coarse == NBK;
        unsigned long long offs[NBK + 1];
        unsigned long long n_recs = 0;
        if (with_offsets) HIPC(hipMemcpyAsync(offs, p.seg_off, sizeof offs, hipMemcpyDeviceToHost, h->stream));
        else HIPC(hipMemcpyAsync(&n_recs, p.total, sizeof n_recs, hipMemcpyDeviceToHost, h->stream));
        HIPC(hipStreamSynchronize(h->stream));
        if (with_offsets) { n_recs = offs[NBK]; p.even_buckets = kq::seg_gate_even(offs, NBK); }
        rc = dest_take(h, p, std::min<uint64_t>(p.n_max, ((uint64_t)n_recs + 15) & ~7ull), &dst); if (rc) return rc;
    }
    return sort_and_submit(h, &p, own_segments(p, p.recs1, p.a1(), p.cfg.n_coarse), dst);
}
static int count_partitioned_records(kq_handle* h, const uint64_t* d_recs, const uint8_t* d_aux, int aux_fmt, uint64_t n, bool raw) {
    PartPlan p;
    int rc = plan_alloc(h, &p, n, 0, 1, !d_aux && !raw);
    if (rc) return rc;
    if (d_aux) p.fmt = FMT_WIDE;
    Dest dst{p.fmt, aux_fmt};
    LevelCfg first = level_flat_to_coarse(p.cfg);
    if (p.fmt == FMT_NARROW) {
        rc = dest_take(h, p, p.n_max, &dst); if (rc) return rc;
        first.top8 = 1;
    } else {
        first.in_raw = raw ? 1 : 0; first.k = (uint32_t)h->k;
    }
    hipLaunchKernelGGL(k_set2, dim3(1), dim3(1), 0, h->stream, p.seg_off, 0ull, (unsigned long long)n);
    rc = run_level(h, &p, first, own_segments(p, d_recs, d_aux, 1), p.recs1, p.a1());
    if (rc) return rc;
    LevelIn coarse{p.recs1, p.a1(), p.group_base, p.group_base + 1, p.cfg.n_coarse, 1};
    if (p.two_level) {
        HIPC(hipMemcpyAsync(p.seg_off, p.group_base, (size_t)(p.cfg.n_coarse + 1) * 8, hipMemcpyDeviceToDevice, h->stream));
        coarse = own_segments(p, p.recs1, p.a1(), p.cfg.n_coarse);
    }
    return sort_and_submit(h, &p, coarse, dst);
}

static int count_seq_dev(kq_handle* h, const char* d_bases, const uint16_t* d_inv, uint64_t len) {
    if (!h || (!d_bases && len)) return fail(KQ_ERR_INVALID, "null argument");
    HIPC(hipSetDevice(h->device));
    if (len < (uint64_t)h->k) return KQ_OK;
    const uint64_t kmers = len - h->k + 1;
    size_t free_b = 0, total_b = 0;
    const bool have_mem_info = slice_reads_free(kmers, h->slice_kmers, h->slice_user, h->pend_budget, h->n_slots()) && hipMemGetInfo(&free_b, &total_b) == hipSuccess;
    const uint64_t slice = choose_slice(kmers, h->slice_kmers, h->slice_user, h->pend_budget, h->n_slots(), free_b, h->work.part.bytes(), have_mem_info);
    struct ForkGuard {
        kq_handle* h; bool swapped = false;
        void leave() { if (swapped) { std::swap(h->work, h->fork_work); swapped = false; } h->stream = h->base; }
        ~ForkGuard() { leave(); (void)join_forks(h); }
    } guard{h};
    const bool forked = slices_fork(h->overlap, h->profile, h->count_path, kmers, slice, h->filt_lo == 0 && h->filt_hi == (uint32_t)h->map_count && !h->windowed);
    if (forked) {
        for (int w = 0; w < 2; ++w) if (!h->fork_stream[w]) HIPC(h->fork_stream[w].create(hipStreamNonBlocking));
        hipEvent_t e_in; int erc = ev_get(h, &e_in); if (erc) return erc;
        HIPC(hipEventRecord(e_in, h->base));
        for (int w = 0; w < 2; ++w) HIPC(hipStreamWaitEvent(h->fork_stream[w].get(), e_in, 0));
    }
    uint64_t slice_no = 0;
    for (uint64_t a = 0; a < kmers; a += slice, ++slice_no) {
        const uint64_t b = std::min(kmers, a + slice);
        int rc = reserve(h, b - a, b - a);
        if (rc) return rc;
        const SliceView v = slice_view(d_bases, d_inv, len, h->k, a, b);
        const bool table_ok = part_table_ok(h->shape(), true);
        bool part = slice_partitions(b - a, table_ok, h->table_bytes(), h->n_regions, h->pend_budget, h->pend_records, h->arena.p != nullptr, h->arena_bytes);
        if (h->count_path == 1) part = false;
        if (h->count_path == 2) {
            if (!table_ok) return fail(KQ_ERR_INVALID, "table too large for the partitioned path");
            part = true;
        }
        if (part) {
            if (forked) {
                const int w = (int)(slice_no & 1);
                if (w == 1) { std::swap(h->work, h->fork_work); guard.swapped = true; }
                h->stream = h->fork_stream[w].get();
                h->fork_busy[w] = true;
            }
            rc = count_partitioned(h, v.ab, v.lead, v.len, v.er, v.pinv);
            if (forked) h->fork_busy[slice_no & 1] = true;
            guard.leave();
            if (rc) return rc;
            continue;
        }
        if (forked) { rc = join_forks(h); if (rc) return rc; }
        PartCfg filt = plan_cfg(h->shape());
        filt.filt_lo = h->filt_lo; filt.filt_hi = h->filt_hi;
        materialize(h);
        h->table_empty = false;
        hipLaunchKernelGGL(k_count_direct, dim3(grid_for(h, n_tiles_of(v.lead, v.len), 1, 32)), dim3(TILE_THREADS), 0, h->stream,
                           h->view(), v.ab, v.lead, v.len, h->k, v.er, filt, v.pinv);
        HIPC(hipGetLastError());
    }
    return KQ_OK;
}
int kq_count_batch_dev(kq_handle* h, const char* d_bases, uint64_t len) { return count_seq_dev(h, d_bases, nullptr, len); }
int kq_count_packed_dev(kq_handle* h, const uint32_t* d_codes, const uint16_t* d_inv, uint64_t n_bases) {
    if (!d_inv && n_bases) return fail(KQ_ERR_INVALID, "null argument");
    return count_seq_dev(h, (const char*)d_codes, d_inv, n_bases);
}
void kq_pack_bases(const char* bases, uint64_t len, uint32_t* codes, uint16_t* inv) {
    static const struct Lut { uint8_t v[256]; Lut() { for (int i = 0; i < 256; ++i) v[i] = 4; v['A'] = v['a'] = 0; v['C'] = v['c'] = 1; v['G'] = v['g'] = 2; v['T'] = v['t'] = 3; } } lut;
    const uint64_t full = len / 16;
    const uint8_t* b = (const uint8_t*)bases;
    for (uint64_t u = 0; u < full; ++u, b += 16) {
        uint32_t c = 0, m = 0;
        for (int i = 0; i < 16; ++i) { const uint32_t x = lut.v[b[i]]; c |= (x & 3u) << (2 * i); m |= (x >> 2) << i; }
        codes[u] = c; inv[u] = (uint16_t)m;
    }
// ... 1722 lines not shown
```

Before: 59.68 billion.

## Add compact MID4 intermediate record format to drop aux byte stream between levels

Adds a new intermediate format that packs the narrow record and its edge/aux bits into a single 32-bit word, with edge indices re-encoded base-5, for the middle partition level. Each segment is split into two halves, so the segment kernel reads a 2x offset table. The last tight level then no longer reads or writes a separate aux byte array. The new path is on by default when its eligibility checks pass, and an option or env var can force the old narrow path. This cuts memory traffic between levels at the cost of extra bit manipulation and a doubled offset table copy.

```diff
diff --git a/include/kreeq_amd.h b/include/kreeq_amd.h
--- a/include/kreeq_amd.h
+++ b/include/kreeq_amd.h
@@ -59,7 +59,7 @@
 int  kq_set_stream(kq_handle* h, void* hip_stream);
 void* kq_get_stream(kq_handle* h);
 enum { KQ_OPT_TRUST_CAPACITY = 1, KQ_OPT_COUNT_PATH = 2, KQ_OPT_SLICE_KMERS = 3, KQ_OPT_COUNT_MAP_RANGE = 4, KQ_OPT_PROFILE = 5,
-       KQ_OPT_LOOKUP_PATH = 6, KQ_OPT_MERGE_PATH = 7, KQ_OPT_NARROW_MID = 8, KQ_OPT_PENDING_BYTES = 9, KQ_OPT_BUCKET_WINDOW = 10, KQ_OPT_OVERLAP = 11, KQ_OPT_COUNT_MAP_PASSES = 12, KQ_OPT_KERNEL_SET = 13, KQ_OPT_SHARD_WINDOW = 14, KQ_OPT_SUBGRAPH_BATCH = 15, KQ_OPT_VARIANT_BATCH = 16,
+       KQ_OPT_LOOKUP_PATH = 6, KQ_OPT_MERGE_PATH = 7, KQ_OPT_NARROW_MID = 8, KQ_OPT_PENDING_BYTES = 9, KQ_OPT_BUCKET_WINDOW = 10, KQ_OPT_OVERLAP = 11, KQ_OPT_COUNT_MAP_PASSES = 12, KQ_OPT_KERNEL_SET = 13, KQ_OPT_SHARD_WINDOW = 14, KQ_OPT_SUBGRAPH_BATCH = 15, KQ_OPT_VARIANT_BATCH = 16, KQ_OPT_MID_FORMAT = 17,
        KQ_OPT_TEST_FAIL_PLAN = 100  };
 int  kq_set_option(kq_handle* h, int option, int64_t value);
 int  kq_get_profile(kq_handle* h, char* buf, uint64_t cap);
diff --git a/kreeq_amd/capi.py b/kreeq_amd/capi.py
--- a/kreeq_amd/capi.py
+++ b/kreeq_amd/capi.py
@@ -240,7 +240,7 @@
         _check(load().kq_flush(self._h))
 
     def set_option(self, option, value):
-        opt = {"trust_capacity": 1, "count_path": 2, "slice_kmers": 3, "count_map_range": 4, "profile": 5, "lookup_path": 6, "merge_path": 7, "narrow_mid": 8, "pending_bytes": 9, "bucket_window": 10, "overlap": 11, "count_map_passes": 12, "kernel_set": 13, "shard_window": 14, "subgraph_batch": 15, "variant_batch": 16, "test_fail_plan": 100}[option]
+        opt = {"trust_capacity": 1, "count_path": 2, "slice_kmers": 3, "count_map_range": 4, "profile": 5, "lookup_path": 6, "merge_path": 7, "narrow_mid": 8, "pending_bytes": 9, "bucket_window": 10, "overlap": 11, "count_map_passes": 12, "kernel_set": 13, "shard_window": 14, "subgraph_batch": 15, "variant_batch": 16, "mid_format": 17, "test_fail_plan": 100}[option]
         if option == "count_map_range":
             value = int(value[0]) | (int(value[1]) << 16)
         if option in ("count_path", "lookup_path", "merge_path"):
diff --git a/kreeq_amd/csrc/kq_formats.h b/kreeq_amd/csrc/kq_formats.h
--- a/kreeq_amd/csrc/kq_formats.h
+++ b/kreeq_amd/csrc/kq_formats.h
@@ -19,6 +19,8 @@
 constexpr int FMT_TOP8 = 4;
 constexpr int FMT_TIGHT = 5;
 constexpr int FMT_NARROW_TO_TIGHT = 6;
+constexpr int FMT_MID4 = 7;
+constexpr int FMT_NARROW_TO_MID4 = 8;
 
 constexpr int MS_THREADS = 256;
 constexpr int MS_ITEMS = 16;
@@ -61,6 +63,7 @@
     uint32_t nr_mid, nr_fshift, nr_fmask, nr_f24;
     uint32_t spb;
     uint32_t rep_shift;
+    uint32_t mid4_sb = 0;
     const uint32_t* rstart = nullptr;
 };
 }
diff --git a/kreeq_amd/csrc/kq_kernels.h b/kreeq_amd/csrc/kq_kernels.h
--- a/kreeq_amd/csrc/kq_kernels.h
+++ b/kreeq_amd/csrc/kq_kernels.h
@@ -536,9 +536,9 @@
                                                            const unsigned long long* __restrict__ unit_base, const uint32_t* __restrict__ m2,
                                                            const unsigned long long* __restrict__ group_base, uint64_t* __restrict__ out,
                                                            uint8_t* __restrict__ out_aux) {
-    constexpr bool WIDE = FMT == FMT_WIDE, TIGHT = FMT == FMT_NARROW_TO_TIGHT, NARROW = FMT == FMT_NARROW || TIGHT, CONVERT = FMT == FMT_PACK8_TO_NARROW,
-                   TOP8 = FMT == FMT_TOP8, HAS_AUX = WIDE || NARROW;
-    constexpr int MS_FMT = (CONVERT || TIGHT) ? FMT_NARROW : TOP8 ? FMT_PACK8 : FMT;
+    constexpr bool WIDE = FMT == FMT_WIDE, TIGHT = FMT == FMT_NARROW_TO_TIGHT, MID4 = FMT == FMT_NARROW_TO_MID4, NARROW = FMT == FMT_NARROW || TIGHT || MID4,
+                   CONVERT = FMT == FMT_PACK8_TO_NARROW, TOP8 = FMT == FMT_TOP8, HAS_AUX = WIDE || NARROW;
+    constexpr int MS_FMT = (CONVERT || TIGHT || MID4) ? FMT_NARROW : TOP8 ? FMT_PACK8 : FMT;
     const uint32_t* recs32 = reinterpret_cast<const uint32_t*>(recs);
     __shared__ MsShared<NBC, MS_FMT, LV_TILE> s;
     __shared__ uint32_t s_rst[TIGHT ? NBC : 1];
@@ -579,6 +579,7 @@
                     const uint32_t bn = i >= hi ? nb : narrow_bin(lv, b, (uint32_t)rec[j]);
                     rec[j] = narrow_word(tight_rec(b >> lv.nr_shift, (uint32_t)rec[j], aux[j], s_rst[bn < nb ? bn : 0u]), 0u, bn);
                 }
+                else if (MID4) rec[j] = narrow_word(mid4_from_narrow((uint32_t)rec[j], aux[j], lv.mid4_sb), 0u, i >= hi ? nb : narrow_bin(lv, b, (uint32_t)rec[j]));
                 else if (NARROW) rec[j] = narrow_word((uint32_t)rec[j], aux[j], i >= hi ? nb : narrow_bin(lv, b, (uint32_t)rec[j]));
                 else if (CONVERT) {
                     const uint64_t hh = rec_hash<false>(rec[j]);
@@ -702,6 +703,7 @@
 #ifndef KQ_LVG_BACK
 #define KQ_LVG_BACK 0
 #endif
+template <bool MID4>
 __global__ __launch_bounds__(LV_THREADS, KQ_LVS_OCC_TIGHT) void k_lv_segment_s(const uint32_t* __restrict__ recs32, const uint8_t* __restrict__ recs_aux, LevelCfg lv,
                                                            const unsigned long long* __restrict__ seg_off, unsigned long long* __restrict__ gb,
                                                            uint32_t* __restrict__ out) {
@@ -715,7 +717,10 @@
     const uint32_t sub = (uint32_t)tid & ((1u << rs) - 1u), my_bin = (uint32_t)tid >> rs;
     const bool own_bin = sub == 0 && my_bin < nb;
     const uint32_t b = blockIdx.x;
-    const uint64_t lo = seg_off[b], hi = seg_off[b + 1];
+    const uint64_t lo = MID4 ? seg_off[2 * b] : seg_off[b], hi = MID4 ? seg_off[2 * b + 2] : seg_off[b + 1];
+    const uint64_t half_at = MID4 ? seg_off[2 * b + 1] : 0;
+    const uint32_t sb = lv.nr_shift;
+    auto bin_of = [&](uint64_t ri, uint32_t e) { return MID4 ? narrow_bin_pos(lv, mid4_pos(e, ri >= half_at ? 1u : 0u, sb)) : narrow_bin(lv, b, e); };
     {
         const uint32_t first = (b >> lv.nr_shift) * lv.nr_rps + (b & ((1u << lv.nr_shift) - 1u)) * lv.nr_sub;
         if ((uint32_t)tid < nb) s_rst[tid] = lv.rstart[first + tid];
@@ -737,7 +742,7 @@
 #pragma unroll
                 for (int c = 0; c < 4; ++c) {
                     const uint64_t ri = 4 * qi + c;
-                    if (qi < q1 && ri >= lo && ri < hi) atomicAdd(&s_hist[1][(narrow_bin(lv, b, e[c]) << rs) | sub], 1u);
+                    if (qi < q1 && ri >= lo && ri < hi) atomicAdd(&s_hist[1][(bin_of(ri, e[c]) << rs) | sub], 1u);
                 }
             }
         }
@@ -768,10 +773,10 @@
     for (int j = 0; j < LV_ITEMS; ++j) {
         const uint64_t i = min(pos + (uint64_t)j * LV_THREADS + tid, last);
         nxt[j] = recs32[i];
-        nxt_aux[j] = recs_aux[i];
-    }
-#pragma unroll
-    for (int j = 0; j < LV_ITEMS; ++j) { landed(nxt[j]); landed(nxt_aux[j]); }
+        nxt_aux[j] = MID4 ? 0u : recs_aux[i];
+    }
+#pragma unroll
+    for (int j = 0; j < LV_ITEMS; ++j) { landed(nxt[j]); if (!MID4) landed(nxt_aux[j]); }
     uint32_t par = 0;
     for (uint64_t r = 0; r < n_rounds; ++r, par ^= 1u) {
         uint32_t* hist = s_hist[par];
@@ -779,8 +784,10 @@
 #pragma unroll
         for (int j = 0; j < LV_ITEMS; ++j) {
             const uint64_t i = pos + (uint64_t)j * LV_THREADS + tid;
-            const uint32_t bn = i >= hi ? nb : narrow_bin(lv, b, nxt[j]);
-            w[j] = narrow_word(tight_rec(b >> lv.nr_shift, nxt[j], nxt_aux[j], s_rst[bn < nb ? bn : 0u]), 0u, bn);
+            const uint32_t bn = i >= hi ? nb : bin_of(i, nxt[j]);
+            const uint32_t rst = s_rst[bn < nb ? bn : 0u];
+            w[j] = narrow_word(MID4 ? tight_from_mid4(b, mid4_pos(nxt[j], i >= half_at ? 1u : 0u, sb), nxt[j], sb, rst)
+                                    : tight_rec(b >> lv.nr_shift, nxt[j], nxt_aux[j], rst), 0u, bn);
             if (bn != nb) atomicAdd(&hist[(bn << rs) | sub], 1u);
         }
         pos = BACK ? (r + 1 < n_rounds ? pos - LV_TILE : pos) : pos + LV_TILE;
@@ -788,7 +795,7 @@
         for (int j = 0; j < LV_ITEMS; ++j) {
             const uint64_t i = min(pos + (uint64_t)j * LV_THREADS + tid, last);
             nxt[j] = recs32[i];
-            nxt_aux[j] = recs_aux[i];
+            nxt_aux[j] = MID4 ? 0u : recs_aux[i];
         }
         __syncthreads();
         const uint32_t cnt = (uint32_t)tid < n_ctr ? hist[tid] : 0u;
@@ -819,7 +826,7 @@
 #pragma unroll
         for (int it = 0; it < LV_ITEMS; ++it) cg[it] = s_grel[(uint32_t)(tid + it * LV_THREADS) < total ? narrow_word_bin(cv[it]) : 0u] + (tid + it * LV_THREADS);
 #pragma unroll
-        for (int j = 0; j < LV_ITEMS; ++j) { landed(nxt[j]); landed(nxt_aux[j]); }
+        for (int j = 0; j < LV_ITEMS; ++j) { landed(nxt[j]); if (!MID4) landed(nxt_aux[j]); }
 #pragma unroll
         for (int it = 0; it < LV_ITEMS; ++it)
             if ((uint32_t)(tid + it * LV_THREADS) < total) out[cg[it]] = (uint32_t)cv[it];
diff --git a/kreeq_amd/csrc/kq_mid4_core.h b/kreeq_amd/csrc/kq_mid4_core.h
--- /dev/null
+++ b/kreeq_amd/csrc/kq_mid4_core.h
@@ -0,0 +1,36 @@
+#pragma once
+#include <cstdint>
+#include "kq_formats.h"
+
+#if defined(__HIPCC__)
+#define KQ_M4_HD __host__ __device__ __forceinline__
+#else
+#define KQ_M4_HD inline
+#endif
+
+namespace kq {
+
+KQ_M4_HD uint32_t idx6_to_e5(uint32_t idx6) {
+    const uint32_t f = idx6 & 7u, b = (idx6 >> 3) & 7u;
+    return 5u * (f < 4u ? f : 4u) + (b < 4u ? b : 4u);
+}
+KQ_M4_HD uint32_t e5_to_idx6(uint32_t e5) {
+    const uint32_t f = (e5 * 13u) >> 6;
+    return f | ((e5 - 5u * f) << 3);
+}
+KQ_M4_HD uint32_t mid4_from_narrow(uint32_t main32, uint32_t aux, uint32_t sb) {
+    const uint32_t t = (main32 << 2) | (aux & 3u);
+    return ((t << (sb - 1u)) & ~31u) | idx6_to_e5(aux >> 2);
+}
+KQ_M4_HD uint32_t mid4_pos(uint32_t w, uint32_t half, uint32_t sb) { return (half << (23u - sb)) | (w >> (9u + sb)); }
+
+KQ_M4_HD uint32_t tight_rec(uint32_t bucket, uint32_t main32, uint32_t aux, uint32_t rstart_r) {
+    const uint32_t d = ((bucket << (32 - NARROW_CBITS)) | (main32 >> NARROW_CBITS)) - rstart_r;
+    return (d << 16) | ((main32 & 0xFFu) << 8) | ((aux & 3u) << 6) | (aux >> 2);
+}
+KQ_M4_HD uint32_t tight_from_mid4(uint32_t seg, uint32_t pos, uint32_t w, uint32_t sb, uint32_t rstart_r) {
+    const uint32_t d = ((seg << (24u - sb)) | pos) - rstart_r;
+    return (d << 16) | ((((w & ~31u) >> (sb - 1u)) & 1023u) << 6) | e5_to_idx6(w & 31u);
+}
+
+}
diff --git a/kreeq_amd/csrc/kq_partition.h b/kreeq_amd/csrc/kq_partition.h
--- a/kreeq_amd/csrc/kq_partition.h
+++ b/kreeq_amd/csrc/kq_partition.h
@@ -1,6 +1,7 @@
 #pragma once
 #include "kq_device.h"
 #include "kq_formats.h"
+#include "kq_mid4_core.h"
 
 namespace kq {
 
@@ -42,10 +43,6 @@
     return (h >> 8) | ((uint64_t)edge_idx6(is_fw, prev, next) << REC_EDGE_SHIFT);
 }
 
-__device__ __forceinline__ uint32_t tight_rec(uint32_t bucket, uint32_t main32, uint32_t aux, uint32_t rstart_r) {
-    const uint32_t d = ((bucket << (32 - NARROW_CBITS)) | (main32 >> NARROW_CBITS)) - rstart_r;
-    return (d << 16) | ((main32 & 0xFFu) << 8) | ((aux & 3u) << 6) | (aux >> 2);
-}
 __device__ __forceinline__ uint64_t tight_hash(uint32_t t, uint32_t rstart_r) { return ((uint64_t)((t >> 16) + rstart_r) << 32) | ((uint64_t)((t >> 6) & 1023u) << 22); }
 __device__ __forceinline__ uint64_t top8_rec(uint64_t h, uint32_t idx6) { return ((h << NARROW_CBITS) & ~63ull) | idx6; }
 __device__ __forceinline__ uint64_t top8_hash(uint32_t bucket, uint64_t rec) { return ((uint64_t)bucket << (64 - NARROW_CBITS)) | ((rec & ~63ull) >> NARROW_CBITS); }
@@ -59,11 +56,13 @@
 __device__ __forceinline__ uint32_t narrow_region(uint32_t bucket, uint32_t main32, uint64_t n_regions) {
     return __umulhi((bucket << (32 - NARROW_CBITS)) | (main32 >> NARROW_CBITS), (uint32_t)n_regions);
 }
+__device__ __forceinline__ uint32_t narrow_bin_pos(const LevelCfg& lv, uint32_t fs) {
+    return lv.nr_f24 ? umul24u(fs, lv.nr_sub) >> lv.nr_fshift : (uint32_t)(((uint64_t)fs * lv.nr_sub) >> lv.nr_fshift);
+}
 __device__ __forceinline__ uint32_t narrow_bin(const LevelCfg& lv, uint32_t , uint32_t main32) {
     const uint32_t f = main32 >> NARROW_CBITS;
     if (lv.nr_mid) return f >> lv.nr_fshift;
-    const uint32_t fs = f & lv.nr_fmask;
-    return lv.nr_f24 ? umul24u(fs, lv.nr_sub) >> lv.nr_fshift : (uint32_t)(((uint64_t)fs * lv.nr_sub) >> lv.nr_fshift);
+    return narrow_bin_pos(lv, f & lv.nr_fmask);
 }
 
 template <int NBC, int FMT, int TILE = MS_TILE>
diff --git a/kreeq_amd/csrc/kq_plan_host.h b/kreeq_amd/csrc/kq_plan_host.h
--- a/kreeq_amd/csrc/kq_plan_host.h
+++ b/kreeq_amd/csrc/kq_plan_host.h
@@ -84,6 +84,11 @@
 inline int plan_fmt(const PartCfg& cfg, int k) { return !cfg.narrow ? FMT_PACK8 : k > PART_MAX_K ? FMT_TOP8 : FMT_NARROW; }
 inline int sequence_fmt(int fmt, int k) { return k > PART_MAX_K && fmt != FMT_TOP8 ? FMT_WIDE : fmt; }
 inline bool tight_ok(int fmt, uint64_t n_regions, bool has_region_starts) { return fmt == FMT_NARROW && n_regions >= TIGHT_MIN_REGIONS && has_region_starts; }
+constexpr int MID4_HASH_BITS = 27;
+inline bool mid4_ok(int fmt, int k, uint32_t sub_bits, bool last_tight) {
+    return fmt == FMT_NARROW && sub_bits > 0 && last_tight && k <= (int)NARROW_MAX_K &&
+           2 * k - (int)(NARROW_CBITS + sub_bits + 1) <= MID4_HASH_BITS && ((uint64_t)512 << sub_bits) <= (uint64_t)SEG_MAX;
+}
 
 struct PlanSizes {
     PartCfg cfg;
@@ -115,6 +120,10 @@
     p.split2 = (p.rec_words + p.aux_words) * 8 >= ((size_t)512 << 20);
     return p;
 }
+inline bool mid4_off_fits(const PlanSizes& p) {
+    const uint64_t n_off = ((uint64_t)512 << p.cfg.sub_bits) + 1;
+    return p.groups_n >= n_off && p.m2_n / 2 >= n_off;
+}
 struct PlanLayout { uint64_t recs1, aux1, recs2, aux2, m1, seg_off, unit_base, group_base, sums, total, hot, m2, words; size_t part2_bytes; };
 inline PlanLayout plan_layout(const PlanSizes& p) {
     uint64_t here = 0, there = 0;
@@ -164,6 +173,12 @@
     lv.spb = 1;
     return lv;
 }
+inline LevelCfg level_narrow_mid4(const PartCfg& cfg, uint32_t sub_bits, bool middle) {
+    LevelCfg lv = level_narrow(cfg, sub_bits, middle);
+    lv.mid4_sb = sub_bits;
+    if (middle) { lv.nb = 2u << sub_bits; lv.nr_fshift = 23 - sub_bits; }
+    return lv;
+}
 inline LevelCfg level_flat_to_coarse(const PartCfg& cfg) {
     LevelCfg lv; lv.n_regions = cfg.n_regions; lv.n_seg = 1; lv.nb = cfg.n_coarse; lv.seg_shift = 32; lv.out_shift = cfg.g_shift; lv.in_raw = 0; lv.k = 0; lv.narrow = 0; lv.top8 = 0;
     lv.nr_shift = lv.nr_rps = lv.nr_sub = lv.nr_inv = 0; lv.nr_div = 1;
diff --git a/kreeq_amd/csrc/kq_select_host.h b/kreeq_amd/csrc/kq_select_host.h
--- a/kreeq_amd/csrc/kq_select_host.h
+++ b/kreeq_amd/csrc/kq_select_host.h
@@ -56,15 +56,23 @@
 
 inline int level_format(uint32_t lv_narrow, bool lockstep) { return lv_narrow == 2 ? FMT_TOP8 : lv_narrow ? FMT_NARROW : lockstep ? FMT_WIDE : FMT_PACK8; }
 inline KernelSel select_level_hist(uint32_t lv_narrow, bool lockstep) { return sel_of(K_LV_HIST, level_format(lv_narrow, lockstep), 0, 0, 0); }
-inline KernelSel select_level_scatter(uint32_t lv_narrow, bool lockstep, bool lv_top8, uint32_t nb, bool rstart, int kernel_set) {
+inline KernelSel select_level_scatter(uint32_t lv_narrow, bool lockstep, bool lv_top8, uint32_t nb, bool rstart, int kernel_set, bool mid4 = false) {
     const int fmt = level_format(lv_narrow, lockstep), nbc = nb < 512 ? 512 : NB_MAX;
     if (lv_top8) return sel_of(K_LV_SCATTER, FMT_PACK8_TO_NARROW, 512, 0, 0);
+    if (mid4) return sel_of(K_LV_SCATTER, FMT_NARROW_TO_MID4, 512, 0, 0);
     if (fmt == FMT_NARROW && nb < 512 && (rstart ? !(kernel_set & KS_LV_TIGHT_UNITS) : (kernel_set & KS_LV_NARROW_S) != 0)) return sel_of(K_LV_SCATTER_S, 0, 0, 0, 0, 0, rstart);
     return sel_of(K_LV_SCATTER, fmt == FMT_NARROW && rstart ? FMT_NARROW_TO_TIGHT : fmt, nbc, 0, 0);
 }
 inline KernelSel select_last_level(int plan_fmt, uint32_t lv_narrow, bool rstart, uint32_t nr_shift, uint32_t nb, uint32_t spb, bool even_buckets, int kernel_set) {
     const bool ok = plan_fmt == FMT_NARROW && lv_narrow == 1 && rstart && nr_shift != 0 && nb < 512 && spb == 1;
     return sel_of(ok && ((kernel_set & KS_SEG_ALWAYS) || (even_buckets && !(kernel_set & KS_SEG_NEVER))) ? K_LV_SEGMENT_S : K_LV_UNITS, 0, 0, 0, 0);
+}
+
+struct MidLastSel { KernelSel last; bool mid4; };
+inline MidLastSel select_mid_last(int plan_fmt, uint32_t lv_narrow, bool rstart, uint32_t nr_shift, uint32_t nb, uint32_t spb, bool even_buckets, int kernel_set,
+                                  bool mid4_eligible, bool keep_narrow) {
+    const KernelSel last = select_last_level(plan_fmt, lv_narrow, rstart, nr_shift, nb, spb, even_buckets, kernel_set);
+    return MidLastSel{last, last.fam == K_LV_SEGMENT_S && mid4_eligible && !keep_narrow};
 }
 
 inline bool table_pass_wants_matrix(int fmt, int kernel_set) { return (fmt == FMT_TIGHT || fmt == FMT_NARROW) && !(kernel_set & KS_P3_SET_OFFSETS); }
diff --git a/kreeq_amd/csrc/kreeq_amd.hip b/kreeq_amd/csrc/kreeq_amd.hip
--- a/kreeq_amd/csrc/kreeq_amd.hip
+++ b/kreeq_amd/csrc/kreeq_amd.hip
@@ -171,6 +171,7 @@
     uint64_t ev_next = 0;
     int overlap = 1;
     int kernel_set = 0;
+    bool mid_narrow = getenv("KQ_MID_FORMAT") && atoi(getenv("KQ_MID_FORMAT")) == 1;
     struct HistKey { const void* ab; const void* pinv; uint64_t lead, len, er_lo, er_hi; uint32_t g1, n_rng; int k;
                      bool operator==(const HistKey& o) const { return ab == o.ab && pinv == o.pinv && lead == o.lead && len == o.len && er_lo == o.er_lo && er_hi == o.er_hi && g1 == o.g1 && n_rng == o.n_rng && k == o.k; } };
     struct HistEntry { HistKey key; DevMem m1_all; };
@@ -404,6 +405,7 @@
 template <int K> static KernelRow<decltype(&k_p1_scatter_c<0>)> p1c() { return {sel_of(K_P1_SCATTER_C, 0, 0, 0, K), k_p1_scatter_c<K>}; }
 template <int W> static KernelRow<decltype(&k_lv_hist<0>)> lvh() { return {sel_of(K_LV_HIST, W, 0, 0, 0), k_lv_hist<W>}; }
 template <int W, int N> static KernelRow<decltype(&k_lv_scatter<0, 512>)> lvw() { return {sel_of(K_LV_SCATTER, W, N, 0, 0), k_lv_scatter<W, N>}; }
+static KernelRow<decltype(&k_lv_scatter<0, 512>)> lv_mid4() { return {sel_of(K_LV_SCATTER, FMT_NARROW_TO_MID4, 512, 0, 0), k_lv_scatter<FMT_NARROW_TO_MID4, 512>}; }
 template <bool T> static KernelRow<decltype(&k_lv_scatter_s<false>)> lvs() { return {sel_of(K_LV_SCATTER_S, 0, 0, 0, 0, 0, T), k_lv_scatter_s<T>}; }
 template <int W, bool HOT> static KernelRow<decltype(&k_count_regions<0, false>)> p3g() { return {sel_of(K_COUNT_REGIONS, W, 0, 0, 0, 0, HOT), k_count_regions<W, HOT>}; }
 template <int K, bool T> static KernelRow<decltype(&k_count_regions_q4<0, false>)> p3q() { return {sel_of(K_COUNT_REGIONS_Q4, 0, 0, 0, K, 0, T), k_count_regions_q4<K, T>}; }
@@ -562,6 +564,9 @@
         case KQ_OPT_KERNEL_SET:
             if (value < 0 || (value & ~(int64_t)KS_ALL)) return fail(KQ_ERR_INVALID, "KQ_OPT_KERNEL_SET is a mask of bits 1, 2, 4, 16, 32, 64, 128");
             h->kernel_set = (int)value; return KQ_OK;
+        case KQ_OPT_MID_FORMAT:
+            if (value < 0 || value > 1) return fail(KQ_ERR_INVALID, "KQ_OPT_MID_FORMAT must be 0 or 1");
+            h->mid_narrow = value != 0; return KQ_OK;
         case KQ_OPT_OVERLAP:
             if (value < 0 || value > 2) return fail(KQ_ERR_INVALID, "KQ_OPT_OVERLAP must be 0, 1 or 2");
             h->overlap = (int)value; return KQ_OK;
@@ -767,7 +772,7 @@
 static int launch_level_scatter(kq_handle* h, const KernelSel& s, const LevelUnits& u, const unsigned long long* gb, uint64_t* out, uint8_t* out_aux) {
     static const KernelRow<decltype(&k_lv_scatter<0, 512>)> rows[] = {
         lvw<FMT_PACK8_TO_NARROW, 512>(), lvw<FMT_TOP8, 512>(), lvw<FMT_TOP8, NB_MAX>(), lvw<FMT_NARROW_TO_TIGHT, 512>(), lvw<FMT_NARROW_TO_TIGHT, NB_MAX>(),
-        lvw<FMT_NARROW, 512>(), lvw<FMT_NARROW, NB_MAX>(), lvw<FMT_WIDE, 512>(), lvw<FMT_WIDE, NB_MAX>(), lvw<FMT_PACK8, 512>(), lvw<FMT_PACK8, NB_MAX>()};
+        lvw<FMT_NARROW, 512>(), lvw<FMT_NARROW, NB_MAX>(), lvw<FMT_WIDE, 512>(), lvw<FMT_WIDE, NB_MAX>(), lvw<FMT_PACK8, 512>(), lvw<FMT_PACK8, NB_MAX>(), lv_mid4()};
     static const KernelRow<decltype(&k_lv_scatter_s<false>)> streamed[] = {lvs<true>(), lvs<false>()};
     if (s.fam == K_LV_SCATTER_S) return launch_row(streamed, "k_lv_scatter_s", s, h, dim3(u.grid), dim3(LV_THREADS), (const uint32_t*)u.in, u.in_aux, u.lv, u.seg_lo, u.seg_hi, u.unit_base, u.m2, gb, (uint32_t*)out, out_aux);
     return launch_row(rows, "k_lv_scatter", s, h, dim3(u.grid), dim3(LV_THREADS), u.in, u.in_aux, u.lv, u.seg_lo, u.seg_hi, u.unit_base, u.m2, gb, out, out_aux);
@@ -788,14 +793,15 @@
     (void)hipMemsetAsync(gb + groups, 0, 8, h->stream);
     scan_u64(h, gb, groups + 1, p->sums, p->total + 1);
     mark(h, "k_lv_hist+offsets+scan");
-    rc = launch_level_scatter(h, select_level_scatter(lv.narrow, src.aux != nullptr, lv.top8 != 0, lv.nb, lv.rstart != nullptr, h->kernel_set), u, gb, out, out_aux);
+    rc = launch_level_scatter(h, select_level_scatter(lv.narrow, src.aux != nullptr, lv.top8 != 0, lv.nb, lv.rstart != nullptr, h->kernel_set, lv.nr_mid && lv.mid4_sb), u, gb, out, out_aux);
     mark(h, "k_lv_scatter");
     return rc;
 }
-static void run_segment_level(kq_handle* h, PartPlan* p, const LevelCfg& lv, const uint64_t* in, const uint8_t* in_aux, uint64_t* out, unsigned long long* gb) {
+static void run_segment_level(kq_handle* h, const LevelCfg& lv, const uint64_t* in, const uint8_t* in_aux, const unsigned long long* off, uint64_t* out, unsigned long long* gb) {
     mark(h, "segment_level");
     mark(h, "k_lv_hist+offsets+scan");
-    hipLaunchKernelGGL(k_lv_segment_s, dim3(lv.n_seg), dim3(LV_THREADS), 0, h->stream, (const uint32_t*)in, in_aux, with_rep_shift(lv), p->seg_off, gb, (uint32_t*)out);
+    if (lv.mid4_sb) hipLaunchKernelGGL(k_lv_segment_s<true>, dim3(lv.n_seg), dim3(LV_THREADS), 0, h->stream, (const uint32_t*)in, in_aux, with_rep_shift(lv), off, gb, (uint32_t*)out);
+    else hipLaunchKernelGGL(k_lv_segment_s<false>, dim3(lv.n_seg), dim3(LV_THREADS), 0, h->stream, (const uint32_t*)in, in_aux, with_rep_shift(lv), off, gb, (uint32_t*)out);
     mark(h, "k_lv_scatter");
 }
 __global__ void k_p3set(P3Set* sets, int i, P3Set v) { sets[i] = v; }
@@ -951,15 +957,27 @@
             last.n_seg = in.n_seg; last.spb = in.spb;
             rc = run_level(h, p, last, in, fin, fin_aux, fin_base);
         } else {
-            LevelCfg mid = level_narrow(p->cfg, sb, true, t8);
+            const bool own_in = in.spb == 1 && in.n_seg == (1u << NARROW_CBITS);
+            const MidLastSel sel = select_mid_last(p->fmt, last.narrow, last.rstart != nullptr, last.nr_shift, last.nb, last.spb, p->even_buckets, h->kernel_set,
+                                                   own_in && mid4_ok(p->fmt, h->k, sb, d.tight) && mid4_off_fits(*p), h->mid_narrow);
+            LevelCfg mid = sel.mid4 ? level_narrow_mid4(p->cfg, sb, true) : level_narrow(p->cfg, sb, true, t8);
             mid.n_seg = in.n_seg; mid.spb = in.spb;
             uint64_t* m = mid_to_2 ? p->recs2 : p->recs1;
-            uint8_t* m_aux = mid_to_2 ? p->a2() : p->a1();
+            uint8_t* m_aux = sel.mid4 ? nullptr : mid_to_2 ? p->a2() : p->a1();
+            if (sel.mid4) mark(h, "mid4_records");
             rc = run_level(h, p, mid, in, m, m_aux);
             if (rc) return rc;
+            if (sel.mid4) {
+                unsigned long long* half_off = reinterpret_cast<unsigned long long*>(p->m2);
+                (void)hipMemcpyAsync(half_off, p->group_base, (size_t)(((2u << NARROW_CBITS) << sb) + 1) * 8, hipMemcpyDeviceToDevice, h->stream);
+                last.mid4_sb = sb;
+                run_segment_level(h, last, m, nullptr, half_off, fin, fin_base);
+                *set = P3Set{fin, fin_aux, fin_base, arena ? d.n_max : p->n_max};
+                return rc;
+            }
             (void)hipMemcpyAsync(p->seg_off, p->group_base, (size_t)(((1u << NARROW_CBITS) << sb) + 1) * 8, hipMemcpyDeviceToDevice, h->stream);
-            if (select_last_level(p->fmt, last.narrow, last.rstart != nullptr, last.nr_shift, last.nb, last.spb, p->even_buckets, h->kernel_set).fam == K_LV_SEGMENT_S)
-                run_segment_level(h, p, last, m, m_aux, fin, fin_base);
+            if (sel.last.fam == K_LV_SEGMENT_S)
+                run_segment_level(h, last, m, m_aux, p->seg_off, fin, fin_base);
             else
                 rc = run_level(h, p, last, own_segments(*p, m, m_aux, last.n_seg), fin, fin_aux, fin_base);
         }
```

Measured after the change: 60.40 billion (median of 6 runs). 1.01x the previous value.
